# umutdundar99/progressive-stable-diffusion

Measured on AMD Instinct MI355X. Metric: images/sec at 512x512, 50 DDIM steps, bs/GPU=4, higher is better.
Workload: dtype f16; 1 GPU; 512x512, 50 DDIM steps, bs=4/GPU, delta-steer lambda=3.0, routing gates on, conditioning prep + VAE decode included; global_batch=4, parallelism=batch-shard x1 + 1 all-gather of uint8 frames

## Files before the change

### include/dadd_hip.h

```cpp
#ifndef DADD_HIP_H
#define DADD_HIP_H

#include <stdint.h>

#ifdef __cplusplus
extern "C" {
#endif

#define DADD_OK 0
#define DADD_EINVAL (-1)
#define DADD_EHIP (-2)
#define DADD_ESTATE (-3)

#define DADD_EPI_BIAS 1
#define DADD_EPI_ROWVEC 2
#define DADD_EPI_RESIDUAL 4
#define DADD_EPI_GEGLU 8
#define DADD_EPI_LNFOLD 128
#define DADD_EPI_LNSTAT 4096
#define DADD_PRE_GN 8192
#define DADD_PRE_GN_SILU 16384
#define DADD_EPI_GNSTAT 2048
#define DADD_EPI_GNAPPLY 32768
#define DADD_EPI_GNAPPLY_SILU 65536
#define DADD_EPI_QUICKGELU 256
#define DADD_EPI_GELU 512
#define DADD_EPI_SIGMOID 1024
#define DADD_EPI_ACT_MASK (256 | 512 | 1024)
#define DADD_TUNE_SHALLOW 16
#define DADD_TUNE_NODMA 32
#define DADD_TUNE_PERSIST 64

#define DADD_XATTN_SPLIT 0
#define DADD_XATTN_BASELINE 1

const char* dadd_last_error(void);
int dadd_version(void);
int dadd_init(void);
int dadd_device_info(int device, int64_t out[4]);

typedef struct {
  const void* x;
  const void* x2;
  const void* w;
  void* out;
  float* partial;
  const float* bias;
  const float* rowvec;
  const void* residual;
  int32_t B, Hi, Wi, C1, C2, Ho, Wo, N;
  int32_t taps, stride, ups, pad;
  int32_t ldo, ldr, ld_rowvec;
  int32_t splitk, flags, tile_n;
  int32_t tile_m;
  int32_t* counters;
  const float* ln_c1;
  float ln_eps;
  float* gn_ws;
  int32_t gn_nchunk, gn_cg;
  float* ln_stats_out;
  const float* ln_stats_in;
  int32_t ln_parts_out, ln_parts_in;
  const float* gn_in_ws;
  const float* gn_in_gamma;
  const float* gn_in_beta;
  int32_t gn_in_nchunk;
  float gn_in_eps;
  const float* gn_in_ws2;
  int32_t gn_in_nchunk2;
  void* gn_out;
  const float* gn_out_gamma;
  const float* gn_out_beta;
  float gn_out_eps;
} dadd_igemm_desc;
int dadd_conv_igemm_f16(const dadd_igemm_desc* d, void* stream);

typedef struct {
  const char* kernel;
  const char* finish;
  int32_t tile_m, tile_n;
  int32_t nsplit, kps;
  int32_t persistent;
  int32_t grid_x, grid_y, block;
  int32_t smem;
  int32_t gm, gn;
} dadd_igemm_choice;
int dadd_conv_igemm_resolve_f16(const dadd_igemm_desc* d, int num_cu, dadd_igemm_choice* out);

int dadd_conv3x3_cin8_f16(const void* x, const void* w, const float* bias, void* out, int B, int H,
                          int W, int Cout, void* stream);
int dadd_conv_in_nchw_f16(const float* x_nchw, const void* w, const float* bias, void* out, int B, int C,
                          int H, int W, int Cout, float* gn_ws, int gn_nchunk, void* stream);
int dadd_conv3x3_cout4_f16(const void* x, const void* w, const float* bias, float* out_nchw, int B,
                           int H, int W, int C, int Cout, int mode, void* stream);
int dadd_conv_out_ddim_f16(const void* x, const void* w, const float* bias, float* latents, const float* coef,
                           int B, int H, int W, int C, int Cout, void* stream);

int dadd_pack_nchw_f32_to_nhwc8_f16(const float* x, void* out, int B, int C, int H, int W,
                                    float scale, const float* mat, const float* vec, void* stream);

int dadd_gaussian_sample_f32(const float* mean, const float* logvar, const float* noise, float scale,
                             float* out, int64_t n, void* stream);

int dadd_frames_to_u8(const float* frames_nchw, void* out_nhwc_u8, int B, int H, int W, void* stream);

int dadd_q_sample_f32(const float* x0, const float* noise, const int64_t* t, const float* alphas_cumprod,
                      float* out, int B, int64_t per_sample, void* stream);
int dadd_mse_rows_f32(const float* pred, const float* target, float* out, int B, int64_t per_sample,
                      void* stream);

#define DADD_GN_MAX_CHUNKS 256
int dadd_groupnorm_f16(const void* x1, int C1, const void* x2, int C2, const float* gamma,
                       const float* beta, void* out, float* ws, int B, int HW, int groups,
                       float eps, int silu, int ws_chunks, void* stream);
int dadd_layernorm_f16(const void* x, const float* gamma, const float* beta, void* out, int M,
                       int C, float eps, void* stream);

int dadd_self_attn_f16(const void* q, const void* k, const void* v, void* out, int B, int N,
                       int heads, int d, int ld_qkv, int ld_out, void* stream);
int dadd_attn_f16(const void* q, const void* k, const void* v, void* out, int B, int Nq, int Nk, int heads,
                  int d, int ld_q, int ld_kv, int ld_out, void* stream);

int dadd_tri_xattn_f16(const void* q, const void* kv, void* out, const float* gates, float lambda,
                       const float* lambda_dev, int mode, int B, int N, int heads, int d, int T, int ld_kv,
                       void* stream);

int dadd_attn2_fused_f16(const void* x, const void* mcat, const void* vw, const float* bias,
                         const void* residual, void* out, float* ln_stats_out, const float* ln_stats_in,
                         int ln_parts_in, const float* ln_c1, const float* ln_d, float ln_eps, int B, int HW, int C,
                         void* stream);

int dadd_ffn_block_f16(const void* x, const void* stream, const float* ln_g, const float* ln_b, float ln_eps,
                       const float* b1, const float* b2, const float* bp, const void* xres, void* out, float* gn_ws,
                       int gn_nchunk, int M, int HW, int C, void* stream_handle);
int dadd_ffn_block_bytes(void);

int dadd_tf_head_f16(const void* x, const void* stream, const float* gn_ws, int gn_nchunk, const float* gn_g,
                     const float* gn_b, float gn_eps, const float* bp, const float* ln_g, const float* ln_b, float ln_eps,
                     void* hs, void* qkv, int M, int HW, int C, void* stream_handle);
int dadd_tf_head_bytes(void);
int dadd_tf_head_debug(void* buf);

int dadd_timestep_features_f32(const int64_t* t, float* out, int M, int dim, void* stream);
int dadd_linear_rows_f32(const float* x, const void* w, const float* bias, float* out, int M, int K,
                         int N, int act_in, int act_out, int w_f32, void* stream);
int dadd_begin_step(const float* table, float* cur_rows, int B, int ncols, const float* coef,
                    float* cur_coef, int32_t* step, void* stream);
int dadd_ddim_update_f32(float* x, const float* eps_c, const float* eps_u, float guidance,
                         const float* guidance_dev, const float* coef, int64_t n, void* stream);

int dadd_clip_patch_rows_f16(const float* pixels, void* out, int B, int H, int W, int patch, int Kp, void* stream);
int dadd_aoe_interp_f32(const float* labels, const float* base, const float* deltas, float* out, int B, int D,
                        int classes, void* stream);
int dadd_purifier_tail_f16(const void* img, const void* dis, const void* gate, const float* gamma,
                           const float* beta, float* out, int M, int C, float eps, void* stream);

// ... 50 lines not shown
```

### progressive-stable-diffusion_amd/backend.py

```python
from __future__ import annotations

import ctypes as C
from typing import Optional

import torch

from . import lib as L


def _p(t: Optional[torch.Tensor]):
    if t is None:
        return None
    if t.device.type != "cuda":
        raise ValueError(f"kernel argument lives on {t.device}, not on the GPU (shape {tuple(t.shape)}, {t.dtype})")
    return t.data_ptr()


_SFX = {torch.float16: "f16", torch.bfloat16: "bf16"}


def _sfx(*ts) -> str:
    kinds = {t.dtype for t in ts if t is not None and t.dtype in _SFX}
    if len(kinds) != 1:
        raise ValueError(f"one op takes fp16 or bf16 operands, not {sorted(str(k) for k in kinds) or 'neither'}")
    return _SFX[kinds.pop()]


def fill_igemm_desc(d, ptr, x, w, out, *, x2=None, bias=None, rowvec=None, residual=None, taps=1, stride=1,
                    ups=0, pad=0, flags=0, splitk=1, partial=None, tile_n=0, tile_m=0, counters=None, ln_c1=None,
                    ln_eps=1e-5, gn_ws=None, gn_nchunk=0, ln_stats_out=None, ln_stats_in=None, gn_in=None, gn_apply=None):
    b, hi, wi, c1 = x.shape
    c2 = 0 if x2 is None else x2.shape[-1]
    n = w.shape[0]
    ho, wo = out.shape[1], out.shape[2]
    assert w.shape[1] == taps * (c1 + c2), (w.shape, taps, c1, c2)
    assert out.shape[-1] == (n // 2 if flags & L.EPI_GEGLU else n) and out.shape[0] == b
    d.x, d.x2, d.w, d.out, d.partial = ptr(x), ptr(x2), ptr(w), ptr(out), ptr(partial)
    d.bias, d.rowvec, d.residual = ptr(bias), ptr(rowvec), ptr(residual)
    d.B, d.Hi, d.Wi, d.C1, d.C2, d.Ho, d.Wo, d.N = b, hi, wi, c1, c2, ho, wo, n
    d.taps, d.stride, d.ups, d.pad = taps, stride, ups, pad
    d.ldo, d.ldr = out.stride(-2), (residual.stride(-2) if residual is not None else 0)
    d.ld_rowvec = rowvec.stride(0) if rowvec is not None else 0
    d.splitk, d.flags, d.tile_n, d.tile_m = splitk, flags, tile_n, tile_m
    d.counters = ptr(counters)
    d.ln_c1, d.ln_eps = ptr(ln_c1), float(ln_eps)
    d.gn_ws, d.gn_nchunk, d.gn_cg = ptr(gn_ws), int(gn_nchunk), (n // 32 if gn_ws is not None else 0)
    if gn_ws is not None:
        assert flags & L.EPI_GNSTAT and gn_ws.numel() >= b * gn_nchunk * 64 and gn_ws.dtype == torch.float32
    if ln_c1 is not None:
        assert flags & L.EPI_LNFOLD and ln_c1.numel() == n and ln_c1.dtype == torch.float32
    m_rows = b * ho * wo
    d.ln_stats_out, d.ln_stats_in, d.ln_parts_out, d.ln_parts_in = ptr(ln_stats_out), ptr(ln_stats_in), 0, 0
    if ln_stats_out is not None:
        assert flags & L.EPI_LNSTAT and ln_stats_out.dtype == torch.float32 and ln_stats_out.dim() == 3 \
            and ln_stats_out.shape[1:] == (m_rows, 2) and ln_stats_out.is_contiguous()
        d.ln_parts_out = ln_stats_out.shape[0]
    if ln_stats_in is not None:
        assert flags & L.EPI_LNFOLD and ln_stats_in.dtype == torch.float32 and ln_stats_in.dim() == 3 \
            and ln_stats_in.shape[1:] == (b * hi * wi, 2) and ln_stats_in.is_contiguous()
        d.ln_parts_in = ln_stats_in.shape[0]
    d.gn_in_ws = d.gn_in_gamma = d.gn_in_beta = d.gn_in_ws2 = None
    d.gn_in_nchunk, d.gn_in_eps, d.gn_in_nchunk2 = 0, 0.0, 0
    if gn_in is not None:
        ws_in, nch_in, gam, bet, eps_in = gn_in[:5]
        assert flags & L.PRE_GN and ws_in.dtype == gam.dtype == bet.dtype == torch.float32 \
            and ws_in.numel() >= b * nch_in * 64 and gam.numel() == c1 + c2 and bet.numel() == c1 + c2
        d.gn_in_ws, d.gn_in_gamma, d.gn_in_beta = ptr(ws_in), ptr(gam), ptr(bet)
        d.gn_in_nchunk, d.gn_in_eps = int(nch_in), float(eps_in)
        if len(gn_in) > 5:
            ws2, nch2 = gn_in[5], gn_in[6]
            assert x2 is not None and ws2.dtype == torch.float32 and ws2.numel() >= b * nch2 * 64
            d.gn_in_ws2, d.gn_in_nchunk2 = ptr(ws2), int(nch2)
    d.gn_out = d.gn_out_gamma = d.gn_out_beta = None
    d.gn_out_eps = 0.0
    if gn_apply is not None:
        g_out, gam, bet, eps_o = gn_apply
        assert flags & L.EPI_GNAPPLY and g_out.shape == out.shape and g_out.dtype == out.dtype and g_out.is_contiguous() \
            and gam.dtype == bet.dtype == torch.float32 and gam.numel() == n and bet.numel() == n
        d.gn_out, d.gn_out_gamma, d.gn_out_beta, d.gn_out_eps = ptr(g_out), ptr(gam), ptr(bet), float(eps_o)
    if partial is not None:
        assert partial.numel() >= splitk * b * ho * wo * n


class HipBackend:
    name = "hip-gfx950"

    def __init__(self, device: torch.device):
        if not torch.cuda.is_available():
            raise RuntimeError("HipBackend needs a ROCm device (torch.cuda.is_available() is False)")
        self.lib = L.load()
        self.device = torch.device(device)
        self.stream = torch.cuda.Stream(device=self.device)
        self._desc = L.IgemmDesc()
        self._wdesc = L.WgradDesc()
        self._ddesc = L.DgradDesc()
        self._edesc = L.EndWgradDesc()
        self._gdesc = L.GnGradDesc()
        self._adesc = L.AttnGradDesc()
        self._n_cu = None
        self._capturing = False
        self._prof_on = False
        with torch.cuda.device(self.device):
            L.check(self.lib.dadd_init())

    @property
    def s(self):
        return self.stream.cuda_stream

    def ctx(self):
        return torch.cuda.stream(self.stream)

    def empty(self, shape, dtype):
        with self.ctx():
            return torch.empty(shape, dtype=dtype, device=self.device)

    def zeros(self, shape, dtype):
        with self.ctx():
            return torch.zeros(shape, dtype=dtype, device=self.device)

    def _after_producer(self, src: torch.Tensor):
        if src.device.type == "cuda" and not self._capturing:
            cur = torch.cuda.current_stream(self.device)
            if cur != self.stream:
                self.stream.wait_stream(cur)
                src.record_stream(self.stream)

    def to_device(self, t: torch.Tensor, dtype=None):
        self._after_producer(t)
        with self.ctx():
            return t.to(device=self.device, dtype=dtype or t.dtype).contiguous()

    def copy_(self, dst: torch.Tensor, src: torch.Tensor):
        self._after_producer(src)
        with self.ctx():
            dst.copy_(src.reshape(dst.shape))

    def zero_(self, t: torch.Tensor):
        with self.ctx():
            t.zero_()

    def clone(self, t: torch.Tensor):
        with self.ctx():
            return t.detach().clone()

    def synchronize(self):
        self.stream.synchronize()

    def wait_current(self):
        self.stream.wait_stream(torch.cuda.current_stream(self.device))

    def release_to_current(self):
        torch.cuda.current_stream(self.device).wait_stream(self.stream)

    @staticmethod
    def _scratch_numel(fn, args, message):
        n = int(fn(*args))
        if n < 0:
            raise ValueError(message.format(*args))
        return n

    def _splitm(self, m, tiles):
        if self._n_cu is None:
            self._n_cu = torch.cuda.get_device_properties(self.device).multi_processor_count
        return max(1, min(-(-2 * self._n_cu // tiles), -(-m // 64)))

    @staticmethod
    def _param_grad_checks(dgamma, dbeta, c, ws, need):
        together = (dgamma is None) == (dbeta is None)
        shaped = all(t is None or (t.dtype == torch.float32 and t.numel() == c and t.is_contiguous()) for t in (dgamma, dbeta))
        ws_ok = ws is not None and ws.dtype == torch.float32 and ws.is_contiguous() and ws.numel() >= need
        return together, shaped, ws_ok

    @staticmethod
    def _pointwise_width(op, f):
        if f % 8 or f == 0:
            raise ValueError(f"{op}: F = {f} must be a positive multiple of 8")

    def pack_latents(self, x, out, scale=1.0, mat=None, vec=None):
        b, c, h, w = x.shape
        assert x.dtype == torch.float32 and out.dtype == torch.float16 and out.shape == (b, h, w, 8)
        L.check(self.lib.dadd_pack_nchw_f32_to_nhwc8_f16(_p(x), _p(out), b, c, h, w, float(scale),
                                                         _p(mat), _p(vec), self.s))

    def conv_cin8(self, x, w, bias, out):
        b, h, wd, c8 = x.shape
        assert c8 == 8 and w.shape[1:] == (9, 8) and out.shape == (b, h, wd, w.shape[0])
        L.check(self.lib.dadd_conv3x3_cin8_f16(_p(x), _p(w), _p(bias), _p(out), b, h, wd, w.shape[0],
                                               self.s))

    def conv_in_nchw(self, x, w, bias, out, gn_ws=None, gn_nchunk=0):
        b, c, h, wd = x.shape
        assert x.dtype == torch.float32 and c <= 4 and w.shape[1:] == (9, 8) and out.shape == (b, h, wd, w.shape[0])
        assert gn_ws is None or (gn_ws.dtype == torch.float32 and gn_ws.numel() >= b * gn_nchunk * 64)
        fn = getattr(self.lib, "dadd_conv_in_nchw_" + _sfx(w, out))
        L.check(fn(_p(x), _p(w), _p(bias), _p(out), b, c, h, wd, w.shape[0], _p(gn_ws), gn_nchunk, self.s))

    def conv_cout4(self, x, w, bias, out, mode=0):
        b, h, wd, c = x.shape
        co = w.shape[0]
        assert w.shape == (co, 9, c) and out.shape == (b, co, h, wd) and out.dtype == torch.float32
        fn = getattr(self.lib, "dadd_conv3x3_cout4_" + _sfx(x, w))
        L.check(fn(_p(x), _p(w), _p(bias), _p(out), b, h, wd, c, co, int(mode), self.s))

    def conv_out_ddim(self, x, w, bias, latents, coef):
        b, h, wd, c = x.shape
        co = w.shape[0]
        assert w.shape == (co, 9, c) and latents.shape == (b, co, h, wd) and latents.dtype == torch.float32 \
            and coef.numel() == 4 and coef.dtype == torch.float32
        fn = getattr(self.lib, "dadd_conv_out_ddim_" + _sfx(x, w))
        L.check(fn(_p(x), _p(w), _p(bias), _p(latents), _p(coef), b, h, wd, c, co, self.s))

    def q_sample(self, x0, noise, t, alphas_cumprod, out):
        b = x0.shape[0]
        assert x0.dtype == torch.float32 and t.dtype == torch.int64 and t.shape == (b,) and noise.shape == x0.shape
        L.check(self.lib.dadd_q_sample_f32(_p(x0), _p(noise), _p(t), _p(alphas_cumprod), _p(out), b,
                                           x0.numel() // b, self.s))

    def mse_rows(self, pred, target, out):
        b = pred.shape[0]
        assert pred.shape == target.shape and out.shape == (b,) and pred.dtype == torch.float32
        L.check(self.lib.dadd_mse_rows_f32(_p(pred), _p(target), _p(out), b, pred.numel() // b, self.s))

    def frames_to_u8(self, frames, out):
        b, c, h, w = frames.shape
        assert c == 3 and frames.dtype == torch.float32 and out.dtype == torch.uint8 and out.shape == (b, h, w, 3)
        L.check(self.lib.dadd_frames_to_u8(_p(frames), _p(out), b, h, w, self.s))

    def gaussian_sample(self, mean, logvar, noise, out, scale=1.0):
        assert mean.shape == logvar.shape == noise.shape == out.shape and mean.dtype == torch.float32
        L.check(self.lib.dadd_gaussian_sample_f32(_p(mean), _p(logvar), _p(noise), float(scale), _p(out),
                                                  mean.numel(), self.s))

    def igemm(self, x, w, out, *, x2=None, bias=None, rowvec=None, residual=None, taps=1, stride=1,
              ups=0, pad=0, flags=0, splitk=1, partial=None, tile_n=0, tile_m=0, counters=None, ln_c1=None,
              ln_eps=1e-5, gn_ws=None, gn_nchunk=0, ln_stats_out=None, ln_stats_in=None, gn_in=None, gn_apply=None):
        fn = getattr(self.lib, "dadd_conv_igemm_" + _sfx(x, x2, w, out, residual, None if gn_apply is None else gn_apply[0]))
        d = self._desc
        fill_igemm_desc(d, _p, x, w, out, x2=x2, bias=bias, rowvec=rowvec, residual=residual, taps=taps, stride=stride,
                        ups=ups, pad=pad, flags=flags, splitk=splitk, partial=partial, tile_n=tile_n, tile_m=tile_m,
                        counters=counters, ln_c1=ln_c1, ln_eps=ln_eps, gn_ws=gn_ws, gn_nchunk=gn_nchunk,
                        ln_stats_out=ln_stats_out, ln_stats_in=ln_stats_in, gn_in=gn_in, gn_apply=gn_apply)
        L.check(fn(C.byref(d), self.s))

    def wgrad_splitm(self, m, n, c, taps=1):
        return self._splitm(m, -(-n // 64) * taps * (c // 64))

    @staticmethod
    def wgrad_partial_numel(splitm, n, c, taps=1):
        return splitm * (n * taps * c + n) if splitm > 1 else 0

    @staticmethod
    def _pixel_ld(t):
        ld = t.stride(-2)
        want, ok = ld, t.stride(-1) == 1
        for size, st in zip(reversed(t.shape[:-1]), reversed(t.stride()[:-1])):
            ok = ok and (size == 1 or st == want)
            want *= size
        if not ok:
            raise ValueError(f"expected dense pixels with one row stride, got shape {tuple(t.shape)} strides {t.stride()}")
        return ld

    def wgrad(self, dy, x, dw, *, dbias=None, taps=1, stride=1, ups=0, pad=0, splitm=None, partial=None, ld_tap=None):
        if dy.dim() == 2:
            dy, x = dy.unsqueeze(0).unsqueeze(0), x.unsqueeze(0).unsqueeze(0)
        b, ho, wo, n = dy.shape
        bx, hi, wi, c = x.shape
        assert bx == b and dy.dim() == 4 and x.dim() == 4
        fn = getattr(self.lib, "dadd_conv_wgrad_" + _sfx(dy, x))
        assert dw.dtype == torch.float32 and dw.stride(-1) == 1 and dw.shape[0] == n
        if dw.dim() == 3:
            assert dw.shape[1:] == (taps, c) and ld_tap in (None, dw.stride(1))
            ld_tap = dw.stride(1)
        else:
            ld_tap = c if ld_tap is None else ld_tap
            assert dw.dim() == 2 and dw.shape[1] >= (taps - 1) * ld_tap + c
        assert dbias is None or (dbias.dtype == torch.float32 and dbias.numel() == n and dbias.is_contiguous())
        m = b * ho * wo
        if splitm is None:
            splitm = self.wgrad_splitm(m, n, c, taps)
        if splitm > 1:
            if partial is None:
                raise ValueError(f"wgrad with splitm = {splitm} needs a partial buffer")
            assert partial.dtype == torch.float32 and partial.is_contiguous() \
                and partial.numel() >= self.wgrad_partial_numel(splitm, n, c, taps), (partial.shape, splitm, n, taps, c)
        d = self._wdesc
        d.dy, d.x, d.dw, d.dbias, d.partial = _p(dy), _p(x), _p(dw), _p(dbias), _p(partial)
        d.B, d.Hi, d.Wi, d.C, d.Ho, d.Wo, d.N = b, hi, wi, c, ho, wo, n
        d.taps, d.stride, d.ups, d.pad = taps, stride, int(ups), pad
        d.ld_dy, d.ld_x, d.ld_dw, d.ld_tap = self._pixel_ld(dy), self._pixel_ld(x), dw.stride(0), ld_tap
        d.splitm = splitm
        L.check(fn(C.byref(d), self.s))

    def dgrad(self, dy, wt, dx, *, taps=1):
        if dy.dim() == 2:
            dy, dx = dy.view(1, 1, *dy.shape), dx.view(1, 1, *dx.shape)
        n = dy.shape[-1]
        if n % 64 != 0:
            raise ValueError(f"dgrad contracts over the N = {n} output channels of the forward; the GEMM kernels need "
                             "a multiple of 64 (the data gradient of the 4-channel conv_out is dgrad_cout4)")
        assert taps in (1, 9) and wt.shape == (dx.shape[-1], taps * n) and dy.is_contiguous() and dx.is_contiguous()
        self.igemm(dy, wt, dx, taps=taps, pad=1 if taps == 9 else 0)

    def dgrad_cout4(self, dy_nchw_f32, wt, dx):
        if dy_nchw_f32.dim() != 4 or dy_nchw_f32.dtype != torch.float32 or not 1 <= dy_nchw_f32.shape[1] <= 4:
            raise ValueError(f"dgrad_cout4 takes dy fp32 NCHW with 1..4 channels, got {tuple(dy_nchw_f32.shape)} {dy_nchw_f32.dtype}")
        b, _, h, wd = dy_nchw_f32.shape
        if wt.dim() != 3 or wt.shape[1:] != (9, 8) or dx.shape != (b, h, wd, wt.shape[0]) or not (
                dy_nchw_f32.is_contiguous() and wt.is_contiguous() and dx.is_contiguous()):
            raise ValueError(f"dgrad_cout4: dy {tuple(dy_nchw_f32.shape)} takes contiguous wt [C,9,8] and dx [B,H,W,C], got "
                             f"{tuple(wt.shape)} and {tuple(dx.shape)}")
        self.conv_in_nchw(dy_nchw_f32, wt, None, dx)

    def end_wgrad_splitm(self, m, cw):
        return self._splitm(m, max(1, cw // 64))

    def end_wgrad_partial_numel(self, splitm, ct, cw, mode):
        return self._scratch_numel(self.lib.dadd_end_wgrad_partial_floats, (int(mode), int(ct), int(cw), int(splitm)),
                                   "end_wgrad takes mode 0 or 1, Ct in 1..4 and Cw a multiple of 64 (got mode {}, Ct {}, Cw {})")

    def end_wgrad(self, thin, wide, dw, *, dbias=None, mode, splitm=None, partial=None):
        if thin.dim() != 4 or wide.dim() != 4 or thin.dtype != torch.float32 or not thin.is_contiguous():
            raise ValueError(f"end_wgrad takes thin fp32 NCHW (contiguous) and wide NHWC, got {tuple(thin.shape)} {thin.dtype} "
                             f"and {tuple(wide.shape)}")
        b, ct, h, wd = thin.shape
# ... 460 lines not shown
```

### progressive-stable-diffusion_amd/csrc/bf16_names.h

```cpp
#pragma once
#define DADD_BF16 1

#define IgemmArgs IgemmArgs_bf16
#define IgemmLaunch IgemmLaunch_bf16

#define igemm_kernel igemm_kernel_bf16
#define splitk_finish_kernel splitk_finish_kernel_bf16
#define splitk_finish_gn_kernel splitk_finish_gn_kernel_bf16
#define splitk_finish_gnapply_kernel splitk_finish_gnapply_kernel_bf16
#define igemm_dma_kernel igemm_dma_kernel_bf16
#define conv3x3_halo_kernel conv3x3_halo_kernel_bf16
#define gn_stats_kernel gn_stats_kernel_bf16
#define gn_apply_kernel gn_apply_kernel_bf16
#define gn_fused_kernel gn_fused_kernel_bf16
#define gn_reduce_kernel gn_reduce_kernel_bf16
#define layernorm_kernel layernorm_kernel_bf16
#define flash_kernel flash_kernel_bf16
#define xattn_kernel xattn_kernel_bf16
#define conv_in_nchw_kernel conv_in_nchw_kernel_bf16
#define conv_in_nchw_gn_kernel conv_in_nchw_gn_kernel_bf16
#define conv_cout4_kernel conv_cout4_kernel_bf16
#define wgrad_kernel wgrad_kernel_bf16
#define wgrad_finish_kernel wgrad_finish_kernel_bf16
#define gn_grad_stats_kernel gn_grad_stats_kernel_bf16
#define gn_grad_partial_kernel gn_grad_partial_kernel_bf16
#define gn_grad_apply_kernel gn_grad_apply_kernel_bf16
#define layernorm_grad_kernel layernorm_grad_kernel_bf16
#define geglu_kernel geglu_kernel_bf16
#define geglu_grad_kernel geglu_grad_kernel_bf16
#define attn_grad_stats_kernel attn_grad_stats_kernel_bf16
#define attn_grad_dkv_kernel attn_grad_dkv_kernel_bf16
#define attn_grad_dq_kernel attn_grad_dq_kernel_bf16
#define dgrad_kernel dgrad_kernel_bf16
#define EndWgradArgs EndWgradArgs_bf16
#define end_wgrad_kernel end_wgrad_kernel_bf16
#define end_wgrad_finish_kernel end_wgrad_finish_kernel_bf16
#define gelu_kernel gelu_kernel_bf16
#define gelu_grad_kernel gelu_grad_kernel_bf16
#define gate_tail_kernel gate_tail_kernel_bf16
#define gate_tail_grad_kernel gate_tail_grad_kernel_bf16
#define rowvec_grad_kernel rowvec_grad_kernel_bf16
#define rowvec_grad_finish_kernel rowvec_grad_finish_kernel_bf16
#define relayout_kernel relayout_kernel_bf16

#define dadd_init_igemm dadd_init_igemm_bf16
#define dadd_init_igemm_dma dadd_init_igemm_dma_bf16
#define dadd_igemm_dma_row dadd_igemm_dma_row_bf16
#define dadd_igemm_resolve dadd_igemm_resolve_bf16
#define dadd_init_conv_halo dadd_init_conv_halo_bf16
#define dadd_conv_halo_applicable dadd_conv_halo_applicable_bf16
#define dadd_conv_halo_gn_channels dadd_conv_halo_gn_channels_bf16
#define dadd_conv_halo_row dadd_conv_halo_row_bf16
#define dadd_init_norm dadd_init_norm_bf16
#define dadd_init_attention dadd_init_attention_bf16
#define dadd_init_attn_grad dadd_init_attn_grad_bf16

#define dadd_conv_igemm_f16 dadd_conv_igemm_bf16
#define dadd_conv_igemm_resolve_f16 dadd_conv_igemm_resolve_bf16
#define dadd_groupnorm_f16 dadd_groupnorm_bf16
#define dadd_layernorm_f16 dadd_layernorm_bf16
#define dadd_attn_f16 dadd_attn_bf16
#define dadd_attn_debug dadd_attn_debug_bf16
#define dadd_self_attn_f16 dadd_self_attn_bf16
#define dadd_tri_xattn_f16 dadd_tri_xattn_bf16
#define dadd_conv_in_nchw_f16 dadd_conv_in_nchw_bf16
#define dadd_conv3x3_cout4_f16 dadd_conv3x3_cout4_bf16
#define dadd_conv_out_ddim_f16 dadd_conv_out_ddim_bf16
#define dadd_conv_wgrad_f16 dadd_conv_wgrad_bf16

#define dadd_groupnorm_grad_f16 dadd_groupnorm_grad_bf16
#define dadd_layernorm_grad_f16 dadd_layernorm_grad_bf16
#define dadd_geglu_f16 dadd_geglu_bf16
#define dadd_geglu_grad_f16 dadd_geglu_grad_bf16

#define dadd_attn_grad_f16 dadd_attn_grad_bf16

#define dadd_gelu_f16 dadd_gelu_bf16
#define dadd_gelu_grad_f16 dadd_gelu_grad_bf16
#define dadd_purifier_gate_tail_f16 dadd_purifier_gate_tail_bf16
#define dadd_purifier_gate_tail_grad_f16 dadd_purifier_gate_tail_grad_bf16

#define dadd_rowvec_grad_f16 dadd_rowvec_grad_bf16

#define dadd_conv_dgrad_f16 dadd_conv_dgrad_bf16

#define dadd_conv_end_wgrad_f16 dadd_conv_end_wgrad_bf16

#define dadd_dgrad_relayout_f16 dadd_dgrad_relayout_bf16
```

### progressive-stable-diffusion_amd/csrc/igemm.hip

```cpp
#include "dadd_common.h"
#include "igemm_args.h"
#include <cstdlib>
#include <string>
#include "igemm_epilogue.h"

namespace {

constexpr int BM = 128;
constexpr int BK = 64;

__device__ __forceinline__ int lds_off(int row, int chunk) {
  return (row * 8 + (chunk ^ ((row >> 1) & 7))) * 8;
}

template <int BM, int BN, bool DEEP>
__global__ __launch_bounds__(256, 2) void igemm_kernel(const IgemmArgs p) {
  constexpr int WM = BM / 2;
  constexpr int MI = WM / 16;
  constexpr int WN = BN / 2;
  constexpr int J = WN / 16;
  constexpr int EPI = (DEEP && BN == 128) ? EPI_COLS : EPI_TILE;
  constexpr int NA = BM * 8 / 256;
  constexpr int NB = BN * 8 / 256;
  extern __shared__ __attribute__((aligned(16))) char smem[];
// ... 298 lines not shown
#pragma unroll
        for (int e = 0; e < VEC; ++e) v[e] = fmaf(keep, tt[u][e], v[e]);
      }
    }
    if (p.flags & DADD_EPI_BIAS) v += *reinterpret_cast<const fv*>(p.bias + c);
    if (p.flags & DADD_EPI_ROWVEC) v += *reinterpret_cast<const fv*>(p.rowvec + (size_t)b * p.ld_rowvec + c);
    if (p.flags & DADD_EPI_RESIDUAL) {
      const hv rv = *reinterpret_cast<const hv*>(p.residual + m * p.ldr + c);
#pragma unroll
      for (int e = 0; e < VEC; ++e) v[e] += (float)rv[e];
    }
    hv o;
#pragma unroll
    for (int e = 0; e < VEC; ++e) o[e] = (half_t)v[e];
    *reinterpret_cast<hv*>(p.out + m * p.ldo + c) = o;
    *reinterpret_cast<hv*>(slab + row * cg + VEC * cv) = o;
  }
  __syncthreads();
  float s = 0.f, ss = 0.f;
  if (t < 256) {
    for (int idx = t; idx < npair; idx += 256) {
      const h2 v = *reinterpret_cast<const h2*>(slab + 2 * idx);
      const float a = (float)v[0], d = (float)v[1];
      s += a + d;
      ss += a * a + d * d;
    }
    s = wave_sum(s);
    ss = wave_sum(ss);
    if (lane == 0) { red[0][wave] = s; red[1][wave] = ss; }
  }
  __syncthreads();
  const double n = (double)HW * (double)cg;
  const double sum = (double)red[0][0] + (double)red[0][1] + (double)red[0][2] + (double)red[0][3];
  const double sq = (double)red[1][0] + (double)red[1][1] + (double)red[1][2] + (double)red[1][3];
  const double mu = sum / n;
  double var = sq / n - mu * mu;
  if (var < 0.0) var = 0.0;
  const float mean = (float)mu, rstd = (float)(1.0 / sqrt(var + (double)p.gno_eps));
  const bool silu = (p.flags & DADD_EPI_GNAPPLY_SILU) != 0;
  for (int idx = t; idx < npair; idx += 512) {
    const int row = idx / hp, cp = idx - row * hp;
    const int c = c0 + 2 * cp;
    const h2 v = *reinterpret_cast<const h2*>(slab + 2 * idx);
    h2 o;
#pragma unroll
    for (int e = 0; e < 2; ++e) {
      const float sc = rstd * p.gno_gamma[c + e];
      float f = ((float)v[e] - mean) * sc + p.gno_beta[c + e];
      if (silu) f = dadd_silu(f);
      o[e] = (half_t)f;
    }
    *reinterpret_cast<h2*>(p.gno_out + ((size_t)b * HW + row) * p.N + c) = o;
  }
}

constexpr double L2_KEEP = 3.0e6;

constexpr int smem_bytes(int bm, int bn) {
  return 2 * (bm + bn) * BK * (int)sizeof(half_t) + (bm == 128 ? (bn == 160 ? 8192 : LN_LDS_BYTES) : 4096);
}

#define REG_ROW(BM, BN, DEEP) \
  {DADD_KNAME("igemm_kernel") "<" #BM ", " #BN ", " #DEEP ">", igemm_kernel<BM, BN, DEEP>, 256, smem_bytes(BM, BN), {BM, BN, DEEP}}
const IgemmKernel REG_KERNELS[] = {
    REG_ROW(128, 128, false), REG_ROW(128, 128, true), REG_ROW(128, 160, false), REG_ROW(64, 128, false),
    REG_ROW(64, 128, true),   REG_ROW(64, 160, false), REG_ROW(64, 160, true),
};
#undef REG_ROW
#define FIN_ROW(KERNEL, THREADS, ...) {DADD_KNAME(#KERNEL), KERNEL<__VA_ARGS__>, THREADS, 0, {__VA_ARGS__}}
const IgemmFinish FINISH_KERNELS[] = {
    FIN_ROW(splitk_finish_gnapply_kernel, 512, 4), FIN_ROW(splitk_finish_gnapply_kernel, 512, 2),
    {DADD_KNAME("splitk_finish_kernel"), splitk_finish_kernel, 256, 0, {}},
    FIN_ROW(splitk_finish_gn_kernel, 256, 160, 16), FIN_ROW(splitk_finish_gn_kernel, 256, 160, 64),
    FIN_ROW(splitk_finish_gn_kernel, 256, 128, 16), FIN_ROW(splitk_finish_gn_kernel, 256, 128, 64),
};
#undef FIN_ROW

int g_num_cu = 0;

}

int dadd_init_igemm() {
  int rc = dadd_init_igemm_dma();
  if (rc == DADD_OK) rc = dadd_init_conv_halo();
  if (rc == DADD_OK) rc = dadd_set_max_lds(REG_KERNELS);
  int dev = 0;
  DADD_HIP(hipGetDevice(&dev));
  DADD_HIP(hipDeviceGetAttribute(&g_num_cu, hipDeviceAttributeMultiprocessorCount, dev));
  return rc;
}

int dadd_igemm_resolve(const dadd_igemm_desc* d, int num_cu, IgemmLaunch* out) {
  DADD_REQUIRE(d != nullptr, "igemm: null descriptor");
  IgemmArgs& a = out->a;
  a = IgemmArgs{};
  a.x = static_cast<const half_t*>(d->x);
  a.x2 = static_cast<const half_t*>(d->x2);
  a.w = static_cast<const half_t*>(d->w);
  a.out = static_cast<half_t*>(d->out);
  a.partial = d->partial;
  a.bias = d->bias;
  a.rowvec = d->rowvec;
  a.residual = static_cast<const half_t*>(d->residual);
  a.counters = d->counters;
  a.B = d->B; a.Hi = d->Hi; a.Wi = d->Wi; a.C1 = d->C1; a.C2 = d->C2;
  a.Ho = d->Ho; a.Wo = d->Wo; a.N = d->N;
  a.taps = d->taps; a.stride = d->stride; a.ups = d->ups; a.pad = d->pad;
  a.flags = d->flags & (15 | DADD_TUNE_PERSIST | DADD_EPI_LNFOLD | DADD_EPI_ACT_MASK | DADD_EPI_GNSTAT | DADD_EPI_LNSTAT |
                        DADD_PRE_GN | DADD_PRE_GN_SILU | DADD_EPI_GNAPPLY | DADD_EPI_GNAPPLY_SILU);
  a.gno_out = static_cast<half_t*>(d->gn_out);
  a.gno_gamma = d->gn_out_gamma;
  a.gno_beta = d->gn_out_beta;
  a.gno_eps = d->gn_out_eps;
  a.gn_ws = d->gn_ws;
  a.gn_nchunk = d->gn_nchunk;
  a.gn_cg = d->gn_cg;
  a.ln_c1 = d->ln_c1;
  a.ln_eps = d->ln_eps;
  a.gni_ws = d->gn_in_ws;
  a.gni_gamma = d->gn_in_gamma;
  a.gni_beta = d->gn_in_beta;
  a.gni_nchunk = d->gn_in_nchunk;
  a.gni_eps = d->gn_in_eps;
  a.gni_ws2 = d->gn_in_ws2;
  a.gni_nchunk2 = d->gn_in_nchunk2;
  a.ln_stats_out = d->ln_stats_out;
  a.ln_stats_in = (a.flags & DADD_EPI_LNFOLD) ? d->ln_stats_in : nullptr;
  a.ln_parts_in = d->ln_parts_in;
  const int Cin = a.C1 + a.C2;
  const bool geglu = (a.flags & DADD_EPI_GEGLU) != 0;
  a.ldo = d->ldo > 0 ? d->ldo : (geglu ? a.N / 2 : a.N);
  a.ldr = d->ldr > 0 ? d->ldr : a.N;
  a.ld_rowvec = d->ld_rowvec > 0 ? d->ld_rowvec : a.N;

  DADD_REQUIRE(a.x && a.w && a.out, "igemm: null x/w/out");
  DADD_REQUIRE(a.taps == 1 || a.taps == 9, "igemm: taps must be 1 or 9, got %d", a.taps);
  DADD_REQUIRE(a.B > 0 && a.Hi > 0 && a.Wi > 0 && a.Ho > 0 && a.Wo > 0 && a.N > 0,
               "igemm: non-positive extent");
  DADD_REQUIRE(Cin % 64 == 0 && a.C1 % 64 == 0 && a.C1 > 0,
               "igemm: channels must be multiples of 64 (C1=%d C2=%d)", a.C1, a.C2);
  DADD_REQUIRE(a.C2 == 0 || a.x2 != nullptr, "igemm: C2>0 needs x2");
  DADD_REQUIRE(a.N % 8 == 0, "igemm: N must be a multiple of 8, got %d", a.N);
  DADD_REQUIRE(a.stride == 1 || a.stride == 2, "igemm: stride must be 1 or 2");
  DADD_REQUIRE(!(a.ups && (a.stride != 1 || a.taps != 9)), "igemm: ups needs a stride-1 3x3");
  DADD_REQUIRE(dadd_aligned16(a.x) && dadd_aligned16(a.w) && dadd_aligned16(a.out) &&
                   (a.x2 == nullptr || dadd_aligned16(a.x2)),
               "igemm: pointers must be 16-byte aligned");
  DADD_REQUIRE(!(a.flags & DADD_EPI_BIAS) || a.bias, "igemm: bias flag without bias");
  DADD_REQUIRE(!(a.flags & DADD_EPI_ROWVEC) || a.rowvec, "igemm: rowvec flag without rowvec");
  DADD_REQUIRE(!(a.flags & DADD_EPI_RESIDUAL) || a.residual, "igemm: residual flag without ptr");
  DADD_REQUIRE(!(a.flags & DADD_EPI_ACT_MASK) || (!geglu && d->splitk <= 1),
               "igemm: an activation epilogue excludes GEGLU and split-K");
  DADD_REQUIRE(!(a.flags & DADD_EPI_LNFOLD) || (a.ln_c1 && a.taps == 1 && a.C2 == 0 && d->splitk <= 1 && a.ln_eps > 0.f),
               "igemm: a folded LayerNorm needs c1, a plain linear over one source (K = C) and no split-K");
  DADD_REQUIRE(a.ln_stats_in == nullptr ||
                   (a.ln_parts_in > 0 && (size_t)a.ln_parts_in * a.B * a.Ho * a.Wo * 8 < 0x7FF00000ull),
               "igemm: ln_stats_in needs ln_parts_in > 0 and fewer than 2 GiB of partials");
  DADD_REQUIRE(a.ldo % 4 == 0 && a.ldr % 4 == 0 && a.ld_rowvec % 4 == 0,
               "igemm: leading dimensions must be multiples of 4");

  a.M = a.B * a.Ho * a.Wo;
  a.K = a.taps * Cin;
  a.nkt = a.K / BK;
  int tile_n = d->tile_n;
  if (geglu) {
    DADD_REQUIRE(a.N % 128 == 0 && (tile_n == 0 || tile_n == 128), "igemm: GEGLU needs N%%128==0");
    tile_n = 128;
  }
  if (tile_n == 0) tile_n = (a.N % 160 == 0) ? 160 : 128;
  DADD_REQUIRE(tile_n == 64 || tile_n == 128 || tile_n == 160, "igemm: tile_n must be 64, 128 or 160");
  a.ntiles = (a.N + tile_n - 1) / tile_n;

  int splitk = d->splitk > 1 ? d->splitk : 1;
  if (splitk > a.nkt) splitk = a.nkt;
  a.kps = (a.nkt + splitk - 1) / splitk;
  const int nsplit = (a.nkt + a.kps - 1) / a.kps;
  a.splitk = nsplit;
  DADD_REQUIRE(nsplit == 1 || (a.partial != nullptr && !geglu),
               "igemm: split-K needs a partial buffer and no GEGLU");

  bool deep = (d->flags & DADD_TUNE_SHALLOW) == 0;
  int tile_m = d->tile_m;
  DADD_REQUIRE(tile_m == 0 || tile_m == 64 || tile_m == 128, "igemm: tile_m must be 0, 64 or 128");
  if (tile_m == 0) tile_m = 128;
  a.mtiles = (a.M + tile_m - 1) / tile_m;
  {
    const double a_bytes = 2.0 * a.B * a.Hi * a.Wi * Cin, w_bytes = 2.0 * a.N * a.K;
    if (a_bytes >= w_bytes) {
      a.gm = (a.mtiles + 7) / 8;
      a.gn = a.ntiles;
    } else {
      a.gm = a.mtiles;
      a.gn = (a.ntiles + 7) / 8;
    }
    if (a.taps == 1 && !(a_bytes >= w_bytes) && a_bytes > L2_KEEP) {
      double best = 1e30;
      for (int ms = 2; ms <= 4; ms *= 2) {
        const int ns = 8 / ms;
        if (a.mtiles % ms || a.ntiles % ns || a_bytes / ms > L2_KEEP) continue;
        const double fetch = a_bytes / ms + w_bytes / ns;
        if (fetch < best) { best = fetch; a.gm = a.mtiles / ms; a.gn = a.ntiles / ns; }
      }
    }
  }
  a.korder = 0;
  const bool dma = ((d->flags & DADD_TUNE_NODMA) == 0 || ((a.flags & DADD_EPI_LNFOLD) && !a.ln_stats_in)) &&
                   !(tile_m == 64 && a.ups);
  DADD_REQUIRE(tile_n != 64 || (dma && tile_m == 64 && !geglu), "igemm: 64-column tiles exist for the 64-row LDS-DMA kernel only");
  const bool persistent = dma && tile_m == 128 && (a.flags & DADD_TUNE_PERSIST) && nsplit == 1 && !a.ups && num_cu > 0 &&
                          a.mtiles * a.ntiles > num_cu;
  if (persistent && ((d->flags & DADD_TUNE_SHALLOW) ? false : 2.0 * a.B * a.Hi * a.Wi * Cin >= 2.0 * a.N * a.K))
    a.gm = a.gn = 0;
  a.fd_on = (size_t)a.B * a.Ho * a.Wo < DADD_FASTDIV_MAX && (size_t)a.K < DADD_FASTDIV_MAX &&
            (size_t)a.mtiles * a.ntiles < DADD_FASTDIV_MAX;
  a.plain = a.taps == 1 && a.stride == 1 && a.pad == 0 && !a.ups && a.Ho == a.Hi && a.Wo == a.Wi;
  if (a.fd_on) {
    a.fd_howo = dadd_fastdiv_make((uint32_t)(a.Ho * a.Wo));
    a.fd_wo = dadd_fastdiv_make((uint32_t)a.Wo);
    a.fd_cin = dadd_fastdiv_make((uint32_t)Cin);
    a.ngn = 1;
    a.fd_t1 = a.fd_t2 = dadd_fastdiv_make(1);
    if (a.gm == 0) {
      a.fd_t0 = dadd_fastdiv_make((uint32_t)a.ntiles);
    } else if (a.gn >= a.ntiles) {
      a.fd_t0 = dadd_fastdiv_make((uint32_t)(a.gm * a.ntiles));
      a.fd_t1 = dadd_fastdiv_make((uint32_t)a.gm);
    } else if (a.gm >= a.mtiles) {
      a.fd_t0 = dadd_fastdiv_make((uint32_t)(a.mtiles * a.gn));
      a.fd_t1 = dadd_fastdiv_make((uint32_t)a.mtiles);
    } else {
      a.ngn = a.ntiles / a.gn;
      a.fd_t0 = dadd_fastdiv_make((uint32_t)(a.gm * a.gn));
      a.fd_t1 = dadd_fastdiv_make((uint32_t)a.gm);
      a.fd_t2 = dadd_fastdiv_make((uint32_t)a.ngn);
    }
  }
  const bool halo = dma && tile_m == 128 && dadd_conv_halo_applicable(a, tile_n);
  int halo_ns = 1;
  if (halo) {
    const int chunks = Cin / BK;
    int sk = d->splitk > 1 ? d->splitk : 1;
    if (sk > chunks) sk = chunks;
    a.kps = (chunks + sk - 1) / sk;
    halo_ns = (chunks + a.kps - 1) / a.kps;
    a.splitk = halo_ns;
    DADD_REQUIRE(halo_ns == 1 || a.partial != nullptr, "igemm: split-K needs a partial buffer");
  }
  if ((a.flags & DADD_EPI_GNSTAT) && (halo ? halo_ns : nsplit) > 1) {
    const int cb = (a.N % 160 == 0) ? 160 : 128, howo = a.Ho * a.Wo;
    const int rows = a.gn_nchunk > 0 ? howo / a.gn_nchunk : 0;
    DADD_REQUIRE(a.gn_ws && a.gn_cg > 0 && a.N == 32 * a.gn_cg && !geglu && a.counters == nullptr && a.N % cb == 0 &&
                     cb % a.gn_cg == 0 && (rows == 16 || rows == 64) && a.M % rows == 0 && howo % rows == 0 &&
                     a.gn_nchunk * rows == howo && !(a.flags & (DADD_EPI_LNFOLD | DADD_EPI_ACT_MASK)),
                 "igemm: GroupNorm statistics with split-K need the finish kernel (no tickets), N == 32 groups in blocks of "
                 "160 / 128 columns, and chunks of 16 or 64 rows: gn_nchunk == Ho*Wo / 16 (or / 64)");
  } else if (a.flags & DADD_EPI_GNSTAT) {
    const int wm_rows = tile_m / 2, wn_cols = tile_n / 2, howo = a.Ho * a.Wo;
    DADD_REQUIRE(a.gn_ws && a.gn_cg > 0 && a.N == 32 * a.gn_cg && !geglu && (tile_n == 128 || tile_n == 160) &&
                     wn_cols % a.gn_cg == 0 && a.M % tile_m == 0 && a.N % tile_n == 0 && howo % wm_rows == 0 &&
                     a.gn_nchunk == howo / wm_rows && !(a.flags & (DADD_EPI_LNFOLD | DADD_EPI_ACT_MASK)),
                 "igemm: GroupNorm statistics need full tiles of 128/160 columns holding whole groups, whole-wave row blocks "
                 "inside one sample (Ho*Wo %% %d == 0, gn_nchunk == Ho*Wo / %d), N == 32 groups, no split-K", wm_rows, wm_rows);
  }
  if (a.flags & DADD_EPI_GNAPPLY) {
    DADD_REQUIRE((halo ? halo_ns : nsplit) > 1 && a.counters == nullptr && a.gno_out && a.gno_gamma && a.gno_beta &&
                     a.gno_eps > 0.f && a.N % 64 == 0 && a.ldo % 2 == 0 && a.ldr % 2 == 0 &&
                     (size_t)a.Ho * a.Wo * (a.N / 32) * 2 <= 16 * 1024 && dadd_aligned16(a.gno_out) &&
                     !(a.flags & (DADD_EPI_GNSTAT | DADD_EPI_LNFOLD | DADD_EPI_LNSTAT | DADD_EPI_ACT_MASK)),
                 "igemm: GroupNorm of the output in the finish kernel needs a finish-kernel split-K launch, gn_out / gamma / "
                 "beta / eps, N %% 64 == 0, a (sample, group) slab of <= 16 KiB and no other statistics / activation flags");
  } else {
    DADD_REQUIRE(!(a.flags & DADD_EPI_GNAPPLY_SILU), "igemm: DADD_EPI_GNAPPLY_SILU without DADD_EPI_GNAPPLY");
  }
  if (a.flags & DADD_EPI_LNSTAT) {
    const int wn_cols = tile_n / 2;
    DADD_REQUIRE(a.ln_stats_out && !geglu && !halo && a.N % wn_cols == 0 && d->ln_parts_out == a.N / wn_cols &&
                     (nsplit == 1 || a.counters != nullptr) && !(a.flags & DADD_EPI_GNSTAT),
                 "igemm: LayerNorm row partials need ln_stats_out, N %% (tile_n/2) == 0, ln_parts_out == N / (tile_n/2) = %d, "
                 "no GEGLU and no finish-kernel split-K", a.N / wn_cols);
  }
  if (a.flags & DADD_PRE_GN) {
    const int cgc = Cin / 32;
    DADD_REQUIRE(a.C2 == 0 || (a.gni_ws2 && a.gni_nchunk2 >= 1 && a.gni_nchunk2 <= 256 && cgc > 0 && a.C1 % 32 == 0 &&
                               a.C2 % 32 == 0 && cgc % (a.C1 / 32) == 0 && cgc % (a.C2 / 32) == 0 && a.C1 % cgc == 0),
                 "igemm: GroupNorm over a concatenation needs the partials of both sources and group widths that nest "
                 "((C1+C2)/32 a multiple of C1/32 and C2/32, dividing C1)");
    DADD_REQUIRE(halo && !(d->flags & DADD_TUNE_SHALLOW) && Cin <= dadd_conv_halo_gn_channels(a.Wo) &&
                     Cin % 32 == 0 && a.gni_ws &&
                     a.gni_gamma && a.gni_beta && a.gni_nchunk >= 1 && a.gni_nchunk <= 256 && a.gni_eps > 0.f,
                 "igemm: GroupNorm on the way in needs the 3x3 halo kernel (stride 1, 64/32/16-wide map, 128x160 tiles), "
                 "Cin <= 1152 / 2048 / 2432 (W = 64 / 32 / 16), the chunk partials (<= 256 chunks), gamma, beta and eps");
  } else {
    DADD_REQUIRE(!(a.flags & DADD_PRE_GN_SILU), "igemm: DADD_PRE_GN_SILU without DADD_PRE_GN");
  }
  const bool window = (size_t)a.B * a.Hi * a.Wi * (size_t)(a.C1 > a.C2 ? a.C1 : a.C2) * 2 < 0x7FF00000ull &&
                      (size_t)a.N * a.K * 2 < 0x7FF00000ull;
  out->nsplit = halo ? halo_ns : nsplit;
  out->tile_m = tile_m;
  out->tile_n = tile_n;
  out->persistent = !halo && persistent;
  out->grid = out->persistent ? dim3(num_cu) : dim3(a.mtiles * a.ntiles, out->nsplit);
  a.pf_kt = (dma && !halo && a.korder == 0 && !out->persistent && a.mtiles >= DADD_PF_MIN_SHARE)
                ? (a.kps < DADD_PF_KTILES ? a.kps : DADD_PF_KTILES) : 0;
  if (halo) {
    DADD_REQUIRE(window, "conv_halo: operand larger than the 2 GiB buffer window");
    const bool duo = (d->flags & DADD_TUNE_SHALLOW) != 0 && !(a.flags & DADD_PRE_GN);
    if (d->flags & DADD_TUNE_SHALLOW) a.flags |= DADD_TUNE_SHALLOW;
    out->main = dadd_conv_halo_row(a.Wo, duo, (a.flags & DADD_PRE_GN) != 0);
  } else if (dma) {
    DADD_REQUIRE(window, "igemm(dma): operand larger than the 2 GiB buffer window");
    DADD_REQUIRE(tile_m == 128 || !a.ups, "igemm(dma): the 64-row tiles have no upsample gather");
    const int lnk = (a.ups || !(a.flags & DADD_EPI_LNFOLD)) ? 0 : (a.ln_stats_in == nullptr ? 1 : (tile_m == 128 ? 2 : 0));
    out->main = dadd_igemm_dma_row(tile_m, tile_n, !out->persistent && tile_m == 128 && a.ups, out->persistent, lnk);
  } else {
    out->main = dadd_find_row(REG_KERNELS, tile_m, tile_n, deep && !(tile_m == 128 && tile_n == 160));
  }
  DADD_REQUIRE(out->main != nullptr, "igemm: no kernel for %d x %d tiles", tile_m, tile_n);
  out->finish = nullptr;
  out->fgrid = dim3(0);
  out->fsmem = 0;
  if (out->nsplit > 1 && a.counters == nullptr) {
    if (a.flags & DADD_EPI_GNAPPLY) {
      const bool vec4 = (a.N / 32) % 4 == 0 && a.ldo % 4 == 0 && a.ldr % 4 == 0 && a.ld_rowvec % 4 == 0;
      out->finish = dadd_find_row(FINISH_KERNELS, vec4 ? 4 : 2);
      out->fgrid = dim3(32, a.B);
      out->fsmem = (unsigned)(a.Ho * a.Wo * (a.N / 32) * 2);
    } else if (!(a.flags & DADD_EPI_GNSTAT)) {
      const size_t total = (size_t)a.M * (a.N / 4);
      const int blocks = (int)((total + 255) / 256);
      out->finish = dadd_find_row(FINISH_KERNELS, 0);
      out->fgrid = dim3(blocks > 2048 ? 2048 : blocks);
    } else {
      const int cb = (a.N % 160 == 0) ? 160 : 128, rows = (a.Ho * a.Wo) / a.gn_nchunk == 16 ? 16 : 64;
      out->finish = dadd_find_row(FINISH_KERNELS, cb, rows);
      out->fgrid = dim3(a.M / rows, a.N / cb);
    }
  }
  return DADD_OK;
}

extern "C" int dadd_conv_igemm_f16(const dadd_igemm_desc* d, void* stream) {
  hipStream_t s = static_cast<hipStream_t>(stream);
  IgemmLaunch l;
  const int rc = dadd_igemm_resolve(d, g_num_cu, &l);
  if (rc != DADD_OK) return rc;
  const IgemmArgs& a = l.a;
  dadd_launch({l.main->name, dadd_igemm_flop(a), dadd_igemm_bytes(a)}, l.main->fn, l.grid, dim3(l.main->threads), l.main->smem, s, a);
  if (l.finish) {
    double bytes = (double)a.M * a.N * (4.0 * l.nsplit + 2.0 + ((a.flags & DADD_EPI_RESIDUAL) ? 2.0 : 0.0));
    if (a.flags & DADD_EPI_GNAPPLY) bytes += 2.0 * a.M * a.N;
    dadd_launch({l.finish->name, 0.0, bytes}, l.finish->fn, l.fgrid, dim3(l.finish->threads), l.fsmem, s, a, l.nsplit);
  }
  DADD_LAUNCH_CHECK();
  return DADD_OK;
}

extern "C" int dadd_conv_igemm_resolve_f16(const dadd_igemm_desc* d, int num_cu, dadd_igemm_choice* out) {
  DADD_REQUIRE(out != nullptr, "igemm: null choice");
  IgemmLaunch l;
  const int rc = dadd_igemm_resolve(d, num_cu, &l);
  if (rc != DADD_OK) return rc;
  *out = {l.main->name, l.finish ? l.finish->name : nullptr, l.tile_m, l.tile_n, l.nsplit, l.a.kps, l.persistent,
          (int)l.grid.x, (int)l.grid.y, l.main->threads, l.main->smem, l.a.gm, l.a.gn};
  return DADD_OK;
}
```

### progressive-stable-diffusion_amd/csrc/igemm_args.h

```cpp
#pragma once
#include "dadd_common.h"
#include "fastdiv.h"

struct IgemmArgs {
  const half_t* x;
  const half_t* x2;
  const half_t* w;
  half_t* out;
  float* partial;
  const float* bias;
  const float* rowvec;
  const half_t* residual;
  int* counters;
  float* gn_ws;
  int gn_nchunk, gn_cg;
  const float* ln_c1;
  float ln_eps;
  float* ln_stats_out;
  const float* ln_stats_in;
  int ln_parts_in;
  const float* gni_ws;
  const float* gni_gamma;
  const float* gni_beta;
  int gni_nchunk;
  float gni_eps;
  const float* gni_ws2;
  int gni_nchunk2;
  half_t* gno_out;
  const float* gno_gamma;
  const float* gno_beta;
  float gno_eps;
  int B, Hi, Wi, C1, C2, Ho, Wo, N;
  int taps, stride, ups, pad;
  int ldo, ldr, ld_rowvec;
  int splitk, flags;
  int M, K, nkt, kps, ntiles;
  int korder;
  int mtiles, gm, gn;
  int fd_on, plain;
  dadd_fastdiv fd_howo, fd_wo, fd_cin;
  dadd_fastdiv fd_t0, fd_t1, fd_t2;
  int ngn;
  int pf_kt;
};

#ifndef DADD_PF_KTILES
#define DADD_PF_KTILES 24
#endif
#ifndef DADD_PF_MIN_SHARE
#define DADD_PF_MIN_SHARE 16
#endif
typedef unsigned dadd_u4 __attribute__((ext_vector_type(4)));
__device__ __forceinline__ dadd_u4 dadd_pf_desc(const void* base, int bytes) {
  const unsigned long long a = (unsigned long long)base;
  return dadd_u4{(unsigned)a, (unsigned)(a >> 32) & 0xFFFFu, (unsigned)bytes, 0x00020000u};
}
__device__ __forceinline__ void dadd_pf_line(unsigned& sink, unsigned off, dadd_u4 desc) {
#if defined(__HIP_DEVICE_COMPILE__)
  asm volatile("buffer_load_dword %0, %1, %2, 0 offen" : "+v"(sink) : "v"(off), "s"(desc));
#endif
}
__device__ __forceinline__ void dadd_pf_drain(unsigned& sink) {
#if defined(__HIP_DEVICE_COMPILE__)
  asm volatile("s_waitcnt vmcnt(0)" : "+v"(sink)::"memory");
#endif
}

__device__ __forceinline__ int row_sample(const IgemmArgs& p, int m, int HoWo) {
  return p.fd_on ? (int)dadd_fastdiv_div((uint32_t)m, p.fd_howo) : m / HoWo;
}
__device__ __forceinline__ void row_decode(const IgemmArgs& p, int m, int HoWo, int& b, int& oy, int& ox) {
  b = row_sample(p, m, HoWo);
  const int rem = m - b * HoWo;
  oy = p.fd_on ? (int)dadd_fastdiv_div((uint32_t)rem, p.fd_wo) : rem / p.Wo;
  ox = rem - oy * p.Wo;
}

__device__ __forceinline__ int xcd_remap(int bid, int nwg) {
  const int q = nwg >> 3, r = nwg & 7, xcd = bid & 7, slot = bid >> 3;
  return (xcd < r ? xcd * (q + 1) : r * (q + 1) + (xcd - r) * q) + slot;
}

__device__ __forceinline__ void tile_decode(const IgemmArgs& p, int tile_id, int& mt, int& nt) {
  if (p.gm == 0) {
    nt = tile_id % p.ntiles;
    mt = tile_id / p.ntiles;
  } else if (p.gn >= p.ntiles) {
    const int per = p.gm * p.ntiles;
    const int g = tile_id / per, idx = tile_id - g * per;
    const int base = g * p.gm;
    const int gsz = min(p.gm, p.mtiles - base);
    mt = base + idx % gsz;
    nt = idx / gsz;
  } else if (p.gm >= p.mtiles) {
    const int per = p.mtiles * p.gn;
    const int g = tile_id / per, idx = tile_id - g * per;
    mt = idx % p.mtiles;
    nt = g * p.gn + idx / p.mtiles;
  } else {
    const int per = p.gm * p.gn;
    const int g = tile_id / per, idx = tile_id - g * per;
    const int ngn = p.ntiles / p.gn;
    const int gmi = g / ngn, gni = g - gmi * ngn;
    mt = gmi * p.gm + idx % p.gm;
    nt = gni * p.gn + idx / p.gm;
  }
}

__device__ __forceinline__ void tile_decode_fast(const IgemmArgs& p, int tile_id, int& mt, int& nt) {
  const auto div = [&](int n, const dadd_fastdiv& f, int d) { return p.fd_on ? (int)dadd_fastdiv_div((uint32_t)n, f) : n / d; };
  if (p.gm == 0) {
    mt = div(tile_id, p.fd_t0, p.ntiles);
    nt = tile_id - mt * p.ntiles;
  } else if (p.gn >= p.ntiles) {
    const int per = p.gm * p.ntiles;
    const int g = div(tile_id, p.fd_t0, per), idx = tile_id - g * per;
    const int base = g * p.gm;
    const int gsz = min(p.gm, p.mtiles - base);
    nt = gsz == p.gm ? div(idx, p.fd_t1, p.gm) : idx / gsz;
    mt = base + idx - nt * gsz;
  } else if (p.gm >= p.mtiles) {
    const int per = p.mtiles * p.gn;
    const int g = div(tile_id, p.fd_t0, per), idx = tile_id - g * per;
    const int q = div(idx, p.fd_t1, p.mtiles);
    mt = idx - q * p.mtiles;
    nt = g * p.gn + q;
  } else {
    const int per = p.gm * p.gn;
    const int g = div(tile_id, p.fd_t0, per), idx = tile_id - g * per;
    const int gmi = div(g, p.fd_t2, p.ngn), gni = g - gmi * p.ngn;
    const int q = div(idx, p.fd_t1, p.gm);
    mt = gmi * p.gm + idx - q * p.gm;
    nt = gni * p.gn + q;
  }
}

static inline double dadd_igemm_flop(const IgemmArgs& a) { return 2.0 * (double)a.M * (double)a.N * (double)a.K; }
static inline double dadd_igemm_bytes(const IgemmArgs& a) {
  const double n_out = (a.flags & DADD_EPI_GEGLU) ? a.N / 2 : a.N;
  return 2.0 * ((double)a.B * a.Hi * a.Wi * (a.C1 + a.C2) + (double)a.N * a.K + (double)a.M * n_out +
                ((a.flags & DADD_EPI_RESIDUAL) ? (double)a.M * a.N : 0.0));
}

typedef half_t dadd_h2 __attribute__((ext_vector_type(2)));
__device__ __forceinline__ void ln_acc_pair(const h8& x, int p, float& s1, float& s2) {
  const dadd_h2 v = {x[2 * p], x[2 * p + 1]};
  const dadd_h2 one = {(half_t)1.0f, (half_t)1.0f};
  s1 = dadd_fdot2(v, one, s1);
  s2 = dadd_fdot2(v, v, s2);
}
template <int MI>
__device__ __forceinline__ void ln_finish(float (&s1)[MI], float (&s2)[MI], int K, float eps) {
  const float inv = 1.0f / (float)K;
#pragma unroll
  for (int i = 0; i < MI; ++i) {
    float a = s1[i], q = s2[i];
    a = dadd_sum_x16x32(a);
    q = dadd_sum_x16x32(q);
    const float mu = a * inv;
    const float var = fmaxf(q * inv - mu * mu, 0.f);
    s1[i] = mu;
    s2[i] = rsqrtf(var + eps);
  }
}

template <typename... A>
struct KernelRow {
  const char* name;
  void (*fn)(A...);
  int threads, smem;
  int targ[5];
};
typedef KernelRow<IgemmArgs> IgemmKernel;
typedef KernelRow<IgemmArgs, int> IgemmFinish;

template <typename Row, int N>
inline const Row* dadd_find_row(const Row (&rows)[N], int k0, int k1 = 0, int k2 = 0, int k3 = 0, int k4 = 0) {
  for (const Row& r : rows)
    if (r.targ[0] == k0 && r.targ[1] == k1 && r.targ[2] == k2 && r.targ[3] == k3 && r.targ[4] == k4) return &r;
  return nullptr;
}
template <typename Row, int N>
inline int dadd_set_max_lds(const Row (&rows)[N]) {
  for (const Row& r : rows)
    DADD_HIP(hipFuncSetAttribute(reinterpret_cast<const void*>(r.fn), hipFuncAttributeMaxDynamicSharedMemorySize, r.smem));
  return DADD_OK;
}

struct IgemmLaunch {
  IgemmArgs a;
  const IgemmKernel* main;
  dim3 grid;
  const IgemmFinish* finish;
  dim3 fgrid;
  unsigned fsmem;
  int nsplit;
  int tile_m, tile_n;
  bool persistent;
};
int dadd_igemm_resolve(const dadd_igemm_desc* d, int num_cu, IgemmLaunch* out);

int dadd_init_igemm_dma();
const IgemmKernel* dadd_igemm_dma_row(int tile_m, int tile_n, bool ups, bool persistent, int lnk);
int dadd_init_conv_halo();
bool dadd_conv_halo_applicable(const IgemmArgs& a, int tile_n);
int dadd_conv_halo_gn_channels(int Wo);
const IgemmKernel* dadd_conv_halo_row(int Wo, bool duo, bool gn_in);
```

### progressive-stable-diffusion_amd/csrc/igemm_dma.hip

```cpp
#include "dadd_common.h"
#include "igemm_args.h"
#include <cstdlib>
#include "igemm_epilogue.h"

namespace {

constexpr int BK = 64;

typedef __attribute__((address_space(3))) void* lptr_t;
constexpr unsigned OOB = 0x80000000u;

__device__ __forceinline__ int lds_off(int row, int chunk) {
  return (row * 8 + (chunk ^ ((row >> 1) & 7))) * 8;
}

template <int N>
__device__ __forceinline__ void wait_vmcnt() {
  asm volatile("s_waitcnt vmcnt(%0)" ::"n"(N) : "memory");
}

template <int BM, int BN, bool UPS, bool PERS, int LNK>
__global__ __launch_bounds__(512, (BM + BN) <= 128 ? 4 : 2) void igemm_dma_kernel(const IgemmArgs p) {
#if defined(__HIP_DEVICE_COMPILE__)
  constexpr bool WS = true;
  constexpr bool LNF = LNK == 1;
  constexpr int WM = BM / 2, MI = WM / 16;
  constexpr int WN = BN / 2;
  constexpr int J = WN / 16;
  constexpr int EPI = !PERS ? EPI_TILE : (BN == 160 && LNK == 2) ? EPI_COLS : EPI_ROWS;
  constexpr int NA = BM / 32;
  constexpr int NBJ = BN / 32;
  constexpr int LPT = NA + NBJ;
  constexpr int A_BYTES = BM * BK * 2, B_BYTES = BN * BK * 2, STAGE = A_BYTES + B_BYTES;
  extern __shared__ __attribute__((aligned(1024))) char smem[];

  const int t = threadIdx.x, lane = t & 63;
  const int wave_all = __builtin_amdgcn_readfirstlane(t >> 6);
  const bool loader = WS && wave_all >= 4;
  const int wave = WS ? (wave_all & 3) : wave_all;
  const int wm = wave >> 1, wn = wave & 1;
  int tile_first, tile_count;
  if constexpr (PERS) {
    const int total = p.mtiles * p.ntiles, nwg = gridDim.x;
    const int l = xcd_remap(blockIdx.x, nwg);
    const int q = total / nwg, r = total - q * nwg;
    tile_first = l * q + min(l, r);
    tile_count = q + (l < r ? 1 : 0);
  } else {
    tile_first = xcd_remap(blockIdx.x, gridDim.x);
    tile_count = 1;
  }
  const int z = PERS ? 0 : blockIdx.y;
  const int kt0 = PERS ? 0 : z * p.kps;
  const int kt1 = PERS ? p.nkt : min(p.nkt, kt0 + p.kps);
  const int nk = kt1 - kt0;
  const int Cin = p.C1 + p.C2;
  const int Hv = UPS ? 2 * p.Hi : p.Hi;
  const int Wv = UPS ? 2 * p.Wi : p.Wi;
  const int HoWo = p.Ho * p.Wo;
  const int lrow = lane >> 3, lch = lane & 7;

  const int shift1 = UPS ? 0 : (p.pad * p.Wi + p.pad) * p.C1;
  const int shift2 = UPS ? 0 : (p.pad * p.Wi + p.pad) * p.C2;
  const size_t pix_total = (size_t)p.B * p.Hi * p.Wi;
  const int rec1 = (int)((pix_total * p.C1 + shift1) * 2);
  const int rec2 = (int)((pix_total * p.C2 + shift2) * 2);
  const int recW = (int)((size_t)p.N * p.K * 2);
  const half_t* base1 = p.x - shift1;
  const half_t* base2 = (p.x2 ? p.x2 : p.x) - shift2;

  unsigned a_v1[NA], a_v2[NA], a_mask[NA];
  int a_pix[NA], a_y[NA], a_x[NA], a_cc[NA];
  unsigned w_v[NBJ];
  auto setup_tile = [&](int tile_id) __attribute__((always_inline)) {
  int nt, mt;
  tile_decode_fast(p, tile_id, mt, nt);
  const int m0 = mt * BM, n0 = nt * BN;
#pragma unroll
  for (int i = 0; i < NA; ++i) {
    const int row = (i * 4 + wave) * 8 + lrow;
    const int m = m0 + row;
    const bool ok = m < p.M;
    const int mm = ok ? m : 0;
    const int cc = (lch ^ ((row >> 1) & 7)) * 8;
    if (!UPS && p.plain) {
      a_v1[i] = (unsigned)((mm * p.C1 + cc) * 2);
      a_v2[i] = (unsigned)((mm * p.C2 + cc) * 2);
      a_mask[i] = ok ? 1u : 0u;
      continue;
    }
    int b, oy, ox;
    row_decode(p, mm, HoWo, b, oy, ox);
    const int pix = b * p.Hi * p.Wi;
    const int y0 = oy * p.stride - p.pad, x0 = ox * p.stride - p.pad;
    a_pix[i] = pix; a_y[i] = ok ? y0 : -100000; a_x[i] = x0; a_cc[i] = cc;
    const int org = pix + oy * p.stride * p.Wi + ox * p.stride;
    a_v1[i] = (unsigned)((org * p.C1 + cc) * 2);
    a_v2[i] = (unsigned)((org * p.C2 + cc) * 2);
    unsigned my = 0, mx = 0;
#pragma unroll
    for (int k3 = 0; k3 < 3; ++k3) {
      my |= (y0 + k3 >= 0 && y0 + k3 < Hv) ? 1u << k3 : 0u;
      mx |= (x0 + k3 >= 0 && x0 + k3 < Wv) ? 1u << k3 : 0u;
    }
    const unsigned mask9 = ((my & 1u) ? mx : 0u) | ((my & 2u) ? mx << 3 : 0u) | ((my & 4u) ? mx << 6 : 0u);
    a_mask[i] = ok ? (p.taps == 9 ? mask9 : (my & mx & 1u)) : 0u;
  }
#pragma unroll
  for (int j = 0; j < NBJ; ++j) {
    const int row = (j * 4 + wave) * 8 + lrow;
    const int n = n0 + row;
    w_v[j] = (n < p.N) ? (unsigned)(((size_t)n * p.K + (lch ^ ((row >> 1) & 7)) * 8) * 2) : OOB;
  }
  };
  int iss_tile = tile_first, iss_left = tile_count;

  const bool tapfast = p.korder != 0;
  int cur_kt = kt0;
  int cur_tap = 0, cur_c = 0, cur_koff = 0, cur_ky = 0, cur_kx = 0;
  auto cursor_init = [&]() {
    if (kt0 == 0) return;
    const int tap0 = p.fd_on ? (int)dadd_fastdiv_div((uint32_t)(kt0 * BK), p.fd_cin) : (kt0 * BK) / Cin;
    cur_tap = __builtin_amdgcn_readfirstlane(tapfast ? kt0 % 9 : tap0);
    cur_c = __builtin_amdgcn_readfirstlane(tapfast ? (kt0 / 9) * BK : kt0 * BK - cur_tap * Cin);
    cur_koff = __builtin_amdgcn_readfirstlane((cur_tap * Cin + cur_c) * 2);
    cur_ky = (p.taps == 9) ? cur_tap / 3 : 0;
    cur_kx = (p.taps == 9) ? cur_tap - 3 * cur_ky : 0;
  };
  int fill_off = wave * 1024;

  struct IssueCtx {
    __amdgpu_buffer_rsrc_t rsA, rsW;
    unsigned soff, koff;
    char* sa;
    int cs, cb, ky, kx, tap;
    bool second;
  };
  auto issue_begin = [&]() {
    IssueCtx c;
    const bool live = PERS ? iss_left > 0 : cur_kt < kt1;
    c.second = cur_c >= p.C1;
    c.cs = c.second ? p.C2 : p.C1;
    c.cb = c.second ? cur_c - p.C1 : cur_c;
    c.ky = cur_ky; c.kx = cur_kx; c.tap = cur_tap;
    c.rsA = __builtin_amdgcn_make_buffer_rsrc((void*)(c.second ? base2 : base1), 0,
                                              live ? (c.second ? rec2 : rec1) : 0, 0x00020000);
    c.rsW = __builtin_amdgcn_make_buffer_rsrc((void*)p.w, 0, live ? recW : 0, 0x00020000);
    c.sa = smem + fill_off;
    c.soff = UPS ? (unsigned)(c.cb * 2) : (unsigned)(((cur_ky * p.Wi + cur_kx) * c.cs + c.cb) * 2);
    c.koff = (unsigned)cur_koff;
    return c;
  };
  auto issue_w = [&](const IssueCtx& c, int j) {
    __builtin_amdgcn_raw_ptr_buffer_load_lds(c.rsW, (lptr_t)(c.sa + A_BYTES + j * 4096), 16, w_v[j], c.koff, 0, 0);
  };
  auto issue_advance = [&]() {
    ++cur_kt;
    const int c1 = cur_c + BK;
    const int cwrap = c1 >= Cin ? 1 : 0;
    const int kx1 = cur_kx + (tapfast ? 1 : cwrap);
    const int w3 = kx1 == 3 ? 1 : 0;
    cur_kx = w3 ? 0 : kx1;
    const int ky1 = cur_ky + w3;
    const int w9 = (tapfast && ky1 == 3) ? 1 : 0;
    cur_ky = w9 ? 0 : ky1;
    cur_koff += tapfast ? (w9 ? (BK - 8 * Cin) * 2 : Cin * 2) : BK * 2;
    cur_tap = tapfast ? (w9 ? 0 : cur_tap + 1) : cur_tap + cwrap;
    cur_c = tapfast ? cur_c + (w9 ? BK : 0) : (cwrap ? 0 : c1);
    const int f1 = fill_off + STAGE;
    fill_off = f1 >= 4 * STAGE ? f1 - 4 * STAGE : f1;
    if constexpr (PERS) {
      if (cur_kt == kt1) {
        cur_kt = 0; cur_c = 0; cur_tap = 0; cur_ky = 0; cur_kx = 0; cur_koff = 0;
        ++iss_tile;
        --iss_left;
        if (iss_left > 0) setup_tile(iss_tile);
      }
    }
  };
  unsigned a_eff[NA];
  int eff_key = -1;
  auto issue = [&]() {
    const IssueCtx c = issue_begin();
    {
      const int key = c.tap * 2 + (c.second ? 1 : 0) + (PERS ? iss_tile * 32 : 0);
      if (key != eff_key) {
        eff_key = key;
#pragma unroll
        for (int i = 0; i < NA; ++i) {
          if constexpr (!UPS) {
            a_eff[i] = ((a_mask[i] >> c.tap) & 1u) ? (c.second ? a_v2[i] : a_v1[i]) : OOB;
          } else {
            const int iy = a_y[i] + c.ky, ix = a_x[i] + c.kx;
            const bool ok = (iy >= 0) & (iy < Hv) & (ix >= 0) & (ix < Wv);
            a_eff[i] = ok ? (unsigned)(((a_pix[i] + (iy >> 1) * p.Wi + (ix >> 1)) * c.cs + a_cc[i]) * 2) : OOB;
          }
        }
      }
#pragma unroll
      for (int i = 0; i < NA; ++i)
        __builtin_amdgcn_raw_ptr_buffer_load_lds(c.rsA, (lptr_t)(c.sa + i * 4096), 16, a_eff[i], c.soff, 0, 0);
#pragma unroll
      for (int jj = 0; jj < NBJ; ++jj) issue_w(c, jj);
    }
    issue_advance();
  };

  const int total_kt = tile_count * nk;
  char* const ln_scr = smem + 4 * STAGE;
  const bool ln_stage = LNK == 2 && !UPS && ln_lds_usable(p, BM, nk);
  const bool ln_sts = ln_stage && ln_lds_stats(p, LN_LDS_BYTES);
  if (loader) {
    const int ln_extra = ln_stage ? ln_lds_count(p, wave, ln_sts) : 0;
    cursor_init();
    setup_tile(tile_first);
    issue();
    issue();
    issue();
    wait_vmcnt<LPT>();
    __builtin_amdgcn_s_barrier();
    bool ext_young = false;
    int kc = 0, ext_tile = tile_first;
    for (int it = 0; it < total_kt; ++it) {
      if (it > 0) {
        if (ext_young) {
          switch (ln_extra) {
            case 1: wait_vmcnt<LPT + 1>(); break;
            case 2: wait_vmcnt<LPT + 2>(); break;
            case 3: wait_vmcnt<LPT + 3>(); break;
            case 4: wait_vmcnt<LPT + 4>(); break;
            default: wait_vmcnt<LPT>(); break;
          }
          ext_young = false;
        } else {
          wait_vmcnt<LPT>();
        }
        __builtin_amdgcn_s_barrier();
      }
      issue();
      if (ln_stage) {
        if (kc == 0) {
          int nt, mt;
          tile_decode_fast(p, ext_tile, mt, nt);
          ln_lds_issue<BN>(p, ln_scr, __builtin_amdgcn_readfirstlane(mt) * BM, __builtin_amdgcn_readfirstlane(nt) * BN, wave,
                           lane, ln_sts);
          ext_young = ln_extra > 0;
          ++ext_tile;
        }
        kc = kc + 1 == nk ? 0 : kc + 1;
      }
    }
    wait_vmcnt<0>();
    return;
  }
  f4 acc[J][MI];
  const int fq = lane >> 4;
  int fa[2], fb[2];
#pragma unroll
  for (int s2 = 0; s2 < 2; ++s2) {
    fa[s2] = lds_off(wm * WM + (lane & 15), s2 * 4 + fq) * 2;
    fb[s2] = A_BYTES + lds_off(wn * WN + (lane & 15), s2 * 4 + fq) * 2;
  }
  unsigned pf_sink = 0;
  if (!PERS && p.pf_kt > 0) {
    int nt, mt;
    tile_decode_fast(p, tile_first, mt, nt);
    mt = __builtin_amdgcn_readfirstlane(mt);
    const int n0 = __builtin_amdgcn_readfirstlane(nt) * BN;
    const dadd_u4 dw = dadd_pf_desc(p.w, recW);
    const unsigned row_bytes = (unsigned)p.K * 2u;
    const int total = BN * min(nk, p.pf_kt);
    for (int q0 = wave * 64; q0 * p.mtiles + mt < total; q0 += 256) {
      const int l = (q0 + lane) * p.mtiles + mt;
      const int kt = l / BN, n = n0 + l - kt * BN;
      const unsigned off = (l < total && n < p.N) ? (unsigned)n * row_bytes + (unsigned)((kt0 + kt) * BK * 2) : OOB;
      dadd_pf_line(pf_sink, off, dw);
    }
  }
  __builtin_amdgcn_s_barrier();
  __builtin_amdgcn_sched_barrier(0);
  h8 xa0[MI], wb0[J], xa1[MI], wb1[J];
#pragma unroll
  for (int i = 0; i < MI; ++i) xa0[i] = *reinterpret_cast<const h8*>(smem + fa[0] + i * 2048);
#pragma unroll
  for (int j = 0; j < J; ++j) wb0[j] = *reinterpret_cast<const h8*>(smem + fb[0] + j * 2048);
  int comp_off = 0;
  bool started = false;
  for (int tl = 0; tl < tile_count; ++tl) {
#pragma unroll
    for (int j = 0; j < J; ++j)
#pragma unroll
      for (int i = 0; i < MI; ++i) acc[j][i] = f4{0.f, 0.f, 0.f, 0.f};
    [[maybe_unused]] float ls1[MI], ls2[MI];
    constexpr int LQ = MI * 4, LPER = (LQ + MI * J - 1) / (MI * J);
    if constexpr (LNF) {
#pragma unroll
      for (int i = 0; i < MI; ++i) ls1[i] = ls2[i] = 0.f;
    }
    for (int it = 0; it < nk; ++it) {
      if (started) __builtin_amdgcn_s_barrier();
      started = true;
      __builtin_amdgcn_sched_barrier(0);
      const int n1 = comp_off + STAGE;
      const int next_off = n1 >= 4 * STAGE ? 0 : n1;
      const char* ca = smem + comp_off + fa[1];
      const char* cb1 = smem + comp_off + fb[1];
      const char* na = smem + next_off + fa[0];
      const char* nb = smem + next_off + fb[0];
#pragma unroll
      for (int k = 0; k < MI * J; ++k) {
        const int jj = k / MI, ii = k % MI;
        acc[jj][ii] = DADD_MFMA_16X16X32(wb0[jj], xa0[ii], acc[jj][ii], 0, 0, 0);
        if constexpr (LNF) {
#pragma unroll
          for (int t2 = 0; t2 < LPER; ++t2)
            if (k * LPER + t2 < LQ) ln_acc_pair(xa0[(k * LPER + t2) / 4], (k * LPER + t2) % 4, ls1[(k * LPER + t2) / 4], ls2[(k * LPER + t2) / 4]);
        }
        if (k == 0) wb1[0] = *reinterpret_cast<const h8*>(cb1);
        else if (k <= MI) xa1[k - 1] = *reinterpret_cast<const h8*>(ca + (k - 1) * 2048);
        else if (k < MI + J) wb1[k - MI] = *reinterpret_cast<const h8*>(cb1 + (k - MI) * 2048);
        __builtin_amdgcn_sched_barrier(0);
      }
#pragma unroll
      for (int k = 0; k < MI * J; ++k) {
        const int jj = k / MI, ii = k % MI;
        acc[jj][ii] = DADD_MFMA_16X16X32(wb1[jj], xa1[ii], acc[jj][ii], 0, 0, 0);
        if constexpr (LNF) {
#pragma unroll
          for (int t2 = 0; t2 < LPER; ++t2)
            if (k * LPER + t2 < LQ) ln_acc_pair(xa1[(k * LPER + t2) / 4], (k * LPER + t2) % 4, ls1[(k * LPER + t2) / 4], ls2[(k * LPER + t2) / 4]);
        }
        if (k == 0) wb0[0] = *reinterpret_cast<const h8*>(nb);
        else if (k <= MI) xa0[k - 1] = *reinterpret_cast<const h8*>(na + (k - 1) * 2048);
        else if (k < MI + J) wb0[k - MI] = *reinterpret_cast<const h8*>(nb + (k - MI) * 2048);
        __builtin_amdgcn_sched_barrier(0);
      }
      comp_off = next_off;
      __builtin_amdgcn_sched_barrier(0);
    }
    dadd_pf_drain(pf_sink);
    int nt, mt;
    tile_decode_fast(p, tile_first + tl, mt, nt);
    if constexpr (LNF) {
      ln_finish<MI>(ls1, ls2, p.K, p.ln_eps);
      igemm_epilogue<J, MI, WM, WN, EPI>(p, acc, mt * BM, nt * BN, wm, wn, lane, z, smem, ls1, ls2);
    } else {
      igemm_epilogue<J, MI, WM, WN, EPI>(p, acc, mt * BM, nt * BN, wm, wn, lane, z, smem, nullptr, nullptr, smem + 4 * STAGE,
                                    ln_sts ? ln_scr + LN_LDS_STATS : nullptr, ln_stage ? ln_scr : nullptr);
    }
  }
#endif
}

constexpr int smem_bytes(int bm, int bn) {
  return 4 * (bm + bn) * BK * 2 + (bm == 128 ? LN_LDS_BYTES : 4096);
}

#define DMA_ROW(BM, BN, UPS, PERS, LNK)                                                                                \
  {DADD_KNAME("igemm_dma_kernel") "<" #BM ", " #BN ", " #UPS ", " #PERS ", " #LNK ">", igemm_dma_kernel<BM, BN, UPS, PERS, LNK>, \
   512, smem_bytes(BM, BN), {BM, BN, UPS, PERS, LNK}}
#define DMA_ROWS2(BM, BN, PERS) DMA_ROW(BM, BN, false, PERS, 0), DMA_ROW(BM, BN, false, PERS, 1)
#define DMA_ROWS3(BM, BN, PERS) DMA_ROWS2(BM, BN, PERS), DMA_ROW(BM, BN, false, PERS, 2)
const IgemmKernel DMA_KERNELS[] = {
    DMA_ROWS3(128, 128, true),  DMA_ROWS3(128, 160, true),
    DMA_ROWS3(128, 128, false), DMA_ROWS3(128, 160, false),
    DMA_ROW(128, 128, true, false, 0), DMA_ROW(128, 160, true, false, 0),
    DMA_ROWS2(64, 64, false), DMA_ROWS2(64, 128, false), DMA_ROWS2(64, 160, false),
};
#undef DMA_ROWS3
#undef DMA_ROWS2
#undef DMA_ROW

}

int dadd_init_igemm_dma() { return dadd_set_max_lds(DMA_KERNELS); }

const IgemmKernel* dadd_igemm_dma_row(int tile_m, int tile_n, bool ups, bool persistent, int lnk) {
  return dadd_find_row(DMA_KERNELS, tile_m, tile_n, ups, persistent, lnk);
}
```

### progressive-stable-diffusion_amd/csrc/igemm_epilogue.h

```cpp
#pragma once
#include "igemm_args.h"
#include "ln_lds.h"
#include <type_traits>

__device__ __forceinline__ f4 epi_add_if(bool on, const f4& v, const f4& b) {
#pragma clang fp contract(off)
  const f4 s = v + b;
  return on ? s : v;
}
__device__ __forceinline__ f4 epi_add_if(bool on, const f4& v, const h4& b) {
#pragma clang fp contract(off)
  const f4 s = {v[0] + (float)b[0], v[1] + (float)b[1], v[2] + (float)b[2], v[3] + (float)b[3]};
  return on ? s : v;
}
__device__ __forceinline__ void epi_activate(int flags, f4& v) {
  if (flags & DADD_EPI_QUICKGELU) {
#pragma unroll
    for (int r = 0; r < 4; ++r) v[r] = v[r] / (1.0f + __expf(-1.702f * v[r]));
  } else if (flags & DADD_EPI_GELU) {
#pragma unroll
    for (int r = 0; r < 4; ++r) v[r] = dadd_gelu(v[r]);
  } else {
#pragma unroll
    for (int r = 0; r < 4; ++r) v[r] = 1.0f / (1.0f + __expf(-v[r]));
// ... 51 lines not shown
  __device__ __forceinline__ void load_res(const IgemmArgs& p, int i, int j) {
    res[j][i] = *reinterpret_cast<const h4*>(p.residual + (size_t)mcl[i] * p.ldr + ncl[j]);
  }
  __device__ __forceinline__ void before(const IgemmArgs& p) {
    if constexpr (MODE != EPI_COLS) {
      if (has_c1) {
#pragma unroll
        for (int j = 0; j < J; ++j) c4[j] = *reinterpret_cast<const f4*>(p.ln_c1 + ncl[j]);
      }
      if (has_bias) {
#pragma unroll
        for (int j = 0; j < J; ++j) b4[j] = *reinterpret_cast<const f4*>(p.bias + ncl[j]);
      }
      if (rv_one) {
#pragma unroll
        for (int j = 0; j < J; ++j) r4[j] = *reinterpret_cast<const f4*>(p.rowvec + (size_t)b0 * p.ld_rowvec + ncl[j]);
      }
    }
    if constexpr (MODE == EPI_TILE) {
      if (has_res) {
#pragma unroll
        for (int i = 0; i < MI; ++i)
#pragma unroll
          for (int j = 0; j < J; ++j) load_res(p, i, j);
      }
    }
  }
  __device__ __forceinline__ void batch(const IgemmArgs& p, int o, int HoWo) {
    if constexpr (MODE == EPI_COLS) {
      load_col(p, o);
      if (has_rv && !rv_one) {
#pragma unroll
        for (int i = 0; i < MI; ++i)
          rq[i] = *reinterpret_cast<const f4*>(p.rowvec + (size_t)row_sample(p, mcl[i], HoWo) * p.ld_rowvec + ncl[o]);
      }
      if (has_res) {
#pragma unroll
        for (int i = 0; i < MI; ++i) load_res(p, i, o);
      }
    } else {
      if (has_rv && !rv_one) {
        const float* row = p.rowvec + (size_t)row_sample(p, mcl[o], HoWo) * p.ld_rowvec;
#pragma unroll
        for (int j = 0; j < J; ++j) r4[j] = *reinterpret_cast<const f4*>(row + ncl[j]);
      }
      if constexpr (MODE == EPI_ROWS) {
        if (has_res) {
#pragma unroll
          for (int j = 0; j < J; ++j) load_res(p, o, j);
        }
      }
    }
  }
  __device__ __forceinline__ f4 rowvec(int i, int j) const {
    if constexpr (MODE == EPI_COLS) return rv_one ? r4[j] : rq[i];
    return r4[j];
  }
};

template <int J, int MI, int MODE, class B, class E, class R>
__device__ __forceinline__ void epi_for_each(B&& batch, E&& elem, R&& row_done) {
  constexpr bool COLS = MODE == EPI_COLS;
#pragma unroll
  for (int o = 0; o < (COLS ? J : MI); ++o) {
    batch(o);
#pragma unroll
    for (int q = 0; q < (COLS ? MI : J); ++q) elem(COLS ? q : o, COLS ? o : q);
    if constexpr (!COLS) row_done(o);
  }
  if constexpr (COLS) {
#pragma unroll
    for (int i = 0; i < MI; ++i) row_done(i);
  }
}

__device__ __forceinline__ float dadd_row16_sum(float v) {
  v += __builtin_bit_cast(float, __builtin_amdgcn_update_dpp(0, __builtin_bit_cast(int, v), 0xB1, 0xF, 0xF, true));
  v += __builtin_bit_cast(float, __builtin_amdgcn_update_dpp(0, __builtin_bit_cast(int, v), 0x4E, 0xF, 0xF, true));
  v += __builtin_bit_cast(float, __builtin_amdgcn_update_dpp(0, __builtin_bit_cast(int, v), 0x141, 0xF, 0xF, true));
  v += __builtin_bit_cast(float, __builtin_amdgcn_update_dpp(0, __builtin_bit_cast(int, v), 0x140, 0xF, 0xF, true));
  return v;
}

enum { EPI_PLAIN = 0, EPI_FOLD_GLOBAL = 1, EPI_FOLD_LDS = 2 };
template <int J, int MI, int WM, int WN, int MODE, int FOLD>
__device__ __forceinline__ void epi_tile(const IgemmArgs& p, f4 (&acc)[J][MI], int m0, int n0, int wm, int wn, int g, int mc,
                                         int HoWo, const float (&lmu)[MI], const float (&lrs)[MI], const char* ln_cb) {
  const bool lnstat = FOLD == EPI_PLAIN && (p.flags & DADD_EPI_LNSTAT) != 0 && n0 + wn * WN < p.N;
  EpiOperands<J, MI, MODE> ops;
  ops.init(p, m0 + wm * WM, n0 + wn * WN, mc, g, HoWo, FOLD != EPI_FOLD_LDS, FOLD == EPI_FOLD_GLOBAL);
  ops.before(p);
  float rs1[MI], rs2[MI];
#pragma unroll
  for (int i = 0; i < MI; ++i) rs1[i] = rs2[i] = 0.f;
  epi_for_each<J, MI, MODE>(
      [&](int o) __attribute__((always_inline)) { ops.batch(p, o, HoWo); },
      [&](int i, int j) __attribute__((always_inline)) {
        const int m = m0 + wm * WM + i * 16 + mc;
        const int c = wn * WN + j * 16 + g * 4, n = n0 + c;
        if (m >= p.M || n >= p.N) return;
        f4 v;
        if constexpr (FOLD == EPI_FOLD_LDS) {
          v = lrs[i] * (acc[j][i] - lmu[i] * *reinterpret_cast<const f4*>(ln_cb + c * 4));
          if (p.flags & DADD_EPI_BIAS) v += *reinterpret_cast<const f4*>(ln_cb + 1024 + c * 4);
        } else if constexpr (FOLD == EPI_FOLD_GLOBAL) {
          v = lrs[i] * (acc[j][i] - lmu[i] * ops.c4[j]) + ops.b4[j];
        } else {
          v = epi_add_if(ops.has_bias, acc[j][i], ops.b4[j]);
        }
        v = epi_add_if(ops.has_rv, v, ops.rowvec(i, j));
        if (p.flags & DADD_EPI_ACT_MASK) epi_activate(p.flags, v);
        v = epi_add_if(ops.has_res, v, ops.res[j][i]);
        h4 o;
#pragma unroll
        for (int r = 0; r < 4; ++r) {
          o[r] = (half_t)v[r];
          if constexpr (FOLD == EPI_PLAIN) {
            const float f = (float)o[r];
            rs1[i] += f;
            rs2[i] = fmaf(f, f, rs2[i]);
          }
        }
        *reinterpret_cast<h4*>(p.out + (size_t)m * p.ldo + n) = o;
      },
      [&](int i) __attribute__((always_inline)) {
        const int m = m0 + wm * WM + i * 16 + mc;
        if (lnstat && m < p.M) {
          const float t1 = dadd_sum_x16x32(rs1[i]), t2 = dadd_sum_x16x32(rs2[i]);
          if (g == 0) {
            const int part = (n0 + wn * WN) / WN;
            reinterpret_cast<dadd_f2*>(p.ln_stats_out)[(size_t)part * p.M + m] = dadd_f2{t1, t2};
          }
        }
      });
}

template <int J, int MI, int WM, int WN, int MODE = EPI_TILE>
__device__ __forceinline__ void igemm_epilogue(const IgemmArgs& p, f4 (&acc)[J][MI], int m0, int n0,
                                               int wm, int wn, int lane, int z, char* smem,
                                               const float* ln_mu = nullptr, const float* ln_rs = nullptr,
                                               char* gn_scratch = nullptr, const char* ln_lds = nullptr,
                                               const char* ln_cb = nullptr) {
  const int g = lane >> 4, mc = lane & 15;
  const int HoWo = p.Ho * p.Wo;
  if (p.splitk > 1) {
#pragma unroll
    for (int i = 0; i < MI; ++i) {
      const int m = m0 + wm * WM + i * 16 + mc;
      if (m >= p.M) continue;
#pragma unroll
      for (int j = 0; j < J; ++j) {
        const int n = n0 + wn * WN + j * 16 + g * 4;
        if (n < p.N) *reinterpret_cast<f4*>(p.partial + ((size_t)z * p.M + m) * p.N + n) = acc[j][i];
      }
    }
    if (p.counters == nullptr) return;
    asm volatile("s_waitcnt vmcnt(0)" ::: "memory");
    __syncthreads();
    volatile int* flag = reinterpret_cast<volatile int*>(smem);
    if (threadIdx.x == 0) {
      __builtin_amdgcn_fence(__ATOMIC_RELEASE, "agent");
      asm volatile("s_waitcnt vmcnt(0)" ::: "memory");
      int* ticket = p.counters + blockIdx.x;
      const int prev = __hip_atomic_fetch_add(ticket, 1, __ATOMIC_RELAXED, __HIP_MEMORY_SCOPE_AGENT);
      const int last = (prev == p.splitk - 1) ? 1 : 0;
      if (last) {
        __builtin_amdgcn_fence(__ATOMIC_ACQUIRE, "agent");
        asm volatile("s_waitcnt vmcnt(0)" ::: "memory");
        __hip_atomic_store(ticket, 0, __ATOMIC_RELAXED, __HIP_MEMORY_SCOPE_AGENT);
      }
      *flag = last;
    }
    __syncthreads();
    if (*flag == 0) return;
#pragma unroll
    for (int i = 0; i < MI; ++i) {
      const int m = m0 + wm * WM + i * 16 + mc;
#pragma unroll
      for (int j = 0; j < J; ++j) {
        const int n = n0 + wn * WN + j * 16 + g * 4;
        f4 v = {0.f, 0.f, 0.f, 0.f};
        if (m < p.M && n < p.N)
          for (int s = 0; s < p.splitk; ++s)
            v += *reinterpret_cast<const f4*>(p.partial + ((size_t)s * p.M + m) * p.N + n);
        acc[j][i] = v;
      }
    }
  }
  if (p.flags & DADD_EPI_GNSTAT) {
    float* scratch = reinterpret_cast<float*>(gn_scratch) + (wm * 2 + wn) * 256;
    const int mrow0 = m0 + wm * WM;
    const int bsmp = row_sample(p, mrow0, HoWo);
    const bool has_bias = (p.flags & DADD_EPI_BIAS) != 0, has_rv = (p.flags & DADD_EPI_ROWVEC) != 0;
    const bool has_res = (p.flags & DADD_EPI_RESIDUAL) != 0;
    f4 b4[J], r4[J];
    h4 res[J][MI];
#pragma unroll
    for (int j = 0; j < J; ++j) {
      b4[j] = r4[j] = f4{0.f, 0.f, 0.f, 0.f};
#pragma unroll
      for (int i = 0; i < MI; ++i) res[j][i] = h4{};
    }
    auto load_blocks = [&](int ja, int jb) __attribute__((always_inline)) {
      const int nw = n0 + wn * WN + g * 4;
      if (has_bias) {
#pragma unroll
        for (int j = 0; j < J; ++j)
          if (j >= ja && j < jb) b4[j] = *reinterpret_cast<const f4*>(p.bias + nw + j * 16);
      }
      if (has_rv) {
#pragma unroll
        for (int j = 0; j < J; ++j)
          if (j >= ja && j < jb) r4[j] = *reinterpret_cast<const f4*>(p.rowvec + (size_t)bsmp * p.ld_rowvec + nw + j * 16);
      }
      if (has_res) {
#pragma unroll
        for (int i = 0; i < MI; ++i)
#pragma unroll
          for (int j = 0; j < J; ++j)
            if (j >= ja && j < jb)
              res[j][i] = *reinterpret_cast<const h4*>(p.residual + (size_t)(mrow0 + i * 16 + mc) * p.ldr + nw + j * 16);
      }
    };
    if constexpr (MODE == EPI_TILE) load_blocks(0, J);
#pragma unroll
    for (int j = 0; j < J; ++j) {
      const int n = n0 + wn * WN + j * 16 + g * 4;
      if constexpr (MODE != EPI_TILE) load_blocks(j, j + 1);
      f4 bias4 = {0.f, 0.f, 0.f, 0.f};
      if (has_bias) bias4 = b4[j];
      bias4 = epi_add_if(has_rv, bias4, r4[j]);
      float cs[4] = {0.f, 0.f, 0.f, 0.f}, cq[4] = {0.f, 0.f, 0.f, 0.f};
#pragma unroll
      for (int i = 0; i < MI; ++i) {
        const int m = mrow0 + i * 16 + mc;
        f4 v = acc[j][i] + bias4;
        v = epi_add_if(has_res, v, res[j][i]);
        h4 o;
#pragma unroll
        for (int r = 0; r < 4; ++r) {
          o[r] = (half_t)v[r];
          const float f = (float)o[r];
          cs[r] += f;
          cq[r] = fmaf(f, f, cq[r]);
        }
        *reinterpret_cast<h4*>(p.out + (size_t)m * p.ldo + n) = o;
      }
#pragma unroll
      for (int r = 0; r < 4; ++r) {
        cs[r] = dadd_row16_sum(cs[r]);
        cq[r] = dadd_row16_sum(cq[r]);
      }
      if (mc == 0) {
#pragma unroll
        for (int r = 0; r < 4; ++r) {
          scratch[(j * 16 + g * 4 + r) * 2] = cs[r];
          scratch[(j * 16 + g * 4 + r) * 2 + 1] = cq[r];
        }
      }
    }
    __builtin_amdgcn_fence(__ATOMIC_RELEASE, "wavefront");
    __builtin_amdgcn_wave_barrier();
    __builtin_amdgcn_fence(__ATOMIC_ACQUIRE, "wavefront");
    const int ngrp = WN / p.gn_cg;
    if (lane < ngrp) {
      float a = 0.f, q = 0.f;
      for (int c = 0; c < p.gn_cg; ++c) {
        a += scratch[(lane * p.gn_cg + c) * 2];
        q += scratch[(lane * p.gn_cg + c) * 2 + 1];
      }
      const int chunk = (mrow0 - bsmp * HoWo) / WM;
      const int grp = (n0 + wn * WN) / p.gn_cg + lane;
      float* w = p.gn_ws + (((size_t)bsmp * p.gn_nchunk + chunk) * 32 + grp) * 2;
      w[0] = a;
      w[1] = q;
    }
    return;
  }
  float lmu[MI], lrs[MI];
  bool fold = false;
  if (ln_mu != nullptr) {
#pragma unroll
    for (int i = 0; i < MI; ++i) {
      lmu[i] = ln_mu[i];
      lrs[i] = ln_rs[i];
    }
    fold = true;
  } else if ((p.flags & DADD_EPI_LNFOLD) && p.ln_stats_in != nullptr) {
    const dadd_f2* st = reinterpret_cast<const dadd_f2*>(p.ln_stats_in);
    float sa[MI], sq[MI];
    int mrow[MI];
#pragma unroll
    for (int i = 0; i < MI; ++i) {
      sa[i] = sq[i] = 0.f;
      mrow[i] = min(m0 + wm * WM + i * 16 + mc, p.M - 1);
    }
    if (ln_lds != nullptr) {
      for (int pp = 0; pp < p.ln_parts_in; ++pp)
#pragma unroll
        for (int i = 0; i < MI; ++i) {
          const dadd_f2 v = *reinterpret_cast<const dadd_f2*>(ln_lds + pp * 1024 + (wm * WM + i * 16 + mc) * 8);
          sa[i] += v[0];
          sq[i] += v[1];
        }
    } else
    for (int pp = 0; pp < p.ln_parts_in; pp += 4) {
      dadd_f2 v[4][MI];
#pragma unroll
      for (int u = 0; u < 4; ++u)
#pragma unroll
        for (int i = 0; i < MI; ++i)
          v[u][i] = st[(size_t)min(pp + u, p.ln_parts_in - 1) * p.M + mrow[i]];
#pragma unroll
      for (int u = 0; u < 4; ++u) {
        const float keep = (pp + u < p.ln_parts_in) ? 1.f : 0.f;
#pragma unroll
        for (int i = 0; i < MI; ++i) {
          sa[i] = fmaf(keep, v[u][i][0], sa[i]);
          sq[i] = fmaf(keep, v[u][i][1], sq[i]);
        }
      }
    }
    const float inv = __builtin_amdgcn_rcpf((float)p.K);
#pragma unroll
    for (int i = 0; i < MI; ++i) {
      const float mu = sa[i] * inv;
      lmu[i] = mu;
      lrs[i] = rsqrtf(fmaxf(epi_ln_var(epi_ln_var_fused(J, MI, i), sq[i] * inv, mu), 0.f) + p.ln_eps);
    }
    fold = true;
  } else {
#pragma unroll
    for (int i = 0; i < MI; ++i) lmu[i] = 0.f, lrs[i] = 1.f;
  }
  const bool lds_fold = fold && ln_cb != nullptr;
  if (lds_fold && (p.flags & DADD_EPI_GEGLU)) {
#pragma unroll
    for (int i = 0; i < MI; ++i) {
      const int m = m0 + wm * WM + i * 16 + mc;
      if (m >= p.M) continue;
      if constexpr (J == 4) {
#pragma unroll
        for (int j = 0; j < 2; ++j) {
          const int ch = wn * WN + j * 16 + g * 4, cg2 = ch + 32;
          if (n0 + cg2 >= p.N) continue;
          f4 hv = lrs[i] * (acc[j][i] - lmu[i] * *reinterpret_cast<const f4*>(ln_cb + ch * 4));
          f4 gv = lrs[i] * (acc[j + 2][i] - lmu[i] * *reinterpret_cast<const f4*>(ln_cb + cg2 * 4));
          if (p.flags & DADD_EPI_BIAS) {
            hv += *reinterpret_cast<const f4*>(ln_cb + 1024 + ch * 4);
            gv += *reinterpret_cast<const f4*>(ln_cb + 1024 + cg2 * 4);
          }
          const int no = (n0 >> 1) + wn * 32 + j * 16 + g * 4;
          const dadd_f2 g01 = dadd_gelu2(dadd_f2{gv[0], gv[1]}), g23 = dadd_gelu2(dadd_f2{gv[2], gv[3]});
          const h4 o = {(half_t)(hv[0] * g01[0]), (half_t)(hv[1] * g01[1]), (half_t)(hv[2] * g23[0]),
                        (half_t)(hv[3] * g23[1])};
          *reinterpret_cast<h4*>(p.out + (size_t)m * p.ldo + no) = o;
        }
      }
    }
    return;
  }
  if (p.flags & DADD_EPI_GEGLU) {
    if constexpr (J == 4) {
      const bool has_bias = (p.flags & DADD_EPI_BIAS) != 0;
      auto geglu = [&](auto folded) __attribute__((always_inline)) {
        constexpr bool FOLD = decltype(folded)::value, COLS = MODE == EPI_COLS;
        f4 c1[J], b4[J];
#pragma unroll
        for (int j = 0; j < J; ++j) c1[j] = b4[j] = f4{0.f, 0.f, 0.f, 0.f};
        auto load_pair = [&](int j) __attribute__((always_inline)) {
          const int nh = min(n0 + wn * WN + j * 16 + g * 4, p.N - 4), ng = min(n0 + wn * WN + j * 16 + g * 4 + 32, p.N - 4);
          if constexpr (FOLD) {
            c1[j] = *reinterpret_cast<const f4*>(p.ln_c1 + nh);
            c1[j + 2] = *reinterpret_cast<const f4*>(p.ln_c1 + ng);
          }
          if (has_bias) {
            b4[j] = *reinterpret_cast<const f4*>(p.bias + nh);
            b4[j + 2] = *reinterpret_cast<const f4*>(p.bias + ng);
          }
        };
        if constexpr (!COLS) {
          load_pair(0);
          load_pair(1);
        }
#pragma unroll
        for (int o = 0; o < (COLS ? 2 : MI); ++o) {
          if constexpr (COLS) load_pair(o);
#pragma unroll
          for (int q = 0; q < (COLS ? MI : 2); ++q) {
            const int i = COLS ? q : o, j = COLS ? o : q;
            const int m = m0 + wm * WM + i * 16 + mc;
            if (m >= p.M || n0 + wn * WN + j * 16 + g * 4 + 32 >= p.N) continue;
            f4 hv, gv;
            if constexpr (FOLD) {
              hv = lrs[i] * (acc[j][i] - lmu[i] * c1[j]) + b4[j];
              gv = lrs[i] * (acc[j + 2][i] - lmu[i] * c1[j + 2]) + b4[j + 2];
            } else {
              hv = epi_add_if(has_bias, acc[j][i], b4[j]);
              gv = epi_add_if(has_bias, acc[j + 2][i], b4[j + 2]);
            }
            const int no = (n0 >> 1) + wn * 32 + j * 16 + g * 4;
            const dadd_f2 g01 = dadd_gelu2(dadd_f2{gv[0], gv[1]}), g23 = dadd_gelu2(dadd_f2{gv[2], gv[3]});
            const h4 o4 = {(half_t)(hv[0] * g01[0]), (half_t)(hv[1] * g01[1]), (half_t)(hv[2] * g23[0]),
                           (half_t)(hv[3] * g23[1])};
            *reinterpret_cast<h4*>(p.out + (size_t)m * p.ldo + no) = o4;
          }
        }
      };
      if (fold) geglu(std::true_type{});
      else geglu(std::false_type{});
    }
    return;
  }
  if (lds_fold) epi_tile<J, MI, WM, WN, MODE, EPI_FOLD_LDS>(p, acc, m0, n0, wm, wn, g, mc, HoWo, lmu, lrs, ln_cb);
  else if (fold) epi_tile<J, MI, WM, WN, MODE, EPI_FOLD_GLOBAL>(p, acc, m0, n0, wm, wn, g, mc, HoWo, lmu, lrs, ln_cb);
  else epi_tile<J, MI, WM, WN, MODE, EPI_PLAIN>(p, acc, m0, n0, wm, wn, g, mc, HoWo, lmu, lrs, ln_cb);
}
```

### progressive-stable-diffusion_amd/engine.py

```python
from __future__ import annotations

import math
from typing import Dict, List, Optional, Tuple

import torch

from . import lib as L
from .routing import get_block_type

F16, F32, BF16 = torch.float16, torch.float32, torch.bfloat16
OPERAND_DTYPES = (F16, BF16)
UNET_CH = (320, 640, 1280, 1280)
VAE_CH = (128, 256, 512, 512)
HEADS = 8
GROUPS = 32
N_CU = 256
FUSED_ATTN2 = True
A2_MIN_TILES = 128


def pack_conv(w: torch.Tensor, dtype=F16) -> torch.Tensor:
    if w.dim() == 2:
        return w.to(dtype).contiguous()
    co, ci, kh, kw = w.shape
    return w.permute(0, 2, 3, 1).reshape(co, kh * kw * ci).to(dtype).contiguous()


def pack_conv_cin8(w: torch.Tensor, dtype=F16) -> torch.Tensor:
    co, ci, _, _ = w.shape
    out = torch.zeros(co, 9, 8, dtype=dtype)
    out[:, :, :ci] = w.permute(0, 2, 3, 1).reshape(co, 9, ci).to(dtype)
    return out.contiguous()


def pack_conv_cout4(w: torch.Tensor, dtype=F16) -> torch.Tensor:
    co, ci, _, _ = w.shape
    return w.permute(0, 2, 3, 1).reshape(co, 9, ci).to(dtype).contiguous()


def geglu_interleave(w: torch.Tensor, b: torch.Tensor) -> Tuple[torch.Tensor, torch.Tensor]:
    n2 = w.shape[0] // 2
    idx = torch.arange(w.shape[0])
    tile, r = idx // 128, idx % 128
    wn, rr = r // 64, r % 64
    col = tile * 64 + wn * 32 + (rr % 32)
    src = torch.where(rr < 32, col, n2 + col)
    return w[src].contiguous(), b[src].contiguous()


def fold_layernorm(w: torch.Tensor, b: Optional[torch.Tensor], gamma: torch.Tensor, beta: torch.Tensor, dtype=F16):
    w, gamma, beta = w.double(), gamma.double(), beta.double()
    w16 = (w * gamma[None, :]).to(dtype)
    bias = w @ beta + (b.double() if b is not None else 0.0)
    return w16, w16.double().sum(dim=1).float(), bias.float()


def lds_image(w: torch.Tensor) -> torch.Tensor:
    r = w.shape[0]
    sw = (torch.arange(r) >> 1) & 7
    idx = (torch.arange(8)[None, :] ^ sw[:, None])
    return w.reshape(r, 8, 8).gather(1, idx[:, :, None].expand(r, 8, 8)).reshape(r, 64).contiguous()


def pack_ffn_stream(w1: torch.Tensor, b1: torch.Tensor, w2: torch.Tensor, wp: torch.Tensor):
    c, hid = 320, 1280
    assert tuple(w1.shape) == (2 * hid, c) and tuple(w2.shape) == (c, hid) and tuple(wp.shape)[:2] == (c, c)
    w1, w2, wp = w1.to(F16), w2.to(F16), wp.reshape(c, c).to(F16)
    pieces, bias = [], []
    e = torch.arange(16)
    for ch in range(hid // 64):
        rows = []
        for wn in range(2):
            for u in range(2):
                h = ch * 64 + wn * 32 + u * 16 + e
                rows += [h, hid + h]
                bias += [b1[h].float(), b1[hid + h].float()]
        rows = torch.cat(rows)
        for kt in range(c // 64):
            pieces.append(lds_image(w1[rows][:, kt * 64:(kt + 1) * 64]))
        for nh in range(2):
            pieces.append(lds_image(w2[nh * 160:(nh + 1) * 160, ch * 64:(ch + 1) * 64]))
    for nh in range(2):
        for kt in range(c // 64):
            pieces.append(lds_image(wp[nh * 160:(nh + 1) * 160, kt * 64:(kt + 1) * 64]))
    return torch.cat([p.reshape(-1) for p in pieces]).contiguous(), torch.cat(bias).contiguous()


def pack_head_stream(wp: torch.Tensor, wq: torch.Tensor, wk: torch.Tensor, wv: torch.Tensor) -> torch.Tensor:
    c = 320
    wp = wp.reshape(c, c).to(F16)
    wqkv = torch.cat([wq, wk, wv]).to(F16)
    assert tuple(wqkv.shape) == (3 * c, c)
    pieces = []
    for w in (wp, wqkv):
        for nh in range(w.shape[0] // 160):
            for kt in range(c // 64):
                pieces.append(lds_image(w[nh * 160:(nh + 1) * 160, kt * 64:(kt + 1) * 64]))
    return torch.cat([p.reshape(-1) for p in pieces]).contiguous()


GN_IN_CONV = True

HALO_DUO = False

FINISH_GN_APPLY = True

WEIGHT_PREFETCH_AHEAD = 0
WEIGHT_PREFETCH_MIN_BYTES = 2 * 1024 * 1024

GN_FROM_EPILOGUE = True
GN_FUSED_MAX_BYTES = 16 * 1024
SPLITK_GN_ROWS = 16


LN_FOLD = "auto"
LN_STATS_FROM_PRODUCER = True
LN_STATS_MAX_PARTS = 8


FUSED_FFN = True
FFN_MIN_BLOCKS = 128
FUSED_HEAD = True


def fold_here(m: int, n: int, k: int, geglu: bool = False) -> bool:
    if LN_FOLD == "auto":
        tile_m, _, _, tune = plan_tiling(m, n, k, 1, geglu, False)
        return tile_m == 64 and not (tune & L.TUNE_NODMA)
    return bool(LN_FOLD)


def choose_tiling(m: int, n: int, k: int, tile_n: int, geglu: bool = False,
                  residual: bool = True) -> Tuple[int, int, int]:
    nkt = k // 64
    nt = math.ceil(n / tile_n)
    t128 = math.ceil(m / 128) * nt
    if geglu:
        if m >= 16384:
            return 64, 1, L.TUNE_NODMA | L.TUNE_SHALLOW
        return 128, 1, (L.TUNE_PERSIST if t128 >= 4 * N_CU else 0)
    if nkt >= 12:
        if n <= 128 and nkt <= 18:
            return 128, 1, L.TUNE_NODMA
        per = 16 if t128 > 64 else (10 if t128 > 16 else 8)
        sk = max(1, min(round(N_CU / t128), nkt // per, 32))
        if not residual and nkt <= 20:
            sk = 1
        return 128, sk, (L.TUNE_PERSIST if sk == 1 and t128 >= 8 * N_CU else 0)
    if t128 > N_CU:
        return 128, 1, L.TUNE_PERSIST
    if not residual and nkt >= 5:
        return 128, 1, 0
    return (128 if t128 >= 2 * N_CU else 64), 1, L.TUNE_NODMA


def choose_splitk(m: int, n: int, k: int, tile_n: int) -> int:
    return choose_tiling(m, n, k, tile_n)[1]


TILING_OVERRIDE: Dict[Tuple, Tuple[int, int, int, int]] = {}
try:
    from .tiling_table import TABLE as TILING_TABLE, TABLE_R3 as TILING_TABLE_R3
except ImportError:
    TILING_TABLE, TILING_TABLE_R3 = {}, {}
TILING_R3 = True


def tiling_key(m, n, k, taps, geglu, residual, ups=0, stride=1):
    return (int(m), int(n), int(k), int(taps), bool(geglu), bool(residual), int(bool(ups)), int(stride))


def plan_tiling(m, n, k, taps, geglu, residual, ups=0, stride=1) -> Tuple[int, int, int, int]:
    key = tiling_key(m, n, k, taps, geglu, residual, ups, stride)
    hit = TILING_OVERRIDE.get(key) or (TILING_TABLE_R3.get(key) if TILING_R3 else None) or TILING_TABLE.get(key)
    if hit is not None:
        return tuple(hit)
    tile_n = 128 if geglu or n % 160 else 160
    tile_m, sk, tune = choose_tiling(m, n, k, tile_n, geglu, residual)
    if (taps == 1 and not geglu and not ups and n % 64 == 0 and k // 64 <= 40
            and math.ceil(m / 128) * math.ceil(n / tile_n) <= N_CU // 2):
        return 64, 64, 1, 0
    return tile_m, tile_n, sk, tune


class Pool:

    def __init__(self, be, dtype=F16):
        self.be = be
        self.dtype = dtype
        self.free: Dict[Tuple, List[torch.Tensor]] = {}
        self.bytes = 0
        self.on_put = None

    def get(self, shape, dtype=None) -> torch.Tensor:
        dtype = dtype or self.dtype
        key = (tuple(shape), dtype)
        lst = self.free.get(key)
# ... 9 lines not shown
                if self.on_put is not None:
                    self.on_put(t)
                self.free.setdefault((tuple(t.shape), t.dtype), []).append(t)


class _Plan:
    def __init__(self, be, wcache=None, dtype=F16, sd=None, prefix=""):
        if dtype not in OPERAND_DTYPES:
            raise ValueError(f"plan dtype must be torch.float16 or torch.bfloat16, got {dtype}")
        self.be = be
        self.wcache = wcache
        self.dtype = dtype
        self.sd, self.prefix = sd, prefix + "."
        self.pool = Pool(be, dtype)
        self.ops: List = []
        self.keep: List[torch.Tensor] = []
        self.gn_partials: Dict[int, Tuple[torch.Tensor, int]] = {}
        self.ln_partials: Dict[int, torch.Tensor] = {}
        self._memo: Dict = {}
        self.gn_ready: Dict[int, Tuple] = {}
        self.pool.on_put = self._forget
        self.gn_ws = None
        self.sk_counters = None

    def rec(self, fn, *a, **k):
        self.ops.append((fn, a, k))

    def run(self):
        for fn, a, k in self.ops:
            fn(*a, **k)

    def _forget(self, t):
        assert t.data_ptr() not in self.gn_ready, f"GroupNorm of a {tuple(t.shape)} buffer written by a finish kernel, never consumed"
        self.gn_partials.pop(t.data_ptr(), None)
        self.ln_partials.pop(t.data_ptr(), None)

    def _end_build(self, prefetch_weights=False):
        assert not self.gn_ready, f"GroupNorm written by a finish kernel, never consumed: {[tuple(r[0].shape) for r in self.gn_ready.values()]}"
        if prefetch_weights:
            self._insert_weight_prefetch()

    def _insert_weight_prefetch(self):
        if not WEIGHT_PREFETCH_AHEAD:
            return
        wops = []
        for i, (fn, a, k) in enumerate(self.ops):
            name = getattr(fn, "__name__", "")
            if name == "igemm":
                wops.append((i, a[1]))
            elif name in ("ffn_block", "tf_head"):
                wops.append((i, a[1]))
        inserts = []
        for j, (i, w) in enumerate(wops):
            if w.numel() * w.element_size() < WEIGHT_PREFETCH_MIN_BYTES or j < WEIGHT_PREFETCH_AHEAD:
                continue
            inserts.append((wops[j - WEIGHT_PREFETCH_AHEAD][0], w))
        for at, w in sorted(inserts, key=lambda t: -t[0]):
            self.ops.insert(at, (self.be.prefetch, (w,), {}))
        if inserts:
            self.ops.append((self.be.prefetch_join, (), {}))

    def dev(self, t, dtype=None):
        d = self.be.to_device(t, dtype)
        self.keep.append(d)
        return d

    def cached(self, key, make):
        key = (*key, self.dtype)
        t = self._memo.get(key)
        if t is None:
            t = self.wcache.get(key) if self.wcache is not None else None
            if t is None:
                t = make()
                if self.wcache is not None:
                    self.wcache[key] = t
            self._memo[key] = t
            self.keep += t if isinstance(t, tuple) else (t,)
        return t

    def w(self, key, pack=pack_conv):
        return self.cached((self.prefix + key, pack.__name__),
                           lambda: self.be.to_device(pack(self.sd[self.prefix + key], self.dtype)))

    def f(self, key):
        return self.cached((self.prefix + key, "f32"), lambda: self.be.to_device(self.sd[self.prefix + key].float()))

    def _gn_partials_for(self, out, nchunk, extra=0):
        ws = self.be.zeros((out.shape[0] * (nchunk + extra) * GROUPS * 2,), F32)
        self.keep.append(ws)
        self.gn_partials[out.data_ptr()] = (ws, nchunk)
        return dict(gn_ws=ws, gn_nchunk=nchunk)

    def _ln_partials_for(self, out, parts):
        st = self.be.zeros((parts, out.numel() // out.shape[-1], 2), F32)
        self.keep.append(st)
        self.ln_partials[out.data_ptr()] = st
        return st

    def conv(self, x, w, out_shape, *, x2=None, bias=None, rowvec=None, residual=None, taps=9,
             stride=1, ups=0, pad=1, flags=0, ln_c1=None, ln_eps=1e-5, gn_stats=False, ln_stats=False,
             ln_stats_in=None, gn_in=None, fuse_gn=None):
        out = self.pool.get(out_shape)
        n = w.shape[0]
        m = out_shape[0] * out_shape[1] * out_shape[2]
        tile_m, tile_n, sk, tune = plan_tiling(m, n, w.shape[1], taps, bool(flags & L.EPI_GEGLU), residual is not None,
                                               ups, stride)
        if taps == 9 and HALO_DUO:
            tune |= L.TUNE_SHALLOW
        if ln_c1 is not None:
            sk = 1
        partial = self.pool.get((sk * m * n,), F32) if sk > 1 else None
        gkw = {}
        if gn_stats and GN_FROM_EPILOGUE and not (flags & L.EPI_GEGLU) and n % 32 == 0:
            howo, cg = out_shape[1] * out_shape[2], n // 32
            if sk == 1:
                wm_rows = tile_m // 2
                ok = tile_n in (128, 160) and (tile_n // 2) % cg == 0 and m % tile_m == 0 and n % tile_n == 0
            else:
                wm_rows = SPLITK_GN_ROWS if howo // SPLITK_GN_ROWS <= 128 else 64
                cb = 160 if n % 160 == 0 else 128
                ok = n % cb == 0 and cb % cg == 0 and m % wm_rows == 0
            nchunk = howo // wm_rows
            if ok and howo % wm_rows == 0 and nchunk >= 1 and howo * cg * 2 > GN_FUSED_MAX_BYTES:
                gkw = self._gn_partials_for(out, nchunk, extra=64 if nchunk > 128 else 0)
                flags |= L.EPI_GNSTAT
        if (ln_stats and LN_STATS_FROM_PRODUCER and not (flags & (L.EPI_GEGLU | L.EPI_GNSTAT)) and sk == 1
                and n % (tile_n // 2) == 0 and n // (tile_n // 2) <= LN_STATS_MAX_PARTS):
            gkw["ln_stats_out"] = self._ln_partials_for(out, n // (tile_n // 2))
            flags |= L.EPI_LNSTAT
        f = flags | (L.EPI_BIAS if bias is not None else 0) | (L.EPI_ROWVEC if rowvec is not None else 0) \
            | (L.EPI_RESIDUAL if residual is not None else 0) | (L.EPI_LNFOLD if ln_c1 is not None else 0) | tune
        kw = dict(ln_c1=ln_c1, ln_eps=ln_eps) if ln_c1 is not None else {}
        if (fuse_gn is not None and FINISH_GN_APPLY and sk > 1 and self.sk_counters is None and not (f & L.EPI_GNSTAT)
                and n % 64 == 0 and out_shape[1] * out_shape[2] * (n // 32) * 2 <= GN_FUSED_MAX_BYTES):
            g_out = self.pool.get(out_shape)
            f |= L.EPI_GNAPPLY | (L.EPI_GNAPPLY_SILU if fuse_gn[3] else 0)
            kw["gn_apply"] = (g_out, fuse_gn[0], fuse_gn[1], fuse_gn[2])
            self.gn_ready[out.data_ptr()] = (g_out, fuse_gn[0].data_ptr(), fuse_gn[1].data_ptr(), float(fuse_gn[2]), bool(fuse_gn[3]))
        if gn_in is not None:
            f |= L.PRE_GN | (L.PRE_GN_SILU if gn_in[5] else 0)
            kw["gn_in"] = tuple(gn_in[:5]) + tuple(gn_in[6:])
        if ln_c1 is not None and ln_stats_in is not None:
            kw["ln_stats_in"] = ln_stats_in
        self.rec(self.be.igemm, x, w, out, x2=x2, bias=bias, rowvec=rowvec, residual=residual,
                 taps=taps, stride=stride, ups=ups, pad=pad, flags=f, splitk=sk, partial=partial,
                 tile_n=tile_n, tile_m=tile_m, counters=self.sk_counters if sk > 1 else None, **kw, **gkw)
        self.pool.put(partial)
        return out

    def gn_in_conv_ok(self, x, x2, w, out_shape, residual) -> Optional[Tuple]:
        cmax = {64: 1152, 32: 2048, 16: 2432}.get(x.shape[2], 0)
        cin = x.shape[-1] + (0 if x2 is None else x2.shape[-1])
        if not GN_IN_CONV or cin > cmax or x.shape[-1] % 64 or cin % 64:
            return None
        part = self.gn_partials.get(x.data_ptr())
        if part is None or part[1] > 128:
            return None
        if x2 is not None:
            part2 = self.gn_partials.get(x2.data_ptr())
            c1_, c2_, cgc = x.shape[-1], x2.shape[-1], cin // 32
            if (part2 is None or part2[1] > 128 or c1_ % 32 or c2_ % 32 or cgc % (c1_ // 32) or cgc % (c2_ // 32)
                    or c1_ % cgc):
                return None
            part = (part[0], part[1], part2[0], part2[1])
        b, h, w_, _ = x.shape
        n, m = w.shape[0], out_shape[0] * out_shape[1] * out_shape[2]
        if tuple(out_shape[1:3]) != (h, w_) or h != w_ or w_ not in (16, 32, 64) or (h * w_) % 128:
            return None
        tile_m, tile_n, _, tune = plan_tiling(m, n, w.shape[1], 9, False, residual is not None, 0, 1)
        if tile_m != 128 or tile_n != 160 or (tune & (L.TUNE_NODMA | L.TUNE_PERSIST)) or HALO_DUO:
            return None
        return part

    def gn(self, x1, x2, gamma, beta, eps, silu):
        c = x1.shape[-1] + (0 if x2 is None else x2.shape[-1])
        ready = self.gn_ready.get(x1.data_ptr()) if x2 is None else None
        if ready is not None and ready[1:] == (gamma.data_ptr(), beta.data_ptr(), float(eps), bool(silu)):
            del self.gn_ready[x1.data_ptr()]
            return ready[0]
        out = self.pool.get((*x1.shape[:3], c))
        part = self.gn_partials.get(x1.data_ptr()) if x2 is None else None
        if part is not None:
            self.rec(self.be.groupnorm, x1, None, gamma, beta, out, part[0], GROUPS, eps, silu, ws_chunks=part[1])
        else:
            self.rec(self.be.groupnorm, x1, x2, gamma, beta, out, self.gn_ws, GROUPS, eps, silu)
        return out


class UNetPlan(_Plan):
# ... 671 lines not shown
```

### progressive-stable-diffusion_amd/lib.py

```python
from __future__ import annotations

import ctypes as C
import os
import subprocess
from typing import Optional

_HERE = os.path.dirname(os.path.abspath(__file__))
LIB_PATH = os.path.join(_HERE, "libdadd_hip.so")
CSRC = os.path.join(_HERE, "csrc")
_SINGLE_SOURCES = ("attn2_fused", "ffn_block", "tf_head", "conditioning", "api",
                   "optim")
_TWINNED_SOURCES = (
    "igemm", "igemm_dma", "conv_halo", "norm", "attention", "elementwise",
    "wgrad",
    "norm_grad",
    "attn_grad",
    "dgrad",
    "end_grad",
    "cond_grad",
    "rows_grad",
    "relayout")
SOURCES = tuple(s + ".hip" for s in _SINGLE_SOURCES) + tuple(s + sfx for s in _TWINNED_SOURCES for sfx in (".hip", "_bf16.hip"))

DADD_OK, DADD_EINVAL, DADD_EHIP, DADD_ESTATE = 0, -1, -2, -3
EPI_BIAS, EPI_ROWVEC, EPI_RESIDUAL, EPI_GEGLU = 1, 2, 4, 8
EPI_LNFOLD, EPI_QUICKGELU, EPI_GELU, EPI_SIGMOID, EPI_GNSTAT, EPI_LNSTAT = 128, 256, 512, 1024, 2048, 4096
PRE_GN, PRE_GN_SILU = 8192, 16384
EPI_GNAPPLY, EPI_GNAPPLY_SILU = 32768, 65536
TUNE_SHALLOW, TUNE_NODMA, TUNE_PERSIST = 16, 32, 64
XATTN_SPLIT, XATTN_BASELINE = 0, 1
DGRAD_STRIDE2, DGRAD_UPS = 0, 1
END_WGRAD_IN, END_WGRAD_OUT = 0, 1
GN_MAX_CHUNKS = 256

vp, i32, i64, f32 = C.c_void_p, C.c_int32, C.c_int64, C.c_float


class IgemmDesc(C.Structure):
    _fields_ = [(n, vp) for n in ("x", "x2", "w", "out", "partial", "bias", "rowvec", "residual")] + \
               [(n, i32) for n in ("B", "Hi", "Wi", "C1", "C2", "Ho", "Wo", "N", "taps", "stride",
                                   "ups", "pad", "ldo", "ldr", "ld_rowvec", "splitk", "flags",
                                   "tile_n", "tile_m")] + [("counters", vp), ("ln_c1", vp), ("ln_eps", f32), ("gn_ws", vp), ("gn_nchunk", i32), ("gn_cg", i32),
                                                           ("ln_stats_out", vp), ("ln_stats_in", vp), ("ln_parts_out", i32), ("ln_parts_in", i32),
                                                           ("gn_in_ws", vp), ("gn_in_gamma", vp), ("gn_in_beta", vp), ("gn_in_nchunk", i32), ("gn_in_eps", f32),
                                                           ("gn_in_ws2", vp), ("gn_in_nchunk2", i32),
                                                           ("gn_out", vp), ("gn_out_gamma", vp), ("gn_out_beta", vp), ("gn_out_eps", f32)]


class IgemmChoice(C.Structure):
    _fields_ = [("kernel", C.c_char_p), ("finish", C.c_char_p)] + \
               [(n, i32) for n in ("tile_m", "tile_n", "nsplit", "kps", "persistent", "grid_x", "grid_y", "block", "smem",
                                   "gm", "gn")]


class WgradDesc(C.Structure):
    _fields_ = [(n, vp) for n in ("dy", "x", "dw", "dbias", "partial")] + \
               [(n, i32) for n in ("B", "Hi", "Wi", "C", "Ho", "Wo", "N", "taps", "stride", "ups", "pad",
                                   "ld_dy", "ld_x", "ld_dw", "ld_tap", "splitm")]


class DgradDesc(C.Structure):
    _fields_ = [(n, vp) for n in ("dy", "wt", "dx")] + \
               [(n, i32) for n in ("B", "Hi", "Wi", "C", "Ho", "Wo", "N", "mode", "ld_dy", "ld_dx")]


class DgradClass(C.Structure):
    _fields_ = [(n, i32) for n in ("first_tile", "pixels", "py", "px", "first_slab", "ntaps")]


class DgradChoice(C.Structure):
    _fields_ = [(n, i32) for n in ("grid_x", "grid_y", "block", "smem", "nclass", "xcd_by_c")] + [("cls", DgradClass * 4)]


class EndWgradDesc(C.Structure):
    _fields_ = [(n, vp) for n in ("thin", "wide", "dw", "dbias", "partial")] + \
               [(n, i32) for n in ("B", "H", "W", "Ct", "Cw", "ld_wide", "mode", "splitm")]


class GnGradDesc(C.Structure):
    _fields_ = [(n, vp) for n in ("x1", "x2", "dy", "gamma", "beta", "dx1", "dx2", "dgamma", "dbeta", "ws")] + \
               [(n, i32) for n in ("B", "HW", "C1", "C2", "groups", "silu")] + [("eps", f32)]


class AttnGradDesc(C.Structure):
    _fields_ = [(n, vp) for n in ("q", "k", "v", "dout", "dq", "dk", "dv", "ws", "do_scale_dev")] + \
               [(n, i64) for n in ("bs_q", "bs_kv", "bs_do", "bs_dq", "bs_dkv")] + \
               [(n, i32) for n in ("B", "Nq", "Nk", "heads", "d", "ld_q", "ld_kv", "ld_do", "ld_dq", "ld_dkv")] + \
               [("do_scale", f32)]


def _with_bf16(table, stems=None):
    out = {}
    for name, proto in table.items():
        out[name] = proto
        if name.endswith("_f16") and (stems is None or name[:-len("_f16")] in stems):
            out[name[:-len("_f16")] + "_bf16"] = proto
    return out


PROTOTYPES = _with_bf16({
    "dadd_last_error": (C.c_char_p, []),
    "dadd_version": (C.c_int, []),
    "dadd_init": (C.c_int, []),
    "dadd_device_info": (C.c_int, [C.c_int, C.POINTER(i64)]),
    "dadd_conv_igemm_f16": (C.c_int, [C.POINTER(IgemmDesc), vp]),
    "dadd_conv_igemm_resolve_f16": (C.c_int, [C.POINTER(IgemmDesc), C.c_int, C.POINTER(IgemmChoice)]),
    "dadd_conv3x3_cin8_f16": (C.c_int, [vp, vp, vp, vp, C.c_int, C.c_int, C.c_int, C.c_int, vp]),
    "dadd_conv_in_nchw_f16": (C.c_int, [vp, vp, vp, vp, C.c_int, C.c_int, C.c_int, C.c_int, C.c_int, vp, C.c_int, vp]),
    "dadd_conv3x3_cout4_f16": (C.c_int, [vp, vp, vp, vp, C.c_int, C.c_int, C.c_int, C.c_int, C.c_int,
                                         C.c_int, vp]),
    "dadd_conv_out_ddim_f16": (C.c_int, [vp, vp, vp, vp, vp, C.c_int, C.c_int, C.c_int, C.c_int, C.c_int, vp]),
    "dadd_pack_nchw_f32_to_nhwc8_f16": (C.c_int, [vp, vp, C.c_int, C.c_int, C.c_int, C.c_int, f32, vp,
                                                  vp, vp]),
    "dadd_q_sample_f32": (C.c_int, [vp, vp, vp, vp, vp, C.c_int, i64, vp]),
    "dadd_mse_rows_f32": (C.c_int, [vp, vp, vp, C.c_int, i64, vp]),
    "dadd_frames_to_u8": (C.c_int, [vp, vp, C.c_int, C.c_int, C.c_int, vp]),
    "dadd_gaussian_sample_f32": (C.c_int, [vp, vp, vp, f32, vp, i64, vp]),
    "dadd_groupnorm_f16": (C.c_int, [vp, C.c_int, vp, C.c_int, vp, vp, vp, vp, C.c_int, C.c_int,
                                     C.c_int, f32, C.c_int, C.c_int, vp]),
    "dadd_layernorm_f16": (C.c_int, [vp, vp, vp, vp, C.c_int, C.c_int, f32, vp]),
    "dadd_self_attn_f16": (C.c_int, [vp, vp, vp, vp, C.c_int, C.c_int, C.c_int, C.c_int, C.c_int,
                                     C.c_int, vp]),
    "dadd_attn2_fused_f16": (C.c_int, [vp, vp, vp, vp, vp, vp, vp, vp, C.c_int, vp, vp, f32, C.c_int, C.c_int, C.c_int, vp]),
    "dadd_ffn_block_f16": (C.c_int, [vp, vp, vp, vp, f32, vp, vp, vp, vp, vp, vp, C.c_int, C.c_int, C.c_int, C.c_int, vp]),
    "dadd_ffn_block_bytes": (C.c_int, []),
    "dadd_tf_head_f16": (C.c_int, [vp, vp, vp, C.c_int, vp, vp, f32, vp, vp, vp, f32, vp, vp, C.c_int, C.c_int, C.c_int, vp]),
    "dadd_tf_head_bytes": (C.c_int, []),
    "dadd_tf_head_debug": (C.c_int, [vp]),
    "dadd_tri_xattn_f16": (C.c_int, [vp, vp, vp, vp, f32, vp, C.c_int, C.c_int, C.c_int, C.c_int, C.c_int,
# ... 172 lines not shown
```

Baseline: 11.54 images/sec.

## Fold nearest-upsample into 3x3 conv as four 2x2 phase convolutions

Nearest-2x-upsample followed by a 3x3 conv is rewritten as four sub-pixel phases, each a 2x2 conv on the low-resolution input with pre-summed weights. A new kernel variant runs over low-res rows, one phase per tile, and scatters outputs to the interleaved high-res positions, with the GN-stat epilogue adapted to match. This cuts the GEMM K from 9*Cin to 4*Cin for the UNet upsample convs and drops the upsample gather. The cost is four times the weight storage and reads, a second kernel instantiation, and fp16 rounding of the summed weights.

```diff
diff --git a/include/dadd_hip.h b/include/dadd_hip.h
--- a/include/dadd_hip.h
+++ b/include/dadd_hip.h
@@ -30,6 +30,7 @@
 #define DADD_TUNE_SHALLOW 16
 #define DADD_TUNE_NODMA 32
 #define DADD_TUNE_PERSIST 64
+#define DADD_TUNE_UPS_FOLD 131072
 
 #define DADD_XATTN_SPLIT 0
 #define DADD_XATTN_BASELINE 1
@@ -72,6 +73,7 @@
   const float* gn_out_gamma;
   const float* gn_out_beta;
   float gn_out_eps;
+  const void* w_fold;
 } dadd_igemm_desc;
 int dadd_conv_igemm_f16(const dadd_igemm_desc* d, void* stream);
 
diff --git a/progressive-stable-diffusion_amd/backend.py b/progressive-stable-diffusion_amd/backend.py
--- a/progressive-stable-diffusion_amd/backend.py
+++ b/progressive-stable-diffusion_amd/backend.py
@@ -28,7 +28,8 @@
 
 def fill_igemm_desc(d, ptr, x, w, out, *, x2=None, bias=None, rowvec=None, residual=None, taps=1, stride=1,
                     ups=0, pad=0, flags=0, splitk=1, partial=None, tile_n=0, tile_m=0, counters=None, ln_c1=None,
-                    ln_eps=1e-5, gn_ws=None, gn_nchunk=0, ln_stats_out=None, ln_stats_in=None, gn_in=None, gn_apply=None):
+                    ln_eps=1e-5, gn_ws=None, gn_nchunk=0, ln_stats_out=None, ln_stats_in=None, gn_in=None, gn_apply=None,
+                    w_fold=None):
     b, hi, wi, c1 = x.shape
     c2 = 0 if x2 is None else x2.shape[-1]
     n = w.shape[0]
@@ -80,6 +81,10 @@
         d.gn_out, d.gn_out_gamma, d.gn_out_beta, d.gn_out_eps = ptr(g_out), ptr(gam), ptr(bet), float(eps_o)
     if partial is not None:
         assert partial.numel() >= splitk * b * ho * wo * n
+    d.w_fold = ptr(w_fold)
+    if w_fold is not None:
+        assert ups and taps == 9 and tuple(w_fold.shape) == (4, n, 4 * (c1 + c2)) and w_fold.dtype == w.dtype \
+            and w_fold.is_contiguous()
 
 
 class HipBackend:
@@ -97,6 +102,7 @@
         self._edesc = L.EndWgradDesc()
         self._gdesc = L.GnGradDesc()
         self._adesc = L.AttnGradDesc()
+        self._ups_folds = {}
         self._n_cu = None
         self._capturing = False
         self._prof_on = False
@@ -231,15 +237,23 @@
         L.check(self.lib.dadd_gaussian_sample_f32(_p(mean), _p(logvar), _p(noise), float(scale), _p(out),
                                                   mean.numel(), self.s))
 
+    def register_ups_fold(self, w9, w4):
+        if tuple(w4.shape) != (4, w9.shape[0], w9.shape[1] // 9 * 4) or w4.dtype != w9.dtype or not w4.is_contiguous() \
+                or w4.device != w9.device:
+            raise ValueError(f"register_ups_fold: w4 must be [4][N][4 Cin] of w9's type, got {tuple(w4.shape)} for {tuple(w9.shape)}")
+        self._ups_folds[w9.data_ptr()] = (w9, w4)
+
     def igemm(self, x, w, out, *, x2=None, bias=None, rowvec=None, residual=None, taps=1, stride=1,
               ups=0, pad=0, flags=0, splitk=1, partial=None, tile_n=0, tile_m=0, counters=None, ln_c1=None,
               ln_eps=1e-5, gn_ws=None, gn_nchunk=0, ln_stats_out=None, ln_stats_in=None, gn_in=None, gn_apply=None):
         fn = getattr(self.lib, "dadd_conv_igemm_" + _sfx(x, x2, w, out, residual, None if gn_apply is None else gn_apply[0]))
         d = self._desc
+        fold = self._ups_folds.get(w.data_ptr()) if (flags & L.TUNE_UPS_FOLD) and ups else None
         fill_igemm_desc(d, _p, x, w, out, x2=x2, bias=bias, rowvec=rowvec, residual=residual, taps=taps, stride=stride,
                         ups=ups, pad=pad, flags=flags, splitk=splitk, partial=partial, tile_n=tile_n, tile_m=tile_m,
                         counters=counters, ln_c1=ln_c1, ln_eps=ln_eps, gn_ws=gn_ws, gn_nchunk=gn_nchunk,
-                        ln_stats_out=ln_stats_out, ln_stats_in=ln_stats_in, gn_in=gn_in, gn_apply=gn_apply)
+                        ln_stats_out=ln_stats_out, ln_stats_in=ln_stats_in, gn_in=gn_in, gn_apply=gn_apply,
+                        w_fold=None if fold is None else fold[1])
         L.check(fn(C.byref(d), self.s))
 
     def wgrad_splitm(self, m, n, c, taps=1):
diff --git a/progressive-stable-diffusion_amd/csrc/bf16_names.h b/progressive-stable-diffusion_amd/csrc/bf16_names.h
--- a/progressive-stable-diffusion_amd/csrc/bf16_names.h
+++ b/progressive-stable-diffusion_amd/csrc/bf16_names.h
@@ -9,6 +9,7 @@
 #define splitk_finish_gn_kernel splitk_finish_gn_kernel_bf16
 #define splitk_finish_gnapply_kernel splitk_finish_gnapply_kernel_bf16
 #define igemm_dma_kernel igemm_dma_kernel_bf16
+#define igemm_ups_fold_kernel igemm_ups_fold_kernel_bf16
 #define conv3x3_halo_kernel conv3x3_halo_kernel_bf16
 #define gn_stats_kernel gn_stats_kernel_bf16
 #define gn_apply_kernel gn_apply_kernel_bf16
@@ -46,6 +47,8 @@
 #define dadd_init_igemm dadd_init_igemm_bf16
 #define dadd_init_igemm_dma dadd_init_igemm_dma_bf16
 #define dadd_igemm_dma_row dadd_igemm_dma_row_bf16
+#define dadd_init_igemm_ups_fold dadd_init_igemm_ups_fold_bf16
+#define dadd_igemm_ups_fold_row dadd_igemm_ups_fold_row_bf16
 #define dadd_igemm_resolve dadd_igemm_resolve_bf16
 #define dadd_init_conv_halo dadd_init_conv_halo_bf16
 #define dadd_conv_halo_applicable dadd_conv_halo_applicable_bf16
diff --git a/progressive-stable-diffusion_amd/csrc/igemm.hip b/progressive-stable-diffusion_amd/csrc/igemm.hip
--- a/progressive-stable-diffusion_amd/csrc/igemm.hip
+++ b/progressive-stable-diffusion_amd/csrc/igemm.hip
@@ -404,6 +404,7 @@
 
 int dadd_init_igemm() {
   int rc = dadd_init_igemm_dma();
+  if (rc == DADD_OK) rc = dadd_init_igemm_ups_fold();
   if (rc == DADD_OK) rc = dadd_init_conv_halo();
   if (rc == DADD_OK) rc = dadd_set_max_lds(REG_KERNELS);
   int dev = 0;
@@ -427,7 +428,7 @@
   a.counters = d->counters;
   a.B = d->B; a.Hi = d->Hi; a.Wi = d->Wi; a.C1 = d->C1; a.C2 = d->C2;
   a.Ho = d->Ho; a.Wo = d->Wo; a.N = d->N;
-  a.taps = d->taps; a.stride = d->stride; a.ups = d->ups; a.pad = d->pad;
+  a.taps = d->taps; a.stride = d->stride; a.ups = d->ups ? 1 : 0; a.pad = d->pad;
   a.flags = d->flags & (15 | DADD_TUNE_PERSIST | DADD_EPI_LNFOLD | DADD_EPI_ACT_MASK | DADD_EPI_GNSTAT | DADD_EPI_LNSTAT |
                         DADD_PRE_GN | DADD_PRE_GN_SILU | DADD_EPI_GNAPPLY | DADD_EPI_GNAPPLY_SILU);
   a.gno_out = static_cast<half_t*>(d->gn_out);
@@ -483,6 +484,20 @@
 
   a.M = a.B * a.Ho * a.Wo;
   a.K = a.taps * Cin;
+  if ((d->flags & DADD_TUNE_UPS_FOLD) && d->w_fold != nullptr && a.ups) {
+    DADD_REQUIRE(a.C2 == 0 && !geglu && !(a.flags & (DADD_EPI_ROWVEC | DADD_EPI_RESIDUAL | DADD_EPI_LNSTAT | DADD_EPI_GNAPPLY)),
+                 "igemm: the folded upsample conv takes one source and a bias / activation / GNSTAT epilogue "
+                 "(no x2, rowvec, residual, GEGLU, LNSTAT, GNAPPLY)");
+    DADD_REQUIRE(dadd_aligned16(d->w_fold), "igemm: pointers must be 16-byte aligned");
+    const long long rows = (long long)a.B * a.Hi * a.Wi;
+    if (d->splitk <= 1 && (d->tile_m == 0 || d->tile_m == 128) && !(d->flags & DADD_TUNE_NODMA) && a.pad == 1 &&
+        a.Ho == 2 * a.Hi && a.Wo == 2 * a.Wi && rows % 128 == 0 &&
+        (!(a.flags & DADD_EPI_GNSTAT) || (a.Hi * a.Wi) % 64 == 0) && (size_t)a.N * 4 * Cin * 2 * 4 < 0x7FF00000ull) {
+      a.ups = 2;
+      a.w = static_cast<const half_t*>(d->w_fold);
+      a.K = 4 * Cin;
+    }
+  }
   a.nkt = a.K / BK;
   int tile_n = d->tile_n;
   if (geglu) {
@@ -537,8 +552,8 @@
             (size_t)a.mtiles * a.ntiles < DADD_FASTDIV_MAX;
   a.plain = a.taps == 1 && a.stride == 1 && a.pad == 0 && !a.ups && a.Ho == a.Hi && a.Wo == a.Wi;
   if (a.fd_on) {
-    a.fd_howo = dadd_fastdiv_make((uint32_t)(a.Ho * a.Wo));
-    a.fd_wo = dadd_fastdiv_make((uint32_t)a.Wo);
+    a.fd_howo = dadd_fastdiv_make((uint32_t)(a.ups == 2 ? a.Hi * a.Wi : a.Ho * a.Wo));
+    a.fd_wo = dadd_fastdiv_make((uint32_t)(a.ups == 2 ? a.Wi : a.Wo));
     a.fd_cin = dadd_fastdiv_make((uint32_t)Cin);
     a.ngn = 1;
     a.fd_t1 = a.fd_t2 = dadd_fastdiv_make(1);
@@ -622,7 +637,7 @@
   out->tile_n = tile_n;
   out->persistent = !halo && persistent;
   out->grid = out->persistent ? dim3(num_cu) : dim3(a.mtiles * a.ntiles, out->nsplit);
-  a.pf_kt = (dma && !halo && a.korder == 0 && !out->persistent && a.mtiles >= DADD_PF_MIN_SHARE)
+  a.pf_kt = (dma && !halo && a.korder == 0 && !out->persistent && (a.ups == 2 ? a.mtiles / 4 : a.mtiles) >= DADD_PF_MIN_SHARE)
                 ? (a.kps < DADD_PF_KTILES ? a.kps : DADD_PF_KTILES) : 0;
   if (halo) {
     DADD_REQUIRE(window, "conv_halo: operand larger than the 2 GiB buffer window");
@@ -633,7 +648,8 @@
     DADD_REQUIRE(window, "igemm(dma): operand larger than the 2 GiB buffer window");
     DADD_REQUIRE(tile_m == 128 || !a.ups, "igemm(dma): the 64-row tiles have no upsample gather");
     const int lnk = (a.ups || !(a.flags & DADD_EPI_LNFOLD)) ? 0 : (a.ln_stats_in == nullptr ? 1 : (tile_m == 128 ? 2 : 0));
-    out->main = dadd_igemm_dma_row(tile_m, tile_n, !out->persistent && tile_m == 128 && a.ups, out->persistent, lnk);
+    out->main = a.ups == 2 ? dadd_igemm_ups_fold_row(tile_m, tile_n)
+                           : dadd_igemm_dma_row(tile_m, tile_n, !out->persistent && tile_m == 128 && a.ups, out->persistent, lnk);
   } else {
     out->main = dadd_find_row(REG_KERNELS, tile_m, tile_n, deep && !(tile_m == 128 && tile_n == 160));
   }
diff --git a/progressive-stable-diffusion_amd/csrc/igemm_args.h b/progressive-stable-diffusion_amd/csrc/igemm_args.h
--- a/progressive-stable-diffusion_amd/csrc/igemm_args.h
+++ b/progressive-stable-diffusion_amd/csrc/igemm_args.h
@@ -76,6 +76,14 @@
   ox = rem - oy * p.Wo;
 }
 
+__device__ __forceinline__ void ups_fold_decode(const IgemmArgs& p, int r, int& b, int& y, int& x) {
+  const int HiWi = p.Hi * p.Wi;
+  b = p.fd_on ? (int)dadd_fastdiv_div((uint32_t)r, p.fd_howo) : r / HiWi;
+  const int rem = r - b * HiWi;
+  y = p.fd_on ? (int)dadd_fastdiv_div((uint32_t)rem, p.fd_wo) : rem / p.Wi;
+  x = rem - y * p.Wi;
+}
+
 __device__ __forceinline__ int xcd_remap(int bid, int nwg) {
   const int q = nwg >> 3, r = nwg & 7, xcd = bid & 7, slot = bid >> 3;
   return (xcd < r ? xcd * (q + 1) : r * (q + 1) + (xcd - r) * q) + slot;
@@ -138,7 +146,7 @@
 static inline double dadd_igemm_flop(const IgemmArgs& a) { return 2.0 * (double)a.M * (double)a.N * (double)a.K; }
 static inline double dadd_igemm_bytes(const IgemmArgs& a) {
   const double n_out = (a.flags & DADD_EPI_GEGLU) ? a.N / 2 : a.N;
-  return 2.0 * ((double)a.B * a.Hi * a.Wi * (a.C1 + a.C2) + (double)a.N * a.K + (double)a.M * n_out +
+  return 2.0 * ((double)a.B * a.Hi * a.Wi * (a.C1 + a.C2) + (double)a.N * a.K * (a.ups == 2 ? 4.0 : 1.0) + (double)a.M * n_out +
                 ((a.flags & DADD_EPI_RESIDUAL) ? (double)a.M * a.N : 0.0));
 }
 
@@ -202,6 +210,8 @@
 
 int dadd_init_igemm_dma();
 const IgemmKernel* dadd_igemm_dma_row(int tile_m, int tile_n, bool ups, bool persistent, int lnk);
+int dadd_init_igemm_ups_fold();
+const IgemmKernel* dadd_igemm_ups_fold_row(int tile_m, int tile_n);
 int dadd_init_conv_halo();
 bool dadd_conv_halo_applicable(const IgemmArgs& a, int tile_n);
 int dadd_conv_halo_gn_channels(int Wo);
diff --git a/progressive-stable-diffusion_amd/csrc/igemm_dma.hip b/progressive-stable-diffusion_amd/csrc/igemm_dma.hip
--- a/progressive-stable-diffusion_amd/csrc/igemm_dma.hip
+++ b/progressive-stable-diffusion_amd/csrc/igemm_dma.hip
@@ -1,360 +1,6 @@
-#include "dadd_common.h"
-#include "igemm_args.h"
-#include <cstdlib>
-#include "igemm_epilogue.h"
+#include "igemm_dma_kernel.h"
 
 namespace {
-
-constexpr int BK = 64;
-
-typedef __attribute__((address_space(3))) void* lptr_t;
-constexpr unsigned OOB = 0x80000000u;
-
-__device__ __forceinline__ int lds_off(int row, int chunk) {
-  return (row * 8 + (chunk ^ ((row >> 1) & 7))) * 8;
-}
-
-template <int N>
-__device__ __forceinline__ void wait_vmcnt() {
-  asm volatile("s_waitcnt vmcnt(%0)" ::"n"(N) : "memory");
-}
-
-template <int BM, int BN, bool UPS, bool PERS, int LNK>
-__global__ __launch_bounds__(512, (BM + BN) <= 128 ? 4 : 2) void igemm_dma_kernel(const IgemmArgs p) {
-#if defined(__HIP_DEVICE_COMPILE__)
-  constexpr bool WS = true;
-  constexpr bool LNF = LNK == 1;
-  constexpr int WM = BM / 2, MI = WM / 16;
-  constexpr int WN = BN / 2;
-  constexpr int J = WN / 16;
-  constexpr int EPI = !PERS ? EPI_TILE : (BN == 160 && LNK == 2) ? EPI_COLS : EPI_ROWS;
-  constexpr int NA = BM / 32;
-  constexpr int NBJ = BN / 32;
-  constexpr int LPT = NA + NBJ;
-  constexpr int A_BYTES = BM * BK * 2, B_BYTES = BN * BK * 2, STAGE = A_BYTES + B_BYTES;
-  extern __shared__ __attribute__((aligned(1024))) char smem[];
-
-  const int t = threadIdx.x, lane = t & 63;
-  const int wave_all = __builtin_amdgcn_readfirstlane(t >> 6);
-  const bool loader = WS && wave_all >= 4;
-  const int wave = WS ? (wave_all & 3) : wave_all;
-  const int wm = wave >> 1, wn = wave & 1;
-  int tile_first, tile_count;
-  if constexpr (PERS) {
-    const int total = p.mtiles * p.ntiles, nwg = gridDim.x;
-    const int l = xcd_remap(blockIdx.x, nwg);
-    const int q = total / nwg, r = total - q * nwg;
-    tile_first = l * q + min(l, r);
-    tile_count = q + (l < r ? 1 : 0);
-  } else {
-    tile_first = xcd_remap(blockIdx.x, gridDim.x);
-    tile_count = 1;
-  }
-  const int z = PERS ? 0 : blockIdx.y;
-  const int kt0 = PERS ? 0 : z * p.kps;
-  const int kt1 = PERS ? p.nkt : min(p.nkt, kt0 + p.kps);
-  const int nk = kt1 - kt0;
-  const int Cin = p.C1 + p.C2;
-  const int Hv = UPS ? 2 * p.Hi : p.Hi;
-  const int Wv = UPS ? 2 * p.Wi : p.Wi;
-  const int HoWo = p.Ho * p.Wo;
-  const int lrow = lane >> 3, lch = lane & 7;
-
-  const int shift1 = UPS ? 0 : (p.pad * p.Wi + p.pad) * p.C1;
-  const int shift2 = UPS ? 0 : (p.pad * p.Wi + p.pad) * p.C2;
-  const size_t pix_total = (size_t)p.B * p.Hi * p.Wi;
-  const int rec1 = (int)((pix_total * p.C1 + shift1) * 2);
-  const int rec2 = (int)((pix_total * p.C2 + shift2) * 2);
-  const int recW = (int)((size_t)p.N * p.K * 2);
-  const half_t* base1 = p.x - shift1;
-  const half_t* base2 = (p.x2 ? p.x2 : p.x) - shift2;
-
-  unsigned a_v1[NA], a_v2[NA], a_mask[NA];
-  int a_pix[NA], a_y[NA], a_x[NA], a_cc[NA];
-  unsigned w_v[NBJ];
-  auto setup_tile = [&](int tile_id) __attribute__((always_inline)) {
-  int nt, mt;
-  tile_decode_fast(p, tile_id, mt, nt);
-  const int m0 = mt * BM, n0 = nt * BN;
-#pragma unroll
-  for (int i = 0; i < NA; ++i) {
-    const int row = (i * 4 + wave) * 8 + lrow;
-    const int m = m0 + row;
-    const bool ok = m < p.M;
-    const int mm = ok ? m : 0;
-    const int cc = (lch ^ ((row >> 1) & 7)) * 8;
-    if (!UPS && p.plain) {
-      a_v1[i] = (unsigned)((mm * p.C1 + cc) * 2);
-      a_v2[i] = (unsigned)((mm * p.C2 + cc) * 2);
-      a_mask[i] = ok ? 1u : 0u;
-      continue;
-    }
-    int b, oy, ox;
-    row_decode(p, mm, HoWo, b, oy, ox);
-    const int pix = b * p.Hi * p.Wi;
-    const int y0 = oy * p.stride - p.pad, x0 = ox * p.stride - p.pad;
-    a_pix[i] = pix; a_y[i] = ok ? y0 : -100000; a_x[i] = x0; a_cc[i] = cc;
-    const int org = pix + oy * p.stride * p.Wi + ox * p.stride;
-    a_v1[i] = (unsigned)((org * p.C1 + cc) * 2);
-    a_v2[i] = (unsigned)((org * p.C2 + cc) * 2);
-    unsigned my = 0, mx = 0;
-#pragma unroll
-    for (int k3 = 0; k3 < 3; ++k3) {
-      my |= (y0 + k3 >= 0 && y0 + k3 < Hv) ? 1u << k3 : 0u;
-      mx |= (x0 + k3 >= 0 && x0 + k3 < Wv) ? 1u << k3 : 0u;
-    }
-    const unsigned mask9 = ((my & 1u) ? mx : 0u) | ((my & 2u) ? mx << 3 : 0u) | ((my & 4u) ? mx << 6 : 0u);
-    a_mask[i] = ok ? (p.taps == 9 ? mask9 : (my & mx & 1u)) : 0u;
-  }
-#pragma unroll
-  for (int j = 0; j < NBJ; ++j) {
-    const int row = (j * 4 + wave) * 8 + lrow;
-    const int n = n0 + row;
-    w_v[j] = (n < p.N) ? (unsigned)(((size_t)n * p.K + (lch ^ ((row >> 1) & 7)) * 8) * 2) : OOB;
-  }
-  };
-  int iss_tile = tile_first, iss_left = tile_count;
-
-  const bool tapfast = p.korder != 0;
-  int cur_kt = kt0;
-  int cur_tap = 0, cur_c = 0, cur_koff = 0, cur_ky = 0, cur_kx = 0;
-  auto cursor_init = [&]() {
-    if (kt0 == 0) return;
-    const int tap0 = p.fd_on ? (int)dadd_fastdiv_div((uint32_t)(kt0 * BK), p.fd_cin) : (kt0 * BK) / Cin;
-    cur_tap = __builtin_amdgcn_readfirstlane(tapfast ? kt0 % 9 : tap0);
-    cur_c = __builtin_amdgcn_readfirstlane(tapfast ? (kt0 / 9) * BK : kt0 * BK - cur_tap * Cin);
-    cur_koff = __builtin_amdgcn_readfirstlane((cur_tap * Cin + cur_c) * 2);
-    cur_ky = (p.taps == 9) ? cur_tap / 3 : 0;
-    cur_kx = (p.taps == 9) ? cur_tap - 3 * cur_ky : 0;
-  };
-  int fill_off = wave * 1024;
-
-  struct IssueCtx {
-    __amdgpu_buffer_rsrc_t rsA, rsW;
-    unsigned soff, koff;
-    char* sa;
-    int cs, cb, ky, kx, tap;
-    bool second;
-  };
-  auto issue_begin = [&]() {
-    IssueCtx c;
-    const bool live = PERS ? iss_left > 0 : cur_kt < kt1;
-    c.second = cur_c >= p.C1;
-    c.cs = c.second ? p.C2 : p.C1;
-    c.cb = c.second ? cur_c - p.C1 : cur_c;
-    c.ky = cur_ky; c.kx = cur_kx; c.tap = cur_tap;
-    c.rsA = __builtin_amdgcn_make_buffer_rsrc((void*)(c.second ? base2 : base1), 0,
-                                              live ? (c.second ? rec2 : rec1) : 0, 0x00020000);
-    c.rsW = __builtin_amdgcn_make_buffer_rsrc((void*)p.w, 0, live ? recW : 0, 0x00020000);
-    c.sa = smem + fill_off;
-    c.soff = UPS ? (unsigned)(c.cb * 2) : (unsigned)(((cur_ky * p.Wi + cur_kx) * c.cs + c.cb) * 2);
-    c.koff = (unsigned)cur_koff;
-    return c;
-  };
-  auto issue_w = [&](const IssueCtx& c, int j) {
-    __builtin_amdgcn_raw_ptr_buffer_load_lds(c.rsW, (lptr_t)(c.sa + A_BYTES + j * 4096), 16, w_v[j], c.koff, 0, 0);
-  };
-  auto issue_advance = [&]() {
-    ++cur_kt;
-    const int c1 = cur_c + BK;
-    const int cwrap = c1 >= Cin ? 1 : 0;
-    const int kx1 = cur_kx + (tapfast ? 1 : cwrap);
-    const int w3 = kx1 == 3 ? 1 : 0;
-    cur_kx = w3 ? 0 : kx1;
-    const int ky1 = cur_ky + w3;
-    const int w9 = (tapfast && ky1 == 3) ? 1 : 0;
-    cur_ky = w9 ? 0 : ky1;
-    cur_koff += tapfast ? (w9 ? (BK - 8 * Cin) * 2 : Cin * 2) : BK * 2;
-    cur_tap = tapfast ? (w9 ? 0 : cur_tap + 1) : cur_tap + cwrap;
-    cur_c = tapfast ? cur_c + (w9 ? BK : 0) : (cwrap ? 0 : c1);
-    const int f1 = fill_off + STAGE;
-    fill_off = f1 >= 4 * STAGE ? f1 - 4 * STAGE : f1;
-    if constexpr (PERS) {
-      if (cur_kt == kt1) {
-        cur_kt = 0; cur_c = 0; cur_tap = 0; cur_ky = 0; cur_kx = 0; cur_koff = 0;
-        ++iss_tile;
-        --iss_left;
-        if (iss_left > 0) setup_tile(iss_tile);
-      }
-    }
-  };
-  unsigned a_eff[NA];
-  int eff_key = -1;
-  auto issue = [&]() {
-    const IssueCtx c = issue_begin();
-    {
-      const int key = c.tap * 2 + (c.second ? 1 : 0) + (PERS ? iss_tile * 32 : 0);
-      if (key != eff_key) {
-        eff_key = key;
-#pragma unroll
-        for (int i = 0; i < NA; ++i) {
-          if constexpr (!UPS) {
-            a_eff[i] = ((a_mask[i] >> c.tap) & 1u) ? (c.second ? a_v2[i] : a_v1[i]) : OOB;
-          } else {
-            const int iy = a_y[i] + c.ky, ix = a_x[i] + c.kx;
-            const bool ok = (iy >= 0) & (iy < Hv) & (ix >= 0) & (ix < Wv);
-            a_eff[i] = ok ? (unsigned)(((a_pix[i] + (iy >> 1) * p.Wi + (ix >> 1)) * c.cs + a_cc[i]) * 2) : OOB;
-          }
-        }
-      }
-#pragma unroll
-      for (int i = 0; i < NA; ++i)
-        __builtin_amdgcn_raw_ptr_buffer_load_lds(c.rsA, (lptr_t)(c.sa + i * 4096), 16, a_eff[i], c.soff, 0, 0);
-#pragma unroll
-      for (int jj = 0; jj < NBJ; ++jj) issue_w(c, jj);
-    }
-    issue_advance();
-  };
-
-  const int total_kt = tile_count * nk;
-  char* const ln_scr = smem + 4 * STAGE;
-  const bool ln_stage = LNK == 2 && !UPS && ln_lds_usable(p, BM, nk);
-  const bool ln_sts = ln_stage && ln_lds_stats(p, LN_LDS_BYTES);
-  if (loader) {
-    const int ln_extra = ln_stage ? ln_lds_count(p, wave, ln_sts) : 0;
-    cursor_init();
-    setup_tile(tile_first);
-    issue();
-    issue();
-    issue();
-    wait_vmcnt<LPT>();
-    __builtin_amdgcn_s_barrier();
-    bool ext_young = false;
-    int kc = 0, ext_tile = tile_first;
-    for (int it = 0; it < total_kt; ++it) {
-      if (it > 0) {
-        if (ext_young) {
-          switch (ln_extra) {
-            case 1: wait_vmcnt<LPT + 1>(); break;
-            case 2: wait_vmcnt<LPT + 2>(); break;
-            case 3: wait_vmcnt<LPT + 3>(); break;
-            case 4: wait_vmcnt<LPT + 4>(); break;
-            default: wait_vmcnt<LPT>(); break;
-          }
-          ext_young = false;
-        } else {
-          wait_vmcnt<LPT>();
-        }
-        __builtin_amdgcn_s_barrier();
-      }
-      issue();
-      if (ln_stage) {
-        if (kc == 0) {
-          int nt, mt;
-          tile_decode_fast(p, ext_tile, mt, nt);
-          ln_lds_issue<BN>(p, ln_scr, __builtin_amdgcn_readfirstlane(mt) * BM, __builtin_amdgcn_readfirstlane(nt) * BN, wave,
-                           lane, ln_sts);
-          ext_young = ln_extra > 0;
-          ++ext_tile;
-        }
-        kc = kc + 1 == nk ? 0 : kc + 1;
-      }
-    }
-    wait_vmcnt<0>();
-    return;
-  }
-  f4 acc[J][MI];
-  const int fq = lane >> 4;
-  int fa[2], fb[2];
-#pragma unroll
-  for (int s2 = 0; s2 < 2; ++s2) {
-    fa[s2] = lds_off(wm * WM + (lane & 15), s2 * 4 + fq) * 2;
-    fb[s2] = A_BYTES + lds_off(wn * WN + (lane & 15), s2 * 4 + fq) * 2;
-  }
-  unsigned pf_sink = 0;
-  if (!PERS && p.pf_kt > 0) {
-    int nt, mt;
-    tile_decode_fast(p, tile_first, mt, nt);
-    mt = __builtin_amdgcn_readfirstlane(mt);
-    const int n0 = __builtin_amdgcn_readfirstlane(nt) * BN;
-    const dadd_u4 dw = dadd_pf_desc(p.w, recW);
-    const unsigned row_bytes = (unsigned)p.K * 2u;
-    const int total = BN * min(nk, p.pf_kt);
-    for (int q0 = wave * 64; q0 * p.mtiles + mt < total; q0 += 256) {
-      const int l = (q0 + lane) * p.mtiles + mt;
-      const int kt = l / BN, n = n0 + l - kt * BN;
-      const unsigned off = (l < total && n < p.N) ? (unsigned)n * row_bytes + (unsigned)((kt0 + kt) * BK * 2) : OOB;
-      dadd_pf_line(pf_sink, off, dw);
-    }
-  }
-  __builtin_amdgcn_s_barrier();
-  __builtin_amdgcn_sched_barrier(0);
-  h8 xa0[MI], wb0[J], xa1[MI], wb1[J];
-#pragma unroll
-  for (int i = 0; i < MI; ++i) xa0[i] = *reinterpret_cast<const h8*>(smem + fa[0] + i * 2048);
-#pragma unroll
-  for (int j = 0; j < J; ++j) wb0[j] = *reinterpret_cast<const h8*>(smem + fb[0] + j * 2048);
-  int comp_off = 0;
-  bool started = false;
-  for (int tl = 0; tl < tile_count; ++tl) {
-#pragma unroll
-    for (int j = 0; j < J; ++j)
-#pragma unroll
-      for (int i = 0; i < MI; ++i) acc[j][i] = f4{0.f, 0.f, 0.f, 0.f};
-    [[maybe_unused]] float ls1[MI], ls2[MI];
-    constexpr int LQ = MI * 4, LPER = (LQ + MI * J - 1) / (MI * J);
-    if constexpr (LNF) {
-#pragma unroll
-      for (int i = 0; i < MI; ++i) ls1[i] = ls2[i] = 0.f;
-    }
-    for (int it = 0; it < nk; ++it) {
-      if (started) __builtin_amdgcn_s_barrier();
-      started = true;
-      __builtin_amdgcn_sched_barrier(0);
-      const int n1 = comp_off + STAGE;
-      const int next_off = n1 >= 4 * STAGE ? 0 : n1;
-      const char* ca = smem + comp_off + fa[1];
-      const char* cb1 = smem + comp_off + fb[1];
-      const char* na = smem + next_off + fa[0];
-      const char* nb = smem + next_off + fb[0];
-#pragma unroll
-      for (int k = 0; k < MI * J; ++k) {
-        const int jj = k / MI, ii = k % MI;
-        acc[jj][ii] = DADD_MFMA_16X16X32(wb0[jj], xa0[ii], acc[jj][ii], 0, 0, 0);
-        if constexpr (LNF) {
-#pragma unroll
-          for (int t2 = 0; t2 < LPER; ++t2)
-            if (k * LPER + t2 < LQ) ln_acc_pair(xa0[(k * LPER + t2) / 4], (k * LPER + t2) % 4, ls1[(k * LPER + t2) / 4], ls2[(k * LPER + t2) / 4]);
-        }
-        if (k == 0) wb1[0] = *reinterpret_cast<const h8*>(cb1);
-        else if (k <= MI) xa1[k - 1] = *reinterpret_cast<const h8*>(ca + (k - 1) * 2048);
-        else if (k < MI + J) wb1[k - MI] = *reinterpret_cast<const h8*>(cb1 + (k - MI) * 2048);
-        __builtin_amdgcn_sched_barrier(0);
-      }
-#pragma unroll
-      for (int k = 0; k < MI * J; ++k) {
-        const int jj = k / MI, ii = k % MI;
-        acc[jj][ii] = DADD_MFMA_16X16X32(wb1[jj], xa1[ii], acc[jj][ii], 0, 0, 0);
-        if constexpr (LNF) {
-#pragma unroll
-          for (int t2 = 0; t2 < LPER; ++t2)
-            if (k * LPER + t2 < LQ) ln_acc_pair(xa1[(k * LPER + t2) / 4], (k * LPER + t2) % 4, ls1[(k * LPER + t2) / 4], ls2[(k * LPER + t2) / 4]);
-        }
-        if (k == 0) wb0[0] = *reinterpret_cast<const h8*>(nb);
-        else if (k <= MI) xa0[k - 1] = *reinterpret_cast<const h8*>(na + (k - 1) * 2048);
-        else if (k < MI + J) wb0[k - MI] = *reinterpret_cast<const h8*>(nb + (k - MI) * 2048);
-        __builtin_amdgcn_sched_barrier(0);
-      }
-      comp_off = next_off;
-      __builtin_amdgcn_sched_barrier(0);
-    }
-    dadd_pf_drain(pf_sink);
-    int nt, mt;
-    tile_decode_fast(p, tile_first + tl, mt, nt);
-    if constexpr (LNF) {
-      ln_finish<MI>(ls1, ls2, p.K, p.ln_eps);
-      igemm_epilogue<J, MI, WM, WN, EPI>(p, acc, mt * BM, nt * BN, wm, wn, lane, z, smem, ls1, ls2);
-    } else {
-      igemm_epilogue<J, MI, WM, WN, EPI>(p, acc, mt * BM, nt * BN, wm, wn, lane, z, smem, nullptr, nullptr, smem + 4 * STAGE,
-                                    ln_sts ? ln_scr + LN_LDS_STATS : nullptr, ln_stage ? ln_scr : nullptr);
-    }
-  }
-#endif
-}
-
-constexpr int smem_bytes(int bm, int bn) {
-  return 4 * (bm + bn) * BK * 2 + (bm == 128 ? LN_LDS_BYTES : 4096);
-}
 
 #define DMA_ROW(BM, BN, UPS, PERS, LNK)                                                                                \
   {DADD_KNAME("igemm_dma_kernel") "<" #BM ", " #BN ", " #UPS ", " #PERS ", " #LNK ">", igemm_dma_kernel<BM, BN, UPS, PERS, LNK>, \
diff --git a/progressive-stable-diffusion_amd/csrc/igemm_dma_kernel.h b/progressive-stable-diffusion_amd/csrc/igemm_dma_kernel.h
--- /dev/null
+++ b/progressive-stable-diffusion_amd/csrc/igemm_dma_kernel.h
@@ -0,0 +1,391 @@
+#pragma once
+#include "dadd_common.h"
+#include "igemm_args.h"
+#include <cstdlib>
+#include "igemm_epilogue.h"
+
+namespace {
+
+constexpr int BK = 64;
+
+typedef __attribute__((address_space(3))) void* lptr_t;
+constexpr unsigned OOB = 0x80000000u;
+
+__device__ __forceinline__ int lds_off(int row, int chunk) {
+  return (row * 8 + (chunk ^ ((row >> 1) & 7))) * 8;
+}
+
+template <int N>
+__device__ __forceinline__ void wait_vmcnt() {
+  asm volatile("s_waitcnt vmcnt(%0)" ::"n"(N) : "memory");
+}
+
+#ifdef DADD_IGEMM_UPS_FOLD
+template <int BM, int BN>
+__global__ __launch_bounds__(512, 2) void igemm_ups_fold_kernel(const IgemmArgs p) {
+  constexpr int UPS = 2, LNK = 0;
+  constexpr bool PERS = false;
+#else
+template <int BM, int BN, bool UPS_GATHER, bool PERS, int LNK>
+__global__ __launch_bounds__(512, (BM + BN) <= 128 ? 4 : 2) void igemm_dma_kernel(const IgemmArgs p) {
+  constexpr int UPS = UPS_GATHER ? 1 : 0;
+#endif
+#if defined(__HIP_DEVICE_COMPILE__)
+  constexpr bool WS = true;
+  constexpr bool GATHER = UPS == 1, FOLD = UPS == 2;
+  constexpr bool LNF = LNK == 1;
+  constexpr int WM = BM / 2, MI = WM / 16;
+  constexpr int WN = BN / 2;
+  constexpr int J = WN / 16;
+  constexpr int EPI = !PERS ? EPI_TILE : (BN == 160 && LNK == 2) ? EPI_COLS : EPI_ROWS;
+  constexpr int NA = BM / 32;
+  constexpr int NBJ = BN / 32;
+  constexpr int LPT = NA + NBJ;
+  constexpr int A_BYTES = BM * BK * 2, B_BYTES = BN * BK * 2, STAGE = A_BYTES + B_BYTES;
+  extern __shared__ __attribute__((aligned(1024))) char smem[];
+
+  const int t = threadIdx.x, lane = t & 63;
+  const int wave_all = __builtin_amdgcn_readfirstlane(t >> 6);
+  const bool loader = WS && wave_all >= 4;
+  const int wave = WS ? (wave_all & 3) : wave_all;
+  const int wm = wave >> 1, wn = wave & 1;
+  int tile_first, tile_count;
+  if constexpr (PERS) {
+    const int total = p.mtiles * p.ntiles, nwg = gridDim.x;
+    const int l = xcd_remap(blockIdx.x, nwg);
+    const int q = total / nwg, r = total - q * nwg;
+    tile_first = l * q + min(l, r);
+    tile_count = q + (l < r ? 1 : 0);
+  } else {
+    tile_first = xcd_remap(blockIdx.x, gridDim.x);
+    tile_count = 1;
+  }
+  const int z = PERS ? 0 : blockIdx.y;
+  const int kt0 = PERS ? 0 : z * p.kps;
+  const int kt1 = PERS ? p.nkt : min(p.nkt, kt0 + p.kps);
+  const int nk = kt1 - kt0;
+  const int Cin = p.C1 + p.C2;
+  const int Hv = GATHER ? 2 * p.Hi : p.Hi;
+  const int Wv = GATHER ? 2 * p.Wi : p.Wi;
+  const int HoWo = p.Ho * p.Wo;
+  const int lrow = lane >> 3, lch = lane & 7;
+
+  const int shift1 = GATHER ? 0 : (p.pad * p.Wi + p.pad) * p.C1;
+  const int shift2 = GATHER ? 0 : (p.pad * p.Wi + p.pad) * p.C2;
+  const size_t pix_total = (size_t)p.B * p.Hi * p.Wi;
+  const int rec1 = (int)((pix_total * p.C1 + shift1) * 2);
+  const int rec2 = (int)((pix_total * p.C2 + shift2) * 2);
+  const int recW = (int)((size_t)p.N * p.K * 2) * (FOLD ? 4 : 1);
+  const half_t* base1 = p.x - shift1;
+  const half_t* base2 = (p.x2 ? p.x2 : p.x) - shift2;
+
+  unsigned a_v1[NA], a_v2[NA], a_mask[NA];
+  int a_pix[NA], a_y[NA], a_x[NA], a_cc[NA];
+  unsigned w_v[NBJ];
+  auto setup_tile = [&](int tile_id) __attribute__((always_inline)) {
+  int nt, mt;
+  tile_decode_fast(p, tile_id, mt, nt);
+  const int m0 = mt * BM, n0 = nt * BN;
+#pragma unroll
+  for (int i = 0; i < NA; ++i) {
+    const int row = (i * 4 + wave) * 8 + lrow;
+    const int m = m0 + row;
+    const bool ok = m < p.M;
+    const int mm = ok ? m : 0;
+    const int cc = (lch ^ ((row >> 1) & 7)) * 8;
+    if constexpr (FOLD) {
+      const int py = (mt >> 1) & 1, px = mt & 1;
+      int b, y, x;
+      ups_fold_decode(p, (mt >> 2) * BM + row, b, y, x);
+      const int org = (b * p.Hi + y + py) * p.Wi + x + px;
+      a_v1[i] = (unsigned)((org * p.C1 + cc) * 2);
+      a_v2[i] = (unsigned)((org * p.C2 + cc) * 2);
+      const int y0 = y + py - 1, x0 = x + px - 1;
+      const unsigned my = (y0 >= 0 ? 1u : 0u) | (y0 + 1 < p.Hi ? 2u : 0u), mx = (x0 >= 0 ? 1u : 0u) | (x0 + 1 < p.Wi ? 2u : 0u);
+      a_mask[i] = ((my & 1u) ? mx : 0u) | ((my & 2u) ? mx << 2 : 0u);
+      continue;
+    }
+    if (UPS == 0 && p.plain) {
+      a_v1[i] = (unsigned)((mm * p.C1 + cc) * 2);
+      a_v2[i] = (unsigned)((mm * p.C2 + cc) * 2);
+      a_mask[i] = ok ? 1u : 0u;
+      continue;
+    }
+    int b, oy, ox;
+    row_decode(p, mm, HoWo, b, oy, ox);
+    const int pix = b * p.Hi * p.Wi;
+    const int y0 = oy * p.stride - p.pad, x0 = ox * p.stride - p.pad;
+    a_pix[i] = pix; a_y[i] = ok ? y0 : -100000; a_x[i] = x0; a_cc[i] = cc;
+    const int org = pix + oy * p.stride * p.Wi + ox * p.stride;
+    a_v1[i] = (unsigned)((org * p.C1 + cc) * 2);
+    a_v2[i] = (unsigned)((org * p.C2 + cc) * 2);
+    unsigned my = 0, mx = 0;
+#pragma unroll
+    for (int k3 = 0; k3 < 3; ++k3) {
+      my |= (y0 + k3 >= 0 && y0 + k3 < Hv) ? 1u << k3 : 0u;
+      mx |= (x0 + k3 >= 0 && x0 + k3 < Wv) ? 1u << k3 : 0u;
+    }
+    const unsigned mask9 = ((my & 1u) ? mx : 0u) | ((my & 2u) ? mx << 3 : 0u) | ((my & 4u) ? mx << 6 : 0u);
+    a_mask[i] = ok ? (p.taps == 9 ? mask9 : (my & mx & 1u)) : 0u;
+  }
+#pragma unroll
+  for (int j = 0; j < NBJ; ++j) {
+    const int row = (j * 4 + wave) * 8 + lrow;
+    const int n = n0 + row;
+    const size_t wrow = FOLD ? (size_t)(mt & 3) * p.N + n : (size_t)n;
+    w_v[j] = (n < p.N) ? (unsigned)((wrow * p.K + (lch ^ ((row >> 1) & 7)) * 8) * 2) : OOB;
+  }
+  };
+  int iss_tile = tile_first, iss_left = tile_count;
+
+  const bool tapfast = p.korder != 0;
+  int cur_kt = kt0;
+  int cur_tap = 0, cur_c = 0, cur_koff = 0, cur_ky = 0, cur_kx = 0;
+  auto cursor_init = [&]() {
+    if (kt0 == 0) return;
+    const int tap0 = p.fd_on ? (int)dadd_fastdiv_div((uint32_t)(kt0 * BK), p.fd_cin) : (kt0 * BK) / Cin;
+    cur_tap = __builtin_amdgcn_readfirstlane(tapfast ? kt0 % 9 : tap0);
+    cur_c = __builtin_amdgcn_readfirstlane(tapfast ? (kt0 / 9) * BK : kt0 * BK - cur_tap * Cin);
+    cur_koff = __builtin_amdgcn_readfirstlane((cur_tap * Cin + cur_c) * 2);
+    cur_ky = (p.taps == 9) ? cur_tap / 3 : 0;
+    cur_kx = (p.taps == 9) ? cur_tap - 3 * cur_ky : 0;
+  };
+  int fill_off = wave * 1024;
+
+  struct IssueCtx {
+    __amdgpu_buffer_rsrc_t rsA, rsW;
+    unsigned soff, koff;
+    char* sa;
+    int cs, cb, ky, kx, tap;
+    bool second;
+  };
+  auto issue_begin = [&]() {
+    IssueCtx c;
+    const bool live = PERS ? iss_left > 0 : cur_kt < kt1;
+    c.second = cur_c >= p.C1;
+    c.cs = c.second ? p.C2 : p.C1;
+    c.cb = c.second ? cur_c - p.C1 : cur_c;
+    c.ky = cur_ky; c.kx = cur_kx; c.tap = cur_tap;
+    c.rsA = __builtin_amdgcn_make_buffer_rsrc((void*)(c.second ? base2 : base1), 0,
+                                              live ? (c.second ? rec2 : rec1) : 0, 0x00020000);
+    c.rsW = __builtin_amdgcn_make_buffer_rsrc((void*)p.w, 0, live ? recW : 0, 0x00020000);
+    c.sa = smem + fill_off;
+    c.soff = GATHER ? (unsigned)(c.cb * 2) : (unsigned)(((cur_ky * p.Wi + cur_kx) * c.cs + c.cb) * 2);
+    c.koff = (unsigned)cur_koff;
+    return c;
+  };
+  auto issue_w = [&](const IssueCtx& c, int j) {
+    __builtin_amdgcn_raw_ptr_buffer_load_lds(c.rsW, (lptr_t)(c.sa + A_BYTES + j * 4096), 16, w_v[j], c.koff, 0, 0);
+  };
+  auto issue_advance = [&]() {
+    ++cur_kt;
+    const int c1 = cur_c + BK;
+    const int cwrap = c1 >= Cin ? 1 : 0;
+    const int kx1 = cur_kx + (tapfast ? 1 : cwrap);
+    const int w3 = kx1 == (FOLD ? 2 : 3) ? 1 : 0;
+    cur_kx = w3 ? 0 : kx1;
+    const int ky1 = cur_ky + w3;
+    const int w9 = (tapfast && ky1 == 3) ? 1 : 0;
+    cur_ky = w9 ? 0 : ky1;
+    cur_koff += tapfast ? (w9 ? (BK - 8 * Cin) * 2 : Cin * 2) : BK * 2;
+    cur_tap = tapfast ? (w9 ? 0 : cur_tap + 1) : cur_tap + cwrap;
+    cur_c = tapfast ? cur_c + (w9 ? BK : 0) : (cwrap ? 0 : c1);
+    const int f1 = fill_off + STAGE;
+    fill_off = f1 >= 4 * STAGE ? f1 - 4 * STAGE : f1;
+    if constexpr (PERS) {
+      if (cur_kt == kt1) {
+        cur_kt = 0; cur_c = 0; cur_tap = 0; cur_ky = 0; cur_kx = 0; cur_koff = 0;
+        ++iss_tile;
+        --iss_left;
+        if (iss_left > 0) setup_tile(iss_tile);
+      }
+    }
+  };
+  unsigned a_eff[NA];
+  int eff_key = -1;
+  auto issue = [&]() {
+    const IssueCtx c = issue_begin();
+    {
+      const int key = c.tap * 2 + (c.second ? 1 : 0) + (PERS ? iss_tile * 32 : 0);
+      if (key != eff_key) {
+        eff_key = key;
+#pragma unroll
+        for (int i = 0; i < NA; ++i) {
+          if constexpr (!GATHER) {
+            a_eff[i] = ((a_mask[i] >> c.tap) & 1u) ? (c.second ? a_v2[i] : a_v1[i]) : OOB;
+          } else {
+            const int iy = a_y[i] + c.ky, ix = a_x[i] + c.kx;
+            const bool ok = (iy >= 0) & (iy < Hv) & (ix >= 0) & (ix < Wv);
+            a_eff[i] = ok ? (unsigned)(((a_pix[i] + (iy >> 1) * p.Wi + (ix >> 1)) * c.cs + a_cc[i]) * 2) : OOB;
+          }
+        }
+      }
+#pragma unroll
+      for (int i = 0; i < NA; ++i)
+        __builtin_amdgcn_raw_ptr_buffer_load_lds(c.rsA, (lptr_t)(c.sa + i * 4096), 16, a_eff[i], c.soff, 0, 0);
+#pragma unroll
+      for (int jj = 0; jj < NBJ; ++jj) issue_w(c, jj);
+    }
+    issue_advance();
+  };
+
+  const int total_kt = tile_count * nk;
+  char* const ln_scr = smem + 4 * STAGE;
+  const bool ln_stage = LNK == 2 && UPS == 0 && ln_lds_usable(p, BM, nk);
+  const bool ln_sts = ln_stage && ln_lds_stats(p, LN_LDS_BYTES);
+  if (loader) {
+    const int ln_extra = ln_stage ? ln_lds_count(p, wave, ln_sts) : 0;
+    cursor_init();
+    setup_tile(tile_first);
+    issue();
+    issue();
+    issue();
+    wait_vmcnt<LPT>();
+    __builtin_amdgcn_s_barrier();
+    bool ext_young = false;
+    int kc = 0, ext_tile = tile_first;
+    for (int it = 0; it < total_kt; ++it) {
+      if (it > 0) {
+        if (ext_young) {
+          switch (ln_extra) {
+            case 1: wait_vmcnt<LPT + 1>(); break;
+            case 2: wait_vmcnt<LPT + 2>(); break;
+            case 3: wait_vmcnt<LPT + 3>(); break;
+            case 4: wait_vmcnt<LPT + 4>(); break;
+            default: wait_vmcnt<LPT>(); break;
+          }
+          ext_young = false;
+        } else {
+          wait_vmcnt<LPT>();
+        }
+        __builtin_amdgcn_s_barrier();
+      }
+      issue();
+      if (ln_stage) {
+        if (kc == 0) {
+          int nt, mt;
+          tile_decode_fast(p, ext_tile, mt, nt);
+          ln_lds_issue<BN>(p, ln_scr, __builtin_amdgcn_readfirstlane(mt) * BM, __builtin_amdgcn_readfirstlane(nt) * BN, wave,
+                           lane, ln_sts);
+          ext_young = ln_extra > 0;
+          ++ext_tile;
+        }
+        kc = kc + 1 == nk ? 0 : kc + 1;
+      }
+    }
+    wait_vmcnt<0>();
+    return;
+  }
+  f4 acc[J][MI];
+  const int fq = lane >> 4;
+  int fa[2], fb[2];
+#pragma unroll
+  for (int s2 = 0; s2 < 2; ++s2) {
+    fa[s2] = lds_off(wm * WM + (lane & 15), s2 * 4 + fq) * 2;
+    fb[s2] = A_BYTES + lds_off(wn * WN + (lane & 15), s2 * 4 + fq) * 2;
+  }
+  unsigned pf_sink = 0;
+  if (!PERS && p.pf_kt > 0) {
+    int nt, mt;
+    tile_decode_fast(p, tile_first, mt, nt);
+    mt = __builtin_amdgcn_readfirstlane(mt);
+    const int n0 = __builtin_amdgcn_readfirstlane(nt) * BN;
+    const dadd_u4 dw = dadd_pf_desc(p.w, recW);
+    const unsigned row_bytes = (unsigned)p.K * 2u;
+    const int total = BN * min(nk, p.pf_kt);
+    if constexpr (FOLD) {
+      const int share = p.mtiles >> 2, mine = mt >> 2, wrow0 = (mt & 3) * p.N;
+      for (int q0 = wave * 64; q0 * share + mine < total; q0 += 256) {
+        const int l = (q0 + lane) * share + mine;
+        const int kt = l / BN, n = n0 + l - kt * BN;
+        const unsigned off = (l < total && n < p.N) ? (unsigned)(wrow0 + n) * row_bytes + (unsigned)(kt * BK * 2) : OOB;
+        dadd_pf_line(pf_sink, off, dw);
+      }
+    } else
+    for (int q0 = wave * 64; q0 * p.mtiles + mt < total; q0 += 256) {
+      const int l = (q0 + lane) * p.mtiles + mt;
+      const int kt = l / BN, n = n0 + l - kt * BN;
+      const unsigned off = (l < total && n < p.N) ? (unsigned)n * row_bytes + (unsigned)((kt0 + kt) * BK * 2) : OOB;
+      dadd_pf_line(pf_sink, off, dw);
+    }
+  }
+  __builtin_amdgcn_s_barrier();
+  __builtin_amdgcn_sched_barrier(0);
+  h8 xa0[MI], wb0[J], xa1[MI], wb1[J];
+#pragma unroll
+  for (int i = 0; i < MI; ++i) xa0[i] = *reinterpret_cast<const h8*>(smem + fa[0] + i * 2048);
+#pragma unroll
+  for (int j = 0; j < J; ++j) wb0[j] = *reinterpret_cast<const h8*>(smem + fb[0] + j * 2048);
+  int comp_off = 0;
+  bool started = false;
+  for (int tl = 0; tl < tile_count; ++tl) {
+#pragma unroll
+    for (int j = 0; j < J; ++j)
+#pragma unroll
+      for (int i = 0; i < MI; ++i) acc[j][i] = f4{0.f, 0.f, 0.f, 0.f};
+    [[maybe_unused]] float ls1[MI], ls2[MI];
+    constexpr int LQ = MI * 4, LPER = (LQ + MI * J - 1) / (MI * J);
+    if constexpr (LNF) {
+#pragma unroll
+      for (int i = 0; i < MI; ++i) ls1[i] = ls2[i] = 0.f;
+    }
+    for (int it = 0; it < nk; ++it) {
+      if (started) __builtin_amdgcn_s_barrier();
+      started = true;
+      __builtin_amdgcn_sched_barrier(0);
+      const int n1 = comp_off + STAGE;
+      const int next_off = n1 >= 4 * STAGE ? 0 : n1;
+      const char* ca = smem + comp_off + fa[1];
+      const char* cb1 = smem + comp_off + fb[1];
+      const char* na = smem + next_off + fa[0];
+      const char* nb = smem + next_off + fb[0];
+#pragma unroll
+      for (int k = 0; k < MI * J; ++k) {
+        const int jj = k / MI, ii = k % MI;
+        acc[jj][ii] = DADD_MFMA_16X16X32(wb0[jj], xa0[ii], acc[jj][ii], 0, 0, 0);
+        if constexpr (LNF) {
+#pragma unroll
+          for (int t2 = 0; t2 < LPER; ++t2)
+            if (k * LPER + t2 < LQ) ln_acc_pair(xa0[(k * LPER + t2) / 4], (k * LPER + t2) % 4, ls1[(k * LPER + t2) / 4], ls2[(k * LPER + t2) / 4]);
+        }
+        if (k == 0) wb1[0] = *reinterpret_cast<const h8*>(cb1);
+        else if (k <= MI) xa1[k - 1] = *reinterpret_cast<const h8*>(ca + (k - 1) * 2048);
+        else if (k < MI + J) wb1[k - MI] = *reinterpret_cast<const h8*>(cb1 + (k - MI) * 2048);
+        __builtin_amdgcn_sched_barrier(0);
+      }
+#pragma unroll
+      for (int k = 0; k < MI * J; ++k) {
+        const int jj = k / MI, ii = k % MI;
+        acc[jj][ii] = DADD_MFMA_16X16X32(wb1[jj], xa1[ii], acc[jj][ii], 0, 0, 0);
+        if constexpr (LNF) {
+#pragma unroll
+          for (int t2 = 0; t2 < LPER; ++t2)
+            if (k * LPER + t2 < LQ) ln_acc_pair(xa1[(k * LPER + t2) / 4], (k * LPER + t2) % 4, ls1[(k * LPER + t2) / 4], ls2[(k * LPER + t2) / 4]);
+        }
+        if (k == 0) wb0[0] = *reinterpret_cast<const h8*>(nb);
+        else if (k <= MI) xa0[k - 1] = *reinterpret_cast<const h8*>(na + (k - 1) * 2048);
+        else if (k < MI + J) wb0[k - MI] = *reinterpret_cast<const h8*>(nb + (k - MI) * 2048);
+        __builtin_amdgcn_sched_barrier(0);
+      }
+      comp_off = next_off;
+      __builtin_amdgcn_sched_barrier(0);
+    }
+    dadd_pf_drain(pf_sink);
+    int nt, mt;
+    tile_decode_fast(p, tile_first + tl, mt, nt);
+    if constexpr (LNF) {
+      ln_finish<MI>(ls1, ls2, p.K, p.ln_eps);
+      igemm_epilogue<J, MI, WM, WN, EPI>(p, acc, mt * BM, nt * BN, wm, wn, lane, z, smem, ls1, ls2);
+    } else {
+      igemm_epilogue<J, MI, WM, WN, EPI, FOLD>(p, acc, mt * BM, nt * BN, wm, wn, lane, z, smem, nullptr, nullptr, smem + 4 * STAGE,
+                                          ln_sts ? ln_scr + LN_LDS_STATS : nullptr, ln_stage ? ln_scr : nullptr);
+    }
+  }
+#endif
+}
+
+constexpr int smem_bytes(int bm, int bn) {
+  return 4 * (bm + bn) * BK * 2 + (bm == 128 ? LN_LDS_BYTES : 4096);
+}
+
+}
diff --git a/progressive-stable-diffusion_amd/csrc/igemm_epilogue.h b/progressive-stable-diffusion_amd/csrc/igemm_epilogue.h
--- a/progressive-stable-diffusion_amd/csrc/igemm_epilogue.h
+++ b/progressive-stable-diffusion_amd/csrc/igemm_epilogue.h
@@ -157,8 +157,16 @@
   return v;
 }
 
+template <int BM>
+__device__ __forceinline__ size_t epi_fold_row(const IgemmArgs& p, int m0, int row) {
+  const int mt = m0 / BM;
+  int b, y, x;
+  ups_fold_decode(p, (mt >> 2) * BM + row, b, y, x);
+  return ((size_t)(b * p.Ho + 2 * y + ((mt >> 1) & 1))) * p.Wo + 2 * x + (mt & 1);
+}
+
 enum { EPI_PLAIN = 0, EPI_FOLD_GLOBAL = 1, EPI_FOLD_LDS = 2 };
-template <int J, int MI, int WM, int WN, int MODE, int FOLD>
+template <int J, int MI, int WM, int WN, int MODE, int FOLD, bool UPSF = false>
 __device__ __forceinline__ void epi_tile(const IgemmArgs& p, f4 (&acc)[J][MI], int m0, int n0, int wm, int wn, int g, int mc,
                                          int HoWo, const float (&lmu)[MI], const float (&lrs)[MI], const char* ln_cb) {
   const bool lnstat = FOLD == EPI_PLAIN && (p.flags & DADD_EPI_LNSTAT) != 0 && n0 + wn * WN < p.N;
@@ -168,6 +176,11 @@
   float rs1[MI], rs2[MI];
 #pragma unroll
   for (int i = 0; i < MI; ++i) rs1[i] = rs2[i] = 0.f;
+  [[maybe_unused]] size_t orow[MI];
+  if constexpr (UPSF) {
+#pragma unroll
+    for (int i = 0; i < MI; ++i) orow[i] = epi_fold_row<2 * WM>(p, m0, wm * WM + i * 16 + mc);
+  }
   epi_for_each<J, MI, MODE>(
       [&](int o) __attribute__((always_inline)) { ops.batch(p, o, HoWo); },
       [&](int i, int j) __attribute__((always_inline)) {
@@ -196,7 +209,8 @@
             rs2[i] = fmaf(f, f, rs2[i]);
           }
         }
-        *reinterpret_cast<h4*>(p.out + (size_t)m * p.ldo + n) = o;
+        if constexpr (UPSF) *reinterpret_cast<h4*>(p.out + orow[i] * p.ldo + n) = o;
+        else *reinterpret_cast<h4*>(p.out + (size_t)m * p.ldo + n) = o;
       },
       [&](int i) __attribute__((always_inline)) {
         const int m = m0 + wm * WM + i * 16 + mc;
@@ -210,7 +224,7 @@
       });
 }
 
-template <int J, int MI, int WM, int WN, int MODE = EPI_TILE>
+template <int J, int MI, int WM, int WN, int MODE = EPI_TILE, bool UPSF = false>
 __device__ __forceinline__ void igemm_epilogue(const IgemmArgs& p, f4 (&acc)[J][MI], int m0, int n0,
                                                int wm, int wn, int lane, int z, char* smem,
                                                const float* ln_mu = nullptr, const float* ln_rs = nullptr,
@@ -265,7 +279,15 @@
   if (p.flags & DADD_EPI_GNSTAT) {
     float* scratch = reinterpret_cast<float*>(gn_scratch) + (wm * 2 + wn) * 256;
     const int mrow0 = m0 + wm * WM;
-    const int bsmp = row_sample(p, mrow0, HoWo);
+    [[maybe_unused]] const int fold_r0 = ((m0 / (2 * WM)) >> 2) * (2 * WM) + wm * WM, fold_ph = (m0 / (2 * WM)) & 3;
+    int bsmp;
+    if constexpr (UPSF) bsmp = p.fd_on ? (int)dadd_fastdiv_div((uint32_t)fold_r0, p.fd_howo) : fold_r0 / (p.Hi * p.Wi);
+    else bsmp = row_sample(p, mrow0, HoWo);
+    [[maybe_unused]] size_t orow[MI];
+    if constexpr (UPSF) {
+#pragma unroll
+      for (int i = 0; i < MI; ++i) orow[i] = epi_fold_row<2 * WM>(p, m0, wm * WM + i * 16 + mc);
+    }
     const bool has_bias = (p.flags & DADD_EPI_BIAS) != 0, has_rv = (p.flags & DADD_EPI_ROWVEC) != 0;
     const bool has_res = (p.flags & DADD_EPI_RESIDUAL) != 0;
     f4 b4[J], r4[J];
@@ -319,7 +341,8 @@
           cs[r] += f;
           cq[r] = fmaf(f, f, cq[r]);
         }
-        *reinterpret_cast<h4*>(p.out + (size_t)m * p.ldo + n) = o;
+        if constexpr (UPSF) *reinterpret_cast<h4*>(p.out + orow[i] * p.ldo + n) = o;
+        else *reinterpret_cast<h4*>(p.out + (size_t)m * p.ldo + n) = o;
       }
 #pragma unroll
       for (int r = 0; r < 4; ++r) {
@@ -344,7 +367,9 @@
         a += scratch[(lane * p.gn_cg + c) * 2];
         q += scratch[(lane * p.gn_cg + c) * 2 + 1];
       }
-      const int chunk = (mrow0 - bsmp * HoWo) / WM;
+      int chunk;
+      if constexpr (UPSF) chunk = (fold_ph * (p.Hi * p.Wi) + fold_r0 - bsmp * (p.Hi * p.Wi)) / WM;
+      else chunk = (mrow0 - bsmp * HoWo) / WM;
       const int grp = (n0 + wn * WN) / p.gn_cg + lane;
       float* w = p.gn_ws + (((size_t)bsmp * p.gn_nchunk + chunk) * 32 + grp) * 2;
       w[0] = a;
@@ -487,6 +512,10 @@
     }
     return;
   }
+  if constexpr (UPSF) {
+    epi_tile<J, MI, WM, WN, MODE, EPI_PLAIN, true>(p, acc, m0, n0, wm, wn, g, mc, HoWo, lmu, lrs, ln_cb);
+    return;
+  }
   if (lds_fold) epi_tile<J, MI, WM, WN, MODE, EPI_FOLD_LDS>(p, acc, m0, n0, wm, wn, g, mc, HoWo, lmu, lrs, ln_cb);
   else if (fold) epi_tile<J, MI, WM, WN, MODE, EPI_FOLD_GLOBAL>(p, acc, m0, n0, wm, wn, g, mc, HoWo, lmu, lrs, ln_cb);
   else epi_tile<J, MI, WM, WN, MODE, EPI_PLAIN>(p, acc, m0, n0, wm, wn, g, mc, HoWo, lmu, lrs, ln_cb);
diff --git a/progressive-stable-diffusion_amd/csrc/igemm_ups_fold.hip b/progressive-stable-diffusion_amd/csrc/igemm_ups_fold.hip
--- /dev/null
+++ b/progressive-stable-diffusion_amd/csrc/igemm_ups_fold.hip
@@ -0,0 +1,15 @@
+#define DADD_IGEMM_UPS_FOLD
+#include "igemm_dma_kernel.h"
+
+namespace {
+
+#define FOLD_ROW(BM, BN) \
+  {DADD_KNAME("igemm_ups_fold_kernel") "<" #BM ", " #BN ">", igemm_ups_fold_kernel<BM, BN>, 512, smem_bytes(BM, BN), {BM, BN}}
+const IgemmKernel FOLD_KERNELS[] = {FOLD_ROW(128, 128), FOLD_ROW(128, 160)};
+#undef FOLD_ROW
+
+}
+
+int dadd_init_igemm_ups_fold() { return dadd_set_max_lds(FOLD_KERNELS); }
+
+const IgemmKernel* dadd_igemm_ups_fold_row(int tile_m, int tile_n) { return dadd_find_row(FOLD_KERNELS, tile_m, tile_n); }
diff --git a/progressive-stable-diffusion_amd/csrc/igemm_ups_fold_bf16.hip b/progressive-stable-diffusion_amd/csrc/igemm_ups_fold_bf16.hip
--- /dev/null
+++ b/progressive-stable-diffusion_amd/csrc/igemm_ups_fold_bf16.hip
@@ -0,0 +1,2 @@
+#include "bf16_names.h"
+#include "igemm_ups_fold.hip"
diff --git a/progressive-stable-diffusion_amd/engine.py b/progressive-stable-diffusion_amd/engine.py
--- a/progressive-stable-diffusion_amd/engine.py
+++ b/progressive-stable-diffusion_amd/engine.py
@@ -53,6 +53,19 @@
     w16 = (w * gamma[None, :]).to(dtype)
     bias = w @ beta + (b.double() if b is not None else 0.0)
     return w16, w16.double().sum(dim=1).float(), bias.float()
+
+
+def fold_ups_weight(w9: torch.Tensor) -> torch.Tensor:
+    n, cin = w9.shape[0], w9.shape[1] // 9
+    assert w9.dim() == 2 and w9.shape[1] == 9 * cin
+    w = w9.reshape(n, 3, 3, cin).double()
+    sets = (((0,), (1, 2)), ((0, 1), (2,)))
+    phases = []
+    for py in range(2):
+        for px in range(2):
+            taps = [w[:, list(sets[py][dy])][:, :, list(sets[px][dx])].sum((1, 2)) for dy in range(2) for dx in range(2)]
+            phases.append(torch.stack(taps, 1).reshape(n, 4 * cin))
+    return torch.stack(phases, 0).to(w9.dtype).contiguous()
 
 
 def lds_image(w: torch.Tensor) -> torch.Tensor:
@@ -113,6 +126,22 @@
 SPLITK_GN_ROWS = 16
 
 
+UPS_FOLD = True
+
+
+def ups_fold_tiling(m: int, n: int, cin: int) -> Optional[Tuple[int, int, int, int]]:
+    if not UPS_FOLD:
+        return None
+    key = tiling_key(m, n, 4 * cin, 9, False, False, 1, 1)
+    hit = TILING_OVERRIDE.get(key) or TILING_TABLE.get(key)
+    if hit is not None:
+        return tuple(hit) if hit[3] & L.TUNE_UPS_FOLD else None
+    tile_m, tile_n, sk, tune = plan_tiling(m, n, 9 * cin, 9, False, False, 1, 1)
+    if sk != 1 or tile_m != 128 or (m // 4) % 128 or (tune & L.TUNE_NODMA):
+        return None
+    return tile_m, tile_n, 1, tune | L.TUNE_UPS_FOLD
+
+
 LN_FOLD = "auto"
 LN_STATS_FROM_PRODUCER = True
 LN_STATS_MAX_PARTS = 8
@@ -288,6 +317,12 @@
         return self.cached((self.prefix + key, pack.__name__),
                            lambda: self.be.to_device(pack(self.sd[self.prefix + key], self.dtype)))
 
+    def ups_fold(self, w9):
+        w4 = self.cached(("ups_fold", w9.data_ptr()), lambda: self.be.to_device(fold_ups_weight(w9.cpu())))
+        if hasattr(self.be, "register_ups_fold"):
+            self.be.register_ups_fold(w9, w4)
+        return w4
+
     def f(self, key):
         return self.cached((self.prefix + key, "f32"), lambda: self.be.to_device(self.sd[self.prefix + key].float()))
 
@@ -311,6 +346,10 @@
         m = out_shape[0] * out_shape[1] * out_shape[2]
         tile_m, tile_n, sk, tune = plan_tiling(m, n, w.shape[1], taps, bool(flags & L.EPI_GEGLU), residual is not None,
                                                ups, stride)
+        fold = ups_fold_tiling(m, n, w.shape[1] // 9) if ups and x2 is None and residual is None and rowvec is None else None
+        if fold is not None:
+            tile_m, tile_n, sk, tune = fold
+            self.ups_fold(w)
         if taps == 9 and HALO_DUO:
             tune |= L.TUNE_SHALLOW
         if ln_c1 is not None:
diff --git a/progressive-stable-diffusion_amd/lib.py b/progressive-stable-diffusion_amd/lib.py
--- a/progressive-stable-diffusion_amd/lib.py
+++ b/progressive-stable-diffusion_amd/lib.py
@@ -12,6 +12,7 @@
                    "optim")
 _TWINNED_SOURCES = (
     "igemm", "igemm_dma", "conv_halo", "norm", "attention", "elementwise",
+    "igemm_ups_fold",
     "wgrad",
     "norm_grad",
     "attn_grad",
@@ -28,6 +29,7 @@
 PRE_GN, PRE_GN_SILU = 8192, 16384
 EPI_GNAPPLY, EPI_GNAPPLY_SILU = 32768, 65536
 TUNE_SHALLOW, TUNE_NODMA, TUNE_PERSIST = 16, 32, 64
+TUNE_UPS_FOLD = 131072
 XATTN_SPLIT, XATTN_BASELINE = 0, 1
 DGRAD_STRIDE2, DGRAD_UPS = 0, 1
 END_WGRAD_IN, END_WGRAD_OUT = 0, 1
@@ -44,7 +46,8 @@
                                                            ("ln_stats_out", vp), ("ln_stats_in", vp), ("ln_parts_out", i32), ("ln_parts_in", i32),
                                                            ("gn_in_ws", vp), ("gn_in_gamma", vp), ("gn_in_beta", vp), ("gn_in_nchunk", i32), ("gn_in_eps", f32),
                                                            ("gn_in_ws2", vp), ("gn_in_nchunk2", i32),
-                                                           ("gn_out", vp), ("gn_out_gamma", vp), ("gn_out_beta", vp), ("gn_out_eps", f32)]
+                                                           ("gn_out", vp), ("gn_out_gamma", vp), ("gn_out_beta", vp), ("gn_out_eps", f32),
+                                                           ("w_fold", vp)]
 
 
 class IgemmChoice(C.Structure):
```

New measurement: 11.73 images/sec (median of 6 runs). 1.02x the previous value.
